# peter-seres/python-ray-tracer

Hardware: AMD Instinct MI355X
Metric: Mrays/sec + frame time (ms) at 1920x1080, 8 spheres, depth=3 (higher is better)
Workload: dtype f64

## Files before the change

### python-ray-tracer_amd/csrc/mi355rt.hip

```cpp
#include "../../include/mi355rt.h"
#include "rt_device.h"
#include "rt_bloom.h"
#include "rt_denoise.h"
#include "rt_denoise_var.h"
#include "rt_feedback.h"
#include "rt_film.h"
#include "rt_film_launch.h"
#include "rt_geometry.h"
#include "rt_guides.h"
#include "rt_launch.h"
#include "rt_plan.h"
#include "rt_scene.h"
#include "rt_streams.h"
#include "rt_temporal.h"

#include <cmath>
#include <cstdio>
#include <cstdlib>
#include <algorithm>
#include <array>
#include <cstring>
#include <memory>
#include <new>
#include <string>
#include <type_traits>
#include <utility>
#include <vector>

#pragma clang fp contract(off)

namespace {

std::string g_create_error;

struct Buf {
    void *p = nullptr;
    size_t cap = 0;
    Buf() = default;
    Buf(Buf &&o) noexcept { *this = std::move(o); }
    Buf &operator=(Buf &&o) noexcept { std::swap(p, o.p); std::swap(cap, o.cap); return *this; }
    ~Buf() { if (p) (void)hipFree(p); }
};

}

#define RT_COUNT_WORDS (4 + 2 * (RT_MAX_DEPTH + 1))
#define RT_RENDER_CHUNKS 8

struct rt_ctx {
    int device = 0;
    hipStream_t stream = nullptr;
    struct Pipeline {
        hipStream_t stream2 = nullptr, copy_stream = nullptr;
        hipEvent_t chunk_ev[RT_RENDER_CHUNKS] = {};
        hipStream_t chunk_stream[RT_RENDER_CHUNKS] = {};
        template <class F> void streams(F f)
        {
            for (hipStream_t s : {stream2, copy_stream}) if (s) f(s);
            for (hipStream_t s : chunk_stream) if (s) f(s);
        }
        ~Pipeline()
        {
            streams([](hipStream_t s) { (void)hipStreamDestroy(s); });
            for (hipEvent_t e : chunk_ev) if (e) (void)hipEventDestroy(e);
        }
    };
    std::unique_ptr<Pipeline> pipe;
    int chunk_mode = -1;
    int cluster_min = rt::CLUSTER_MIN;
    int lanes_primary = 1;
    rt::PlanKnobs knobs;
    int render_chunks = 4;
    int log_kernels = 0;
    int remeasure = 24;
    struct Slot {
        hipStream_t stream = nullptr;
        Buf u8, f32;
    } slots[RT_RENDER_SLOTS];
    hipEvent_t ev0 = nullptr, ev1 = nullptr;
    Buf scene[RT_SCENE_RING];
    int scene_cur = 0;
    Buf pixel_loc, u8, f32;
    rt::SceneLayout lay;
    Buf texels[RT_SCENE_RING];
    bool have_scene = false;
    rt::View view;
    size_t lds_limit_set[rt::FAMILIES] = {};
    size_t ground_lds_set = 0;
    size_t guides_lds_set = 0;
    unsigned *tile_stats = nullptr;
    struct Feedback : rt::FeedbackSlot {
        Buf cost, gtmp, btmp, order[2];
    } fbs[RT_FEEDBACK_SLOTS];
    rt::FeedbackBook book;
    rt_ctx() { for (int i = 0; i < RT_FEEDBACK_SLOTS; ++i) book.slot[i] = &fbs[i]; }
    template <class F> void own_streams(F f)
    {
        if (stream) f(stream);
        for (Slot &sl : slots) if (sl.stream) f(sl.stream);
        if (pipe) pipe->streams(f);
    }
    ~rt_ctx()
    {
        for (auto &f : fbs)
            for (void *e : rt::release_events(f)) (void)hipEventDestroy((hipEvent_t)e);
        pipe.reset();
        own_streams([](hipStream_t s) { (void)hipStreamDestroy(s); });
        for (hipEvent_t e : {ev0, ev1}) if (e) (void)hipEventDestroy(e);
    }
    rt_stats stats = {};
    Buf counts;
    int cu_count = 256;
    unsigned long long epoch = 1;
    unsigned long long scene_epoch = 1;
    rt::StreamBook<Buf> streams;
    std::string err;
};

namespace {

int fail(rt_ctx *ctx, int code, const std::string &msg)
{
    if (ctx) ctx->err = msg; else g_create_error = msg;
    return code;
}

#define RT_HIP(ctx, call)                                                                         \
    do {                                                                                          \
        hipError_t e_ = (call);                                                                   \
        if (e_ != hipSuccess)                                                                     \
            return fail((ctx), RT_ERR_HIP, std::string(#call) + ": " + hipGetErrorString(e_));    \
    } while (0)

int ensure(rt_ctx *ctx, Buf &b, size_t bytes)
{
    if (bytes <= b.cap) return RT_OK;
    if (b.p) { RT_HIP(ctx, hipFree(b.p)); b.p = nullptr; b.cap = 0; }
    RT_HIP(ctx, hipMalloc(&b.p, bytes));
    b.cap = bytes;
    return RT_OK;
}

int refuse(rt_ctx *ctx, const rt::Refusal &r)
{
    if (r.code == RT_OK) return RT_OK;
    return fail(ctx, r.code, r.entry ? std::string(r.entry) + ": " + r.msg : std::string(r.msg));
}

int check_params(rt_ctx *ctx, const rt_params *p, int x0, int x1) { return refuse(ctx, rt::check_params(ctx->have_scene, ctx->view, ctx->lay, p, x0, x1)); }

hipStream_t stream_of(rt_ctx *ctx, void *stream) { return stream ? (hipStream_t)stream : ctx->stream; }

using StreamRecord = rt::StreamBook<Buf>::Record;

int stream_record(rt_ctx *ctx, hipStream_t stream, StreamRecord **out)
{
    const int rc = ctx->streams.record(stream, out);
    if (rc != RT_OK) return fail(ctx, rc, ctx->streams.NO_MEMORY);
    ctx->streams.reads_scene(**out, ctx->scene_cur);
    return RT_OK;
}

int raise_lds(rt_ctx *ctx, const void *const *fns, size_t n, size_t lds, size_t &set)
{
    if (lds <= 48 * 1024 || lds <= set) return RT_OK;
    for (size_t i = 0; i < n; ++i)
        if (fns[i]) RT_HIP(ctx, hipFuncSetAttribute(fns[i], hipFuncAttributeMaxDynamicSharedMemorySize, (int)lds));
    set = lds;
    return RT_OK;
}

using rt::Shape; using rt::SHAPES; using rt::NSHAPES; using rt::has_kernel; using rt::has_ground_kernel;

template <rt::Family F, int I, bool GROUND = false>
const void *kernel_at()
{
    constexpr Shape s = SHAPES[I];
    if constexpr (GROUND ? has_ground_kernel(F, s) : has_kernel(F, s))
        return (const void *)rt::render_kernel<s.aa, s.park, s.wpw, s.count, s.lat, s.mode, F, GROUND>;
    else
        return nullptr;
}
template <rt::Family F, int... I>
std::array<const void *, NSHAPES> family_kernels(std::integer_sequence<int, I...>)
{
    return {kernel_at<F, I>()...};
}
template <int... I>
std::array<const void *, NSHAPES> ground_kernels(std::integer_sequence<int, I...>)
{
    return {kernel_at<rt::Family::PLAIN, I, true>()...};
}

constexpr std::make_integer_sequence<int, NSHAPES> ALL_SHAPES{};
const std::array<const void *, NSHAPES> KERNELS[rt::FAMILIES] = {
    family_kernels<rt::Family::PLAIN>(ALL_SHAPES), family_kernels<rt::Family::MAT>(ALL_SHAPES),
    family_kernels<rt::Family::REFR>(ALL_SHAPES),  family_kernels<rt::Family::SCAT>(ALL_SHAPES),
    family_kernels<rt::Family::SOFT>(ALL_SHAPES),  family_kernels<rt::Family::LENS>(ALL_SHAPES),
    family_kernels<rt::Family::LENS_SOFT>(ALL_SHAPES),
    family_kernels<rt::Family::TEX_SCAT>(ALL_SHAPES), family_kernels<rt::Family::TEX_SOFT>(ALL_SHAPES),
    family_kernels<rt::Family::TEX_LENS>(ALL_SHAPES), family_kernels<rt::Family::TEX_LENS_SOFT>(ALL_SHAPES),
    family_kernels<rt::Family::LIT_SCAT>(ALL_SHAPES), family_kernels<rt::Family::LIT_SOFT>(ALL_SHAPES),
    family_kernels<rt::Family::LIT_LENS>(ALL_SHAPES), family_kernels<rt::Family::LIT_LENS_SOFT>(ALL_SHAPES),
    family_kernels<rt::Family::SKY_SCAT>(ALL_SHAPES), family_kernels<rt::Family::SKY_SOFT>(ALL_SHAPES),
    family_kernels<rt::Family::SKY_LENS>(ALL_SHAPES), family_kernels<rt::Family::SKY_LENS_SOFT>(ALL_SHAPES),
};
const std::array<const void *, NSHAPES> GROUND_KERNELS = ground_kernels(ALL_SHAPES);
const std::array<const void *, NSHAPES> &kernels_of(int fi, bool ground) { return ground ? GROUND_KERNELS : KERNELS[fi]; }
static_assert(rt::FAMILIES == 19 && (int)rt::Family::TEX_LENS_SOFT == 10 && (int)rt::Family::LIT_LENS_SOFT == 14 &&
              (int)rt::Family::SKY_SCAT == 15 && (int)rt::Family::SKY_LENS_SOFT == 18,
              "KERNELS lists the families in enum order");

int stream_buffer(rt_ctx *ctx, Buf &b, hipStream_t stream, size_t bytes, bool sync)
{
    if (sync) RT_HIP(ctx, hipStreamSynchronize(stream));
    return ensure(ctx, b, bytes);
}

int acquire_tables(rt_ctx *ctx, StreamRecord &sr, const rt::KParams &k, const float **out)
{
    const hipStream_t stream = (hipStream_t)sr.stream;
    const rt::TableKey key = rt::table_key(ctx->scene_epoch, k.anchors, k.floor_anch, k.cam_o);
    const size_t bytes = rt::table_floats(k.S, k.NC, k.anchors, false, true, k.P) * sizeof(float);
    const rt::TableDecision d = ctx->streams.tables(sr, key, bytes);
    Buf &b = sr.buf[rt::BUF_TABLES0 + d.set];
    if (d.rebuild) {
        int rc = stream_buffer(ctx, b, stream, d.bytes, d.sync);
        if (rc != RT_OK) return rc;
        hipLaunchKernelGGL(rt::tables_kernel, dim3(1), dim3(rt::TABLE_THREADS), 0, stream, k, (float *)b.p);
        ctx->stats.table_builds++;
        RT_HIP(ctx, hipGetLastError());
        ctx->streams.tables_queued(sr, d.set, key);
    }
    *out = (const float *)b.p;
    return RT_OK;
}

int dispatch(rt_ctx *ctx, const rt_params *p, rt::KParams &k, const rt::LaunchPlan &plan, hipStream_t stream, int nframes, int64_t frame_stride);

int launch(rt_ctx *ctx, const rt_params *p, int x0, int x1, void *d_u8, void *d_f32, int64_t plane_stride,
           hipStream_t stream, int nframes = 1, int64_t frame_stride = 0)
{
    const rt::View &v = ctx->view;
    long long li0 = 0, li1 = 0;
    const bool lattice = p->aa_mode == RT_AA_REFERENCE && !v.explicit_grid && rt_geo_lattice(v.w, v.h, x0, x1, &li0, &li1) &&
                         !(p->flags & RT_FLAG_AA_PER_PIXEL);
    const rt::LaunchPlan plan = rt::plan_launch(ctx->lay, ctx->knobs, v.lens_a, !lattice && p->aa_mode != 0, p->flags, lattice, rt::anchors_of(ctx->lay));
    if (plan.index < 0 || !KERNELS[(int)plan.family][plan.index])
        return fail(ctx, RT_ERR_STATE, "no render kernel for this launch");
    StreamRecord *sr = nullptr;
    int rc = stream_record(ctx, stream, &sr);
    if (rc != RT_OK) return rc;
    rt::KParams k;
    rt::render_part(k, v, ctx->lay, plan.family, p, (const double *)ctx->scene[ctx->scene_cur].p, (const double *)ctx->pixel_loc.p,
                    (const float *)ctx->texels[ctx->scene_cur].p, ctx->lanes_primary, x0, x1, d_u8, d_f32, plane_stride, ctx->tile_stats);
    rc = acquire_tables(ctx, *sr, k, &k.ftab);
    if (rc != RT_OK) return rc;
    if (lattice) {
        Buf &lb = sr->buf[rt::BUF_LATTICE];
        const size_t bytes = (size_t)(li1 - li0) * (size_t)(2ll * v.h - 1) * 3 * sizeof(double);
        rc = stream_buffer(ctx, lb, stream, bytes, rt::growth(lb.cap, bytes).sync);
        if (rc != RT_OK) return rc;
        double *lat = (double *)lb.p;
        rt::KParams kl;
        rt::lattice_pair(k, kl, li0, li1, lat);
        const long long npx = (long long)(x1 - x0) * v.h;
        for (int f = 0; f < nframes; ++f) {
            rc = dispatch(ctx, p, kl, plan, stream, 1, 0);
            if (rc != RT_OK) return rc;
            const rt::KParams kf = rt::frame_params(k, f, frame_stride);
            hipLaunchKernelGGL(rt::aa_resolve_kernel, dim3((unsigned)((npx + 255) / 256)), dim3(256), 0, stream, kf);
            RT_HIP(ctx, hipGetLastError());
        }
        return RT_OK;
    }
    return dispatch(ctx, p, k, plan, stream, nframes, frame_stride);
}

using Feedback = rt_ctx::Feedback;
static_assert(std::is_convertible<hipStream_t, void *>::value && std::is_convertible<hipEvent_t, void *>::value,
              "rt_feedback.h keeps streams and events as opaque handles");
int feedback_slot(rt_ctx *ctx, const rt::FeedbackKey &key, Feedback **out);
int switch_order(rt_ctx *ctx, Feedback &f);
int launch_one(rt_ctx *ctx, rt::KParams &k, const rt::LaunchPlan &plan, const rt_geo_plan &g, const rt::OrderShape &os,
               Feedback *f, hipStream_t stream, int nframes, int64_t frame_stride);

int dispatch(rt_ctx *ctx, const rt_params *p, rt::KParams &k, const rt::LaunchPlan &plan, hipStream_t stream, int nframes, int64_t frame_stride)
{
    const int x0 = k.x0, x1 = k.x1;
    const rt_geo_plan g = rt_geo_plan_of(x0, x1, k.h, plan.shape.wpw, nframes);
    auto frame_of = [&](int fr) { return rt::frame_params(k, fr, frame_stride); };
    if (g.nslabs > 1) {
        for (int fr = 0; fr < nframes; ++fr)
            for (long long s = 0; s < g.nslabs; ++s) {
                rt::KParams kf = rt::slab_params(frame_of(fr), g, s);
                int rc = dispatch(ctx, p, kf, plan, stream, 1, 0);
                if (rc != RT_OK) return rc;
            }
        return RT_OK;
    }
    if (nframes > g.frames_per_dispatch) {
        const int fpd = (int)g.frames_per_dispatch;
        for (int fr = 0; fr < nframes; fr += fpd) {
            rt::KParams kf = frame_of(fr);
            int rc = dispatch(ctx, p, kf, plan, stream, std::min(fpd, nframes - fr), frame_stride);
            if (rc != RT_OK) return rc;
        }
        return RT_OK;
    }
    const rt::OrderShape os = rt::order_shape(plan, ctx->knobs, p->flags, g);
    Feedback *f = nullptr;
    if (os.feedback) {
        int rc = feedback_slot(ctx, rt::feedback_key(x0, x1, k.h, k.aa, plan.shape.lat, k.depth, k.spp, os.code), &f);
        if (rc == RT_OK) rc = switch_order(ctx, *f);
        if (rc != RT_OK) return rc;
    }
    if (nframes > 1 && f && !rt::settled(*f, ctx->epoch, ctx->remeasure)) {
        rt::KParams kf = frame_of(0);
        int rc = dispatch(ctx, p, kf, plan, stream, 1, 0);
        if (rc != RT_OK) return rc;
        if (f->building) RT_HIP(ctx, hipEventSynchronize((hipEvent_t)f->done));
        rt::KParams kr = frame_of(1);
        return dispatch(ctx, p, kr, plan, stream, nframes - 1, frame_stride);
    }
    return launch_one(ctx, k, plan, g, os, f, stream, nframes, frame_stride);
}

int feedback_slot(rt_ctx *ctx, const rt::FeedbackKey &key, Feedback **out)
{
    bool live = false;
    const int i = ctx->book.find(key, &live);
    if (live) RT_HIP(ctx, hipDeviceSynchronize());
    ctx->book.claim(i, key);
    Feedback *f = &ctx->fbs[i];
    if (!f->done) {
        hipEvent_t ev = nullptr;
        RT_HIP(ctx, hipEventCreateWithFlags(&ev, hipEventDisableTiming));
        f->done = ev;
    }
    *out = f;
    return RT_OK;
}

int switch_order(rt_ctx *ctx, Feedback &f)
{
    if (!f.building) return RT_OK;
    const hipError_t q = hipEventQuery((hipEvent_t)f.done);
    if (q != hipSuccess) {
        (void)hipGetLastError();
        return RT_OK;
    }
    for (void *us : rt::switch_order(f)) {
        hipEvent_t ev = (hipEvent_t)rt::take_spare(f);
        if (!ev) RT_HIP(ctx, hipEventCreateWithFlags(&ev, hipEventDisableTiming));
        RT_HIP(ctx, hipEventRecord(ev, (hipStream_t)us));
        rt::add_fence(f, us, ev);
    }
    return RT_OK;
}

int launch_one(rt_ctx *ctx, rt::KParams &k, const rt::LaunchPlan &plan, const rt_geo_plan &g, const rt::OrderShape &os,
               Feedback *f, hipStream_t stream, int nframes, int64_t frame_stride)
{
    const Shape &sh = plan.shape;
    const int fi = (int)plan.family;
    const bool ground = rt::ground_plane(ctx->lay, ctx->knobs, plan.family, sh.count ? RT_FLAG_COUNT_RAYS : 0) && has_ground_kernel(plan.family, sh);
    const std::array<const void *, NSHAPES> &kernels = kernels_of(fi, ground);
    const void *fn = kernels[plan.index];
    if (!fn) return fail(ctx, RT_ERR_STATE, "no render kernel for this launch");
    const unsigned grid = (unsigned)g.blocks;
    if (ctx->log_kernels)
        std::fprintf(stderr, "mi355rt: render_kernel<%d, %d, %d, %d, %d, %d, (rt::Family)%d>%s\n", (int)sh.aa, (int)sh.park, sh.wpw, (int)sh.count,
                     (int)sh.lat, sh.mode, fi, ground ? " ground" : "");
    int rc = raise_lds(ctx, kernels.data(), kernels.size(), plan.lds, ground ? ctx->ground_lds_set : ctx->lds_limit_set[fi]);
    if (rc != RT_OK) return rc;
    if (sh.count) {
        if (!ctx->counts.p) {
            rc = ensure(ctx, ctx->counts, RT_COUNT_WORDS * sizeof(unsigned long long));
            if (rc != RT_OK) return rc;
            RT_HIP(ctx, hipMemsetAsync(ctx->counts.p, 0, RT_COUNT_WORDS * sizeof(unsigned long long), stream));
        }
        k.ray_counts = (unsigned long long *)ctx->counts.p;
    }
    const rt::FeedbackLaunch d = f ? rt::decide_launch(*f, stream, ctx->epoch, ctx->remeasure) : rt::FeedbackLaunch{};
    if (d.read >= 0) k.order = (const unsigned *)f->order[d.read].p;
    if (d.measure) {
        const size_t words = (size_t)os.items * sizeof(unsigned);
        rc = ensure(ctx, f->cost, words);
        if (rc == RT_OK) rc = ensure(ctx, f->btmp, words);
        if (rc == RT_OK) rc = ensure(ctx, f->order[0], 2 * words);
        if (rc == RT_OK) rc = ensure(ctx, f->order[1], 2 * words);
        if (rc == RT_OK) rc = ensure(ctx, f->gtmp, words + sizeof(unsigned));
        if (rc != RT_OK) return rc;
        for (void *ev : d.wait) RT_HIP(ctx, hipStreamWaitEvent(stream, (hipEvent_t)ev, 0));
        k.cost = (unsigned *)f->cost.p;
    }
    rt::dispatch_part(k, nframes, grid, frame_stride, os);
    void *args[] = {(void *)&k};
    RT_HIP(ctx, hipLaunchKernel(fn, dim3(grid * (unsigned)nframes), dim3(64 * sh.wpw), args, plan.lds, stream));
    ctx->stats.launches++;
    ctx->stats.frames += (uint64_t)nframes;
    if (d.settled) ctx->stats.launches_settled++;
    if (d.measure) ctx->stats.launches_measuring++;
    if (d.measure) {
        hipLaunchKernelGGL(rt::order_kernel, dim3(1), dim3(rt::ORDER_THREADS), 0, stream, (const unsigned *)f->cost.p,
                           (unsigned *)f->gtmp.p, (unsigned *)f->btmp.p, (unsigned *)f->order[d.write].p, (int)os.items, os.otiles ? os.gshift + os.wshift : os.gshift,
                           os.otiles ? os.wshift : 0, os.otiles ? k.ntiles : (int)grid);
        RT_HIP(ctx, hipEventRecord((hipEvent_t)f->done, stream));
        rt::order_queued(*f, ctx->epoch);
    }
    RT_HIP(ctx, hipGetLastError());
    return RT_OK;
}

template <class Prepare>
int variance_filter(rt_ctx *ctx, const rt::DenoiseVarArgs &common, int levels, const rt::FilmPingPong &pp, hipStream_t st, Prepare prepare)
{
    const dim3 grid(rt::denoise_grid((long long)common.ws * common.h, ctx->cu_count));
    for (int k = 0; k <= levels; ++k) {
        const rt::FilmWrite w = rt::film_write(true, levels, k, nullptr, 0, pp);
        if (k == 0) prepare(w, grid);
        else hipLaunchKernelGGL(rt::denoise_var_kernel, grid, dim3(rt::DENOISE_THREADS), 0, st, rt::denoise_var_write(common, w, levels, k));
        RT_HIP(ctx, hipGetLastError());
    }
    return RT_OK;
}

template <class Args>
int temporal_launch(rt_ctx *ctx, void (*kernel)(Args), const Args &a, void *stream)
{
    RT_HIP(ctx, hipSetDevice(ctx->device));
    hipLaunchKernelGGL(kernel, dim3(rt::temporal_grid((long long)ctx->view.w * ctx->view.h, ctx->cu_count)), dim3(rt::TEMPORAL_THREADS), 0,
                       stream_of(ctx, stream), a);
    RT_HIP(ctx, hipGetLastError());
    return RT_OK;
}

}

extern "C" {

int rt_abi_version(void) { return RT_ABI_VERSION; }

int rt_device_count(int *count)
{
    if (!count) return RT_ERR_BAD_ARG;
    int n = 0;
    hipError_t e = hipGetDeviceCount(&n);
    if (e != hipSuccess) { *count = 0; g_create_error = std::string("hipGetDeviceCount: ") + hipGetErrorString(e); return RT_ERR_NO_DEVICE; }
    *count = n;
    return RT_OK;
}

int rt_create(rt_ctx **out, int device)
{
    if (!out) return fail(nullptr, RT_ERR_BAD_ARG, "ctx out-pointer is NULL");
    *out = nullptr;
    int n = 0;
    hipError_t e = hipGetDeviceCount(&n);
    if (e != hipSuccess || n <= 0)
        return fail(nullptr, RT_ERR_NO_DEVICE, std::string("no HIP device: ") + (e != hipSuccess ? hipGetErrorString(e) : "device count is 0"));
    if (device < 0 || device >= n) return fail(nullptr, RT_ERR_NO_DEVICE, "device index out of range");
    rt_ctx *ctx = new (std::nothrow) rt_ctx;
    if (!ctx) return fail(nullptr, RT_ERR_ALLOC, "out of host memory");
    ctx->device = device;
    if (const char *e = std::getenv("MI355RT_LANES_PRIMARY")) ctx->lanes_primary = std::atoi(e);
    if (const char *e = std::getenv("MI355RT_LANES_MINS")) ctx->knobs.lanes_min_spheres = std::atoi(e);
    if (const char *e = std::getenv("MI355RT_CLUSTER_MINS")) ctx->cluster_min = std::max(8, std::atoi(e));
    if (const char *e = std::getenv("MI355RT_CHUNK_MODE")) ctx->chunk_mode = std::atoi(e);
    if (const char *e = std::getenv("MI355RT_ORDER_GROUP")) { const int v = std::atoi(e); if (v >= 0 && v <= 6) ctx->knobs.order_group = v; }
    if (const char *e = std::getenv("MI355RT_REMEASURE")) ctx->remeasure = std::max(0, std::atoi(e));
    if (const char *e = std::getenv("MI355RT_F32_RECORDS")) ctx->knobs.f32_records = std::atoi(e) != 0;
    if (const char *e = std::getenv("MI355RT_WPW2_MAX_IMAGE")) ctx->knobs.wpw2_max_image = (size_t)std::max(0, std::atoi(e));
    if (const char *e = std::getenv("MI355RT_ORDER_TILES")) ctx->knobs.order_tiles = std::atoi(e) != 0;
    if (const char *e = std::getenv("MI355RT_LANES_PARK")) ctx->knobs.lanes_park = std::atoi(e) != 0;
    if (const char *e = std::getenv("MI355RT_GROUND_PLANE")) ctx->knobs.ground_plane = std::atoi(e) != 0;
    if (const char *e = std::getenv("MI355RT_LOG_KERNELS")) ctx->log_kernels = std::atoi(e) != 0;
    if (const char *e = std::getenv("MI355RT_SEQ_ORDER")) ctx->knobs.seq_order = std::atoi(e) != 0 ? 1 : 0;
    if (const char *e = std::getenv("MI355RT_CHUNKS")) { const int v = std::atoi(e); if (v >= 1 && v <= RT_RENDER_CHUNKS) ctx->render_chunks = v; }
    hipError_t s;
    if ((s = hipSetDevice(device)) != hipSuccess || (s = hipStreamCreateWithFlags(&ctx->stream, hipStreamNonBlocking)) != hipSuccess ||
        (s = hipEventCreate(&ctx->ev0)) != hipSuccess || (s = hipEventCreate(&ctx->ev1)) != hipSuccess) {
        std::string m = std::string("context setup: ") + hipGetErrorString(s);
        delete ctx;
        return fail(nullptr, RT_ERR_HIP, m);
    }
    {
        int cus = 0;
        if (hipDeviceGetAttribute(&cus, hipDeviceAttributeMultiprocessorCount, device) == hipSuccess && cus > 0) ctx->cu_count = cus;
        else (void)hipGetLastError();
    }
    *out = ctx;
    return RT_OK;
}

int rt_destroy(rt_ctx *ctx)
{
    if (!ctx) return RT_OK;
    (void)hipSetDevice(ctx->device);
    ctx->own_streams([](hipStream_t s) { (void)hipStreamSynchronize(s); });
    delete ctx;
    return RT_OK;
}

const char *rt_last_error(const rt_ctx *ctx) { return ctx ? ctx->err.c_str() : g_create_error.c_str(); }

static int set_scene(rt_ctx *ctx, const rt::SceneDesc &desc)
{
    if (!ctx) return RT_ERR_BAD_ARG;
    const rt::PackedScene ps = rt::pack_scene(desc, ctx->cluster_min, ctx->knobs.lanes_min_spheres);
    if (ps.status != RT_OK) return fail(ctx, ps.status, ps.error);
    RT_HIP(ctx, hipSetDevice(ctx->device));
    const size_t bytes = ps.rec.size() * sizeof(double);
    const int next = (ctx->scene_cur + 1) % RT_SCENE_RING;
    int rc = ctx->streams.drain_scene(next, [ctx](void *st) { RT_HIP(ctx, hipStreamSynchronize((hipStream_t)st)); return (int)RT_OK; });
    if (rc == RT_OK) rc = ensure(ctx, ctx->scene[next], bytes);
    if (rc != RT_OK) return rc;
    if (ps.layout.T > 0 || ps.layout.lit) {
        rc = ensure(ctx, ctx->texels[next], ps.texels.size() * sizeof(float));
        if (rc != RT_OK) return rc;
        RT_HIP(ctx, hipMemcpyAsync(ctx->texels[next].p, ps.texels.data(), ps.texels.size() * sizeof(float), hipMemcpyHostToDevice, ctx->stream));
    }
    RT_HIP(ctx, hipMemcpyAsync(ctx->scene[next].p, ps.rec.data(), bytes, hipMemcpyHostToDevice, ctx->stream));
    RT_HIP(ctx, hipStreamSynchronize(ctx->stream));
    ctx->scene_cur = next;
    ctx->lay = ps.layout;
    ctx->have_scene = true;
    ctx->epoch++;
    ctx->scene_epoch++;
    return RT_OK;
}

static rt::SceneDesc scene_desc(const float *spheres, int S, const float *lights, int L, const float *planes, int P, int flags,
                                const double *materials, int M, int ncols, const int32_t *sphere_material, const int32_t *plane_material)
{
    rt::SceneDesc d;
    d.spheres = spheres; d.S = S; d.lights = lights; d.L = L; d.planes = planes; d.P = P; d.flags = flags;
    d.materials = materials; d.M = M; d.ncols = ncols; d.sphere_material = sphere_material; d.plane_material = plane_material;
    return d;
}

static void add_textures(rt::SceneDesc &d, const rt_texture *textures, int T, const int32_t *sphere_texture, const int32_t *plane_texture,
                         const float *texels, int64_t n_texels)
{
    d.textures = textures; d.T = T; d.sphere_texture = sphere_texture; d.plane_texture = plane_texture;
    d.texels = texels; d.n_texels = n_texels;
}

static int set_scene_radii(rt_ctx *ctx, rt::SceneDesc &d, const float *light_radius, int shadow_samples)
{
    if (!ctx) return RT_ERR_BAD_ARG;
    if (d.L > 0 && !light_radius) return fail(ctx, RT_ERR_BAD_ARG, "light_radius is NULL with L > 0");
    static const float none = 0.0f;
    d.light_radius = light_radius ? light_radius : &none;
    d.shadow_samples = shadow_samples;
    return set_scene(ctx, d);
}

int rt_set_scene(rt_ctx *ctx, const float *spheres, int S, const float *lights, int L, const float *planes, int P, int flags)
{
    return set_scene(ctx, scene_desc(spheres, S, lights, L, planes, P, flags, nullptr, 0, 3, nullptr, nullptr));
}

int rt_set_scene_materials(rt_ctx *ctx, const float *spheres, int S, const float *lights, int L, const float *planes, int P, int flags,
                           const double *materials, int M, const int32_t *sphere_material, const int32_t *plane_material)
{
    return set_scene(ctx, scene_desc(spheres, S, lights, L, planes, P, flags, materials, M, 3, sphere_material, plane_material));
}

int rt_set_scene_materials_ex(rt_ctx *ctx, const float *spheres, int S, const float *lights, int L, const float *planes, int P, int flags,
                              const double *materials, int M, int ncols, const int32_t *sphere_material, const int32_t *plane_material)
{
    if (!ctx) return RT_ERR_BAD_ARG;
    if (ncols != 3 && ncols != 5) return fail(ctx, RT_ERR_BAD_ARG, "ncols must be 3 or 5");
    return set_scene(ctx, scene_desc(spheres, S, lights, L, planes, P, flags, materials, M, ncols, sphere_material, plane_material));
}

int rt_set_scene_materials_scatter(rt_ctx *ctx, const float *spheres, int S, const float *lights, int L, const float *planes, int P,
                                   int flags, const double *materials, int M, int ncols, const int32_t *sphere_material,
                                   const int32_t *plane_material)
{
    return set_scene(ctx, scene_desc(spheres, S, lights, L, planes, P, flags, materials, M, ncols, sphere_material, plane_material));
}

int rt_set_scene_area_lights(rt_ctx *ctx, const float *spheres, int S, const float *lights, int L, const float *planes, int P,
                             int flags, const double *materials, int M, int ncols, const int32_t *sphere_material,
                             const int32_t *plane_material, const float *light_radius, int shadow_samples)
{
    rt::SceneDesc d = scene_desc(spheres, S, lights, L, planes, P, flags, materials, M, ncols, sphere_material, plane_material);
    return set_scene_radii(ctx, d, light_radius, shadow_samples);
}

int rt_set_scene_textures(rt_ctx *ctx, const float *spheres, int S, const float *lights, int L, const float *planes, int P,
                          int flags, const double *materials, int M, int ncols, const int32_t *sphere_material,
                          const int32_t *plane_material, const float *light_radius, int shadow_samples,
                          const rt_texture *textures, int T, const int32_t *sphere_texture, const int32_t *plane_texture,
                          const float *texels, int64_t n_texels)
{
    rt::SceneDesc d = scene_desc(spheres, S, lights, L, planes, P, flags, materials, M, ncols, sphere_material, plane_material);
    add_textures(d, textures, T, sphere_texture, plane_texture, texels, n_texels);
    return set_scene_radii(ctx, d, light_radius, shadow_samples);
}

int rt_set_scene_lighting(rt_ctx *ctx, const float *spheres, int S, const float *lights, int L, const float *planes, int P,
                          int flags, const double *materials, int M, int ncols, const int32_t *sphere_material,
                          const int32_t *plane_material, const float *light_radius, int shadow_samples,
                          const rt_texture *textures, int T, const int32_t *sphere_texture, const int32_t *plane_texture,
                          const float *texels, int64_t n_texels, const float *light_rgb)
{
    rt::SceneDesc d = scene_desc(spheres, S, lights, L, planes, P, flags, materials, M, ncols, sphere_material, plane_material);
    add_textures(d, textures, T, sphere_texture, plane_texture, texels, n_texels);
    d.light_rgb = light_rgb; d.lighting = true;
    return set_scene_radii(ctx, d, light_radius, shadow_samples);
}

int rt_set_scene_sky(rt_ctx *ctx, const float *spheres, int S, const float *lights, int L, const float *planes, int P,
                     int flags, const double *materials, int M, int ncols, const int32_t *sphere_material,
                     const int32_t *plane_material, const float *light_radius, int shadow_samples,
                     const rt_texture *textures, int T, const int32_t *sphere_texture, const int32_t *plane_texture,
                     const float *texels, int64_t n_texels, const float *light_rgb, const double *sky)
{
    rt::SceneDesc d = scene_desc(spheres, S, lights, L, planes, P, flags, materials, M, ncols, sphere_material, plane_material);
    add_textures(d, textures, T, sphere_texture, plane_texture, texels, n_texels);
    d.light_rgb = light_rgb; d.lighting = true; d.sky = sky;
    return set_scene_radii(ctx, d, light_radius, shadow_samples);
}

int rt_set_camera(rt_ctx *ctx, const double origin[3], const double rotation[9])
{
    if (!ctx) return RT_ERR_BAD_ARG;
    if (!origin || !rotation) return fail(ctx, RT_ERR_BAD_ARG, "NULL camera array");
    rt::View &v = ctx->view;
    if (v.have_cam && std::memcmp(v.cam_o, origin, sizeof v.cam_o) == 0 &&
        std::memcmp(v.cam_R, rotation, sizeof v.cam_R) == 0) return RT_OK;
    std::memcpy(v.cam_o, origin, sizeof v.cam_o);
    std::memcpy(v.cam_R, rotation, sizeof v.cam_R);
    v.have_cam = true;
    ctx->epoch++;
    return RT_OK;
}

int rt_set_lens(rt_ctx *ctx, double aperture, double focus_distance)
{
    if (!ctx) return RT_ERR_BAD_ARG;
    if (!(std::isfinite(aperture) && aperture >= 0.0)) return fail(ctx, RT_ERR_BAD_ARG, "aperture must be finite and >= 0");
    if (!(std::isfinite(focus_distance) && focus_distance > 0.0))
        return fail(ctx, RT_ERR_BAD_ARG, "focus_distance must be finite and > 0");
    rt::View &v = ctx->view;
    if (aperture == v.lens_a && (focus_distance == v.lens_f || aperture == 0.0)) { v.lens_f = focus_distance; return RT_OK; }
    v.lens_a = aperture;
    v.lens_f = focus_distance;
    ctx->epoch++;
    return RT_OK;
}

int rt_set_raygen(rt_ctx *ctx, int w, int h, double px, double y0, double dy, double z0, double dz)
{
    if (!ctx) return RT_ERR_BAD_ARG;
    if (!rt_geo_frame_ok(w, h)) return fail(ctx, RT_ERR_BAD_ARG, "frame size out of range (1 <= w <= 2^31 - 8, 1 <= h <= 2^29 - 32, w*h <= 2^31)");
    rt::View &v = ctx->view;
    {
        const double now[5] = {px, y0, dy, z0, dz}, was[5] = {v.px, v.y0, v.dy, v.z0, v.dz};
        if (v.have_grid && !v.explicit_grid && v.w == w && v.h == h && std::memcmp(now, was, sizeof now) == 0)
            return RT_OK;
    }
    v.w = w; v.h = h; v.px = px; v.y0 = y0; v.dy = dy; v.z0 = z0; v.dz = dz;
    v.explicit_grid = false;
    v.have_grid = true;
    ctx->epoch++;
    return RT_OK;
}

int rt_set_pixel_loc(rt_ctx *ctx, const double *pixel_loc, int w, int h)
{
    if (!ctx) return RT_ERR_BAD_ARG;
    if (!pixel_loc) return fail(ctx, RT_ERR_BAD_ARG, "pixel_loc is NULL");
    if (!rt_geo_frame_ok(w, h)) return fail(ctx, RT_ERR_BAD_ARG, "frame size out of range (1 <= w <= 2^31 - 8, 1 <= h <= 2^29 - 32, w*h <= 2^31)");
    RT_HIP(ctx, hipSetDevice(ctx->device));
    const size_t bytes = (size_t)3 * w * h * sizeof(double);
    if (ctx->pixel_loc.p) RT_HIP(ctx, hipDeviceSynchronize());
    int rc = ensure(ctx, ctx->pixel_loc, bytes);
    if (rc != RT_OK) return rc;
    RT_HIP(ctx, hipMemcpyAsync(ctx->pixel_loc.p, pixel_loc, bytes, hipMemcpyHostToDevice, ctx->stream));
    RT_HIP(ctx, hipStreamSynchronize(ctx->stream));
    ctx->view.w = w; ctx->view.h = h;
    ctx->view.explicit_grid = true;
    ctx->view.have_grid = true;
    ctx->epoch++;
    return RT_OK;
}

int rt_render_device(rt_ctx *ctx, const rt_params *params, int x0, int x1, void *d_u8, void *d_f32, int64_t plane_stride, void *stream)
{
    if (!ctx) return RT_ERR_BAD_ARG;
    int rc = check_params(ctx, params, x0, x1);
    if (rc == RT_OK) rc = refuse(ctx, rt::check_device_outputs(ctx->view, params, x0, x1, 1, d_u8, d_f32, plane_stride, 0));
    if (rc != RT_OK) return rc;
    RT_HIP(ctx, hipSetDevice(ctx->device));
    return launch(ctx, params, x0, x1, d_u8, d_f32, plane_stride, stream_of(ctx, stream));
}

int rt_render_sequence(rt_ctx *ctx, const rt_params *params, int x0, int x1, int n, void *d_u8, void *d_f32, int64_t plane_stride,
                       int64_t frame_stride, const double *cameras, void *const *streams, int n_streams, int frames_per_launch)
{
    if (!ctx) return RT_ERR_BAD_ARG;
    if (n < 0) return fail(ctx, RT_ERR_BAD_ARG, "rt_render_sequence: negative frame count");
    if (n == 0) return RT_OK;
    if (cameras) {
        int rc0 = rt_set_camera(ctx, cameras, cameras + 3);
        if (rc0 != RT_OK) return rc0;
    }
    int rc = check_params(ctx, params, x0, x1);
    if (rc == RT_OK) rc = refuse(ctx, rt::check_device_outputs(ctx->view, params, x0, x1, n, d_u8, d_f32, plane_stride, frame_stride));
    if (rc != RT_OK) return rc;
    if (n_streams < 0 || (n_streams > 0 && !streams)) return fail(ctx, RT_ERR_BAD_ARG, "rt_render_sequence: n_streams without a stream array");
    RT_HIP(ctx, hipSetDevice(ctx->device));
    auto stream_of = [&](int i) { return (n_streams > 0 && streams[i % n_streams]) ? (hipStream_t)streams[i % n_streams] : ctx->stream; };
    uint8_t *u8 = (uint8_t *)d_u8;
    float *f32 = (float *)d_f32;
    if (cameras) {
        for (int i = 0; i < n; ++i) {
            rc = rt_set_camera(ctx, cameras + 12 * (size_t)i, cameras + 12 * (size_t)i + 3);
            if (rc == RT_OK) rc = launch(ctx, params, x0, x1, u8 ? u8 + (size_t)i * frame_stride : nullptr,
                                         f32 ? f32 + (size_t)i * frame_stride : nullptr, plane_stride, stream_of(i));
            if (rc != RT_OK) return rc;
        }
        return RT_OK;
    }
    const int fpl = frames_per_launch > 0 ? frames_per_launch : 8;
    for (int i = 0, g = 0; i < n; i += fpl, ++g) {
        const int nf = std::min(fpl, n - i);
        rc = launch(ctx, params, x0, x1, u8 ? u8 + (size_t)i * frame_stride : nullptr, f32 ? f32 + (size_t)i * frame_stride : nullptr,
                    plane_stride, stream_of(g), nf, frame_stride);
        if (rc != RT_OK) return rc;
    }
    return RT_OK;
}

static int film_queue_passes(rt_ctx *ctx, const rt_params *params, int x0, int x1, int passes, int reset, void *d_sum, int64_t sum_stride,
                             void *d_sq, int64_t sq_stride, void *stream)
{
    int rc = RT_OK;
    const long long npx = (long long)(x1 - x0) * ctx->view.h;
    RT_HIP(ctx, hipSetDevice(ctx->device));
    hipStream_t st = stream_of(ctx, stream);
    rt_params p = *params;
    p.flags &= ~(RT_FLAG_U8_RGB | RT_FLAG_U8_HWC);
    const rt::FilmBatch fb = rt::film_batch(npx, passes);
    StreamRecord *sr = nullptr;
    rc = stream_record(ctx, st, &sr);
    if (rc != RT_OK) return rc;
    Buf &scratch = sr->buf[rt::BUF_FILM];
    rc = stream_buffer(ctx, scratch, st, fb.batch * fb.pass_bytes, rt::growth(scratch.cap, fb.batch * fb.pass_bytes).sync);
    if (rc != RT_OK) return rc;
    float *const frames = (float *)scratch.p;
    const dim3 grid(rt::film_grid((npx + 3) >> 2, ctx->cu_count, 3), 3);
    for (int i = 0; i < passes; i += fb.batch) {
        const int nb = std::min(fb.batch, passes - i), first = (reset && i == 0) ? 1 : 0;
        for (int b = 0; b < nb; ++b) {
            p.seed = params->seed + (uint32_t)(i + b);
            rc = launch(ctx, &p, x0, x1, nullptr, frames + (size_t)b * 3 * fb.fplane, fb.fplane, st);
            if (rc != RT_OK) return rc;
        }
        if (d_sq) hipLaunchKernelGGL(rt::film_add2_kernel, grid, dim3(rt::FILM_THREADS), 0, st,
                                     rt::film_add2_args(d_sum, sum_stride, d_sq, sq_stride, frames, fb.fplane, npx, nb, first));
        else hipLaunchKernelGGL(rt::film_add_kernel, grid, dim3(rt::FILM_THREADS), 0, st, rt::film_add_args(d_sum, sum_stride, frames, fb.fplane, npx, nb, first));
        RT_HIP(ctx, hipGetLastError());
    }
    return RT_OK;
}

int rt_film_accumulate(rt_ctx *ctx, const rt_params *params, int x0, int x1, int passes, int reset, void *d_sum, int64_t sum_stride,
                       void *stream)
{
    if (!ctx) return RT_ERR_BAD_ARG;
    int rc = refuse(ctx, rt::check_film_accumulate("rt_film_accumulate", ctx->have_scene, ctx->view, ctx->lay, params, x0, x1, passes, d_sum, sum_stride,
                                                   false, nullptr, 0));
    if (rc != RT_OK) return rc;
    return film_queue_passes(ctx, params, x0, x1, passes, reset, d_sum, sum_stride, nullptr, 0, stream);
}

int rt_film_accumulate_moments(rt_ctx *ctx, const rt_params *params, int x0, int x1, int passes, int reset, void *d_sum, int64_t sum_stride,
                               void *d_sq, int64_t sq_stride, void *stream)
{
    if (!ctx) return RT_ERR_BAD_ARG;
    int rc = refuse(ctx, rt::check_film_accumulate("rt_film_accumulate_moments", ctx->have_scene, ctx->view, ctx->lay, params, x0, x1, passes, d_sum,
                                                   sum_stride, true, d_sq, sq_stride));
    if (rc != RT_OK) return rc;
    return film_queue_passes(ctx, params, x0, x1, passes, reset, d_sum, sum_stride, d_sq, sq_stride, stream);
}

int rt_film_resolve(rt_ctx *ctx, const void *d_sum, int64_t sum_stride, int ws, int h, int64_t n, const rt_film_tone *tone,
                    void *d_u8, void *d_f32, int64_t out_stride, void *stream)
{
    if (!ctx) return RT_ERR_BAD_ARG;
    int rc = refuse(ctx, rt::check_film_resolve(d_sum, sum_stride, ws, h, n, tone, d_u8, d_f32, out_stride));
    if (rc != RT_OK) return rc;
    RT_HIP(ctx, hipSetDevice(ctx->device));
    const rt::FilmResolveArgs a = rt::film_resolve_args(d_sum, sum_stride, ws, h, n, tone, d_u8, d_f32, out_stride);
    hipLaunchKernelGGL(rt::film_resolve_kernel, dim3(rt::film_grid((a.npx + 3) >> 2, ctx->cu_count, 1)), dim3(rt::FILM_THREADS), 0,
                       stream_of(ctx, stream), a);
    RT_HIP(ctx, hipGetLastError());
    return RT_OK;
}

int rt_render_guides(rt_ctx *ctx, int x0, int x1, void *d_guides, int64_t plane_stride, void *stream)
{
    if (!ctx) return RT_ERR_BAD_ARG;
    if (!d_guides) return fail(ctx, RT_ERR_BAD_ARG, "rt_render_guides: d_guides is NULL");
    const rt::View &v = ctx->view;
    int rc = refuse(ctx, rt::check_state(ctx->have_scene, v));
    if (rc == RT_OK) rc = refuse(ctx, rt::check_columns(v, x0, x1));
    if (rc != RT_OK) return rc;
    if (plane_stride < (int64_t)(x1 - x0) * v.h) return fail(ctx, RT_ERR_BAD_ARG, "rt_render_guides: plane_stride smaller than the slab");
    RT_HIP(ctx, hipSetDevice(ctx->device));
    hipStream_t st = stream_of(ctx, stream);
    StreamRecord *sr = nullptr;
    rc = stream_record(ctx, st, &sr);
    if (rc != RT_OK) return rc;
    rt::KParams k;
    rt::guides_part(k, v, ctx->lay, (const double *)ctx->scene[ctx->scene_cur].p, (const double *)ctx->pixel_loc.p,
                    (const float *)ctx->texels[ctx->scene_cur].p, ctx->lanes_primary, x0, x1, d_guides, plane_stride);
    const rt::GuidesPlan plan = rt::plan_guides(ctx->lay, ctx->knobs, k.anchors);
    if (ctx->log_kernels) std::fprintf(stderr, "mi355rt: guides_kernel<%d>\n", plan.mode);
    rc = acquire_tables(ctx, *sr, k, &k.ftab);
    if (rc != RT_OK) return rc;
    const void *fn = plan.mode == 2 ? (const void *)rt::guides_kernel<2> : (plan.mode == 1 ? (const void *)rt::guides_kernel<1> : (const void *)rt::guides_kernel<0>);
    const void *const all[] = {(const void *)rt::guides_kernel<0>, (const void *)rt::guides_kernel<1>, (const void *)rt::guides_kernel<2>};
    rc = raise_lds(ctx, all, 3, plan.lds, ctx->guides_lds_set);
    if (rc != RT_OK) return rc;
    rt::div_magic((unsigned)k.tiles_y, k.tiles_y_magic, k.tiles_y_shift);
    const rt_geo_plan g = rt_geo_plan_of(x0, x1, v.h, rt::GUIDE_WPW, 1);
    for (long long s = 0; s < g.nslabs; ++s) {
        rt::KParams ks = rt::slab_params(k, g, s);
        int tex = ctx->lay.T > 0 ? 1 : 0;
        void *args[] = {(void *)&ks, (void *)&tex};
        const unsigned blocks = (unsigned)((ks.ntiles + rt::GUIDE_WPW - 1) / rt::GUIDE_WPW);
        RT_HIP(ctx, hipLaunchKernel(fn, dim3(blocks), dim3(64 * rt::GUIDE_WPW), args, plan.lds, st));
    }
    RT_HIP(ctx, hipGetLastError());
    return RT_OK;
}

int rt_film_denoise(rt_ctx *ctx, const void *d_sum, int64_t sum_stride, int ws, int h, int64_t n, const void *d_guides, int64_t guide_stride,
                    const rt_denoise *dn, void *d_out, int64_t out_stride, void *d_work, int64_t work_stride, void *stream)
{
    if (!ctx) return RT_ERR_BAD_ARG;
    int nsq = -1;
    int rc = refuse(ctx, rt::check_film_denoise(d_sum, sum_stride, ws, h, n, d_guides, guide_stride, dn, d_out, out_stride, d_work, work_stride, nsq));
    if (rc != RT_OK) return rc;
    RT_HIP(ctx, hipSetDevice(ctx->device));
    hipStream_t st = stream_of(ctx, stream);
    const rt::FilmPingPong pp = {d_out, out_stride, d_work, work_stride};
    const dim3 grid(rt::denoise_grid((long long)ws * h, ctx->cu_count));
    for (int i = 0; i < (dn->levels ? dn->levels : 1); ++i) {
        const rt::FilmWrite w = rt::film_write(false, dn->levels, i, d_sum, sum_stride, pp);
        hipLaunchKernelGGL(rt::denoise_kernel, grid, dim3(rt::DENOISE_THREADS), 0, st, rt::denoise_args(w, d_guides, guide_stride, ws, h, n, dn, nsq, i));
        RT_HIP(ctx, hipGetLastError());
    }
    return RT_OK;
}

int rt_film_denoise_variance(rt_ctx *ctx, const void *d_sum, int64_t sum_stride, const void *d_sq, int64_t sq_stride, int ws, int h, int64_t n,
                             const void *d_guides, int64_t guide_stride, const rt_denoise_variance *dv, void *d_out, int64_t out_stride,
                             void *d_work, int64_t work_stride, void *stream)
{
    if (!ctx) return RT_ERR_BAD_ARG;
    int nsq = -1;
    int rc = refuse(ctx, rt::check_film_denoise_variance(d_sum, sum_stride, d_sq, sq_stride, ws, h, n, d_guides, guide_stride, dv, d_out, out_stride,
                                                         d_work, work_stride, nsq));
    if (rc != RT_OK) return rc;
    RT_HIP(ctx, hipSetDevice(ctx->device));
    hipStream_t st = stream_of(ctx, stream);
    rt::DenoiseVarArgs a = rt::denoise_var_common(d_guides, guide_stride, ws, h, dv, nsq);
    rt::denoise_var_inputs(a, d_sum, sum_stride, d_sq, sq_stride, n, dv->levels);
    return variance_filter(ctx, a, dv->levels, {d_out, out_stride, d_work, work_stride}, st, [&](const rt::FilmWrite &w, dim3 grid) {
        hipLaunchKernelGGL(rt::denoise_var_prepare_kernel, grid, dim3(rt::DENOISE_THREADS), 0, st, rt::denoise_var_write(a, w, dv->levels, 0));
    });
}

int rt_film_temporal(rt_ctx *ctx, const void *d_sum, int64_t sum_stride, int64_t n, const void *d_guides, int64_t guide_stride,
                     const void *d_hist, int64_t hist_stride, const void *d_hist_len, const void *d_hist_guides, int64_t hist_guide_stride,
                     const rt_temporal *tp, void *d_out, int64_t out_stride, void *d_out_len, void *stream)
{
    if (!ctx) return RT_ERR_BAD_ARG;
    const rt::View &v = ctx->view;
    int rc = refuse(ctx, rt::check_film_temporal("rt_film_temporal", v, d_sum, sum_stride, n, d_guides, guide_stride, d_hist, hist_stride, d_hist_len,
                                                 d_hist_guides, hist_guide_stride, tp, d_out, out_stride, d_out_len));
    if (rc != RT_OK) return rc;
    rt::TemporalArgs a;
    rt::temporal_args(a, v, d_sum, sum_stride, n, d_guides, guide_stride, d_hist, hist_stride, d_hist_len, d_hist_guides, hist_guide_stride, tp, d_out,
                      out_stride, d_out_len);
    return temporal_launch(ctx, rt::temporal_kernel, a, stream);
}

int rt_film_temporal_moments(rt_ctx *ctx, const void *d_sum, int64_t sum_stride, const void *d_sq, int64_t sq_stride, int64_t n,
                             const void *d_guides, int64_t guide_stride, const void *d_hist, int64_t hist_stride, const void *d_hist_sq,
                             int64_t hist_sq_stride, const void *d_hist_len, const void *d_hist_guides, int64_t hist_guide_stride,
                             const rt_temporal *tp, void *d_out, int64_t out_stride, void *d_out_sq, int64_t out_sq_stride, void *d_out_len,
                             void *stream)
{
    if (!ctx) return RT_ERR_BAD_ARG;
    const rt::View &v = ctx->view;
    int rc = refuse(ctx, rt::check_film_temporal_moments(v, d_sum, sum_stride, d_sq, sq_stride, n, d_guides, guide_stride, d_hist, hist_stride, d_hist_sq,
                                                         hist_sq_stride, d_hist_len, d_hist_guides, hist_guide_stride, tp, d_out, out_stride, d_out_sq,
                                                         out_sq_stride, d_out_len));
    if (rc != RT_OK) return rc;
    rt::TemporalMomentsArgs m;
    rt::temporal_args(m.t, v, d_sum, sum_stride, n, d_guides, guide_stride, d_hist, hist_stride, d_hist_len, d_hist_guides, hist_guide_stride, tp, d_out,
                      out_stride, d_out_len);
    rt::temporal_moments_args(m, d_sq, sq_stride, d_hist_sq, hist_sq_stride, d_out_sq, out_sq_stride);
    return temporal_launch(ctx, rt::temporal_moments_kernel, m, stream);
}

int rt_film_denoise_variance_temporal(rt_ctx *ctx, const void *d_mean, int64_t mean_stride, const void *d_msq, int64_t msq_stride,
                                      const void *d_len, int ws, int h, const void *d_guides, int64_t guide_stride,
                                      const rt_denoise_variance *dv, double spatial_below, void *d_out, int64_t out_stride, void *d_work,
                                      int64_t work_stride, void *stream)
{
    if (!ctx) return RT_ERR_BAD_ARG;
    int nsq = -1;
    int rc = refuse(ctx, rt::check_film_denoise_variance_temporal(d_mean, mean_stride, d_msq, msq_stride, d_len, ws, h, d_guides, guide_stride, dv,
                                                                  spatial_below, d_out, out_stride, d_work, work_stride, nsq));
    if (rc != RT_OK) return rc;
    RT_HIP(ctx, hipSetDevice(ctx->device));
    hipStream_t st = stream_of(ctx, stream);
    return variance_filter(ctx, rt::denoise_var_common(d_guides, guide_stride, ws, h, dv, nsq), dv->levels, {d_out, out_stride, d_work, work_stride}, st,
                           [&](const rt::FilmWrite &w, dim3 grid) {
        hipLaunchKernelGGL(rt::denoise_var_prepare_len_kernel, grid, dim3(rt::DENOISE_THREADS), 0, st,
                           rt::denoise_var_len_args(w, d_mean, mean_stride, d_msq, msq_stride, d_len, ws, h, d_guides, guide_stride, dv, spatial_below));
    });
}

int rt_film_bloom(rt_ctx *ctx, const void *d_sum, int64_t sum_stride, int ws, int h, int64_t n, const rt_bloom *bl, void *d_out,
                  int64_t out_stride, void *d_work, int64_t work_stride, void *stream)
{
    if (!ctx) return RT_ERR_BAD_ARG;
    int rc = refuse(ctx, rt::check_film_bloom(d_sum, sum_stride, ws, h, n, bl, d_out, out_stride, d_work, work_stride));
    if (rc != RT_OK) return rc;
    RT_HIP(ctx, hipSetDevice(ctx->device));
    hipStream_t st = stream_of(ctx, stream);
    const rt::BloomPlan plan = rt::bloom_plan(bl->levels, bl->flags);
    const dim3 grid(rt::bloom_grid((long long)ws * h, ctx->cu_count)), tiles(rt::bloom_tile_blocks(ws, h), 3), threads(rt::BLOOM_THREADS);
    for (int k = 0; k < plan.count; ++k) {
        const rt::BloomLaunch &l = plan.l[k];
        const rt::BloomArgs a = rt::bloom_args(l, d_sum, sum_stride, ws, h, n, bl, d_out, out_stride, d_work, work_stride);
        if (l.kind == rt::BLOOM_BRIGHT) hipLaunchKernelGGL(rt::bloom_bright_kernel, grid, threads, 0, st, a);
        else if (l.kind == rt::BLOOM_X) hipLaunchKernelGGL(rt::bloom_x_kernel, grid, threads, 0, st, a);
        else if (l.kind == rt::BLOOM_Y) hipLaunchKernelGGL(rt::bloom_y_kernel, grid, threads, 0, st, a);
        else if (l.step == 1) hipLaunchKernelGGL(rt::bloom_tile_kernel<1>, tiles, threads, 0, st, a);
        else if (l.step == 2) hipLaunchKernelGGL(rt::bloom_tile_kernel<2>, tiles, threads, 0, st, a);
        else hipLaunchKernelGGL(rt::bloom_tile_kernel<4>, tiles, threads, 0, st, a);
        RT_HIP(ctx, hipGetLastError());
    }
    return RT_OK;
}

static int render_staged(rt_ctx *ctx, const rt_params *params, int x0, int x1, uint8_t *out_u8, float *out_f32, Buf &u8, Buf &f32,
                         hipStream_t stream)
{
    const size_t npx = (size_t)(x1 - x0) * ctx->view.h;
    int rc = out_u8 ? ensure(ctx, u8, 3 * npx) : RT_OK;
    if (rc == RT_OK && out_f32) rc = ensure(ctx, f32, 3 * npx * sizeof(float));
    if (rc == RT_OK)
        rc = launch(ctx, params, x0, x1, out_u8 ? u8.p : nullptr, out_f32 ? f32.p : nullptr,
                    (params->flags & RT_FLAG_U8_HWC) ? (int64_t)(x1 - x0) : (int64_t)npx, stream);
    if (rc != RT_OK) return rc;
    if (out_u8) RT_HIP(ctx, hipMemcpyAsync(out_u8, u8.p, 3 * npx, hipMemcpyDeviceToHost, stream));
    if (out_f32) RT_HIP(ctx, hipMemcpyAsync(out_f32, f32.p, 3 * npx * sizeof(float), hipMemcpyDeviceToHost, stream));
    return RT_OK;
}

int rt_render(rt_ctx *ctx, const rt_params *params, int x0, int x1, uint8_t *out_u8, float *out_f32)
{
    if (!ctx) return RT_ERR_BAD_ARG;
    int rc = check_params(ctx, params, x0, x1);
    if (rc != RT_OK) return rc;
    if (!out_u8 && !out_f32) return fail(ctx, RT_ERR_BAD_ARG, "both output pointers are NULL");
    RT_HIP(ctx, hipSetDevice(ctx->device));
    const size_t npx = (size_t)(x1 - x0) * ctx->view.h;
    if (out_u8 && (rc = ensure(ctx, ctx->u8, 3 * npx)) != RT_OK) return rc;
    if (out_f32 && (rc = ensure(ctx, ctx->f32, 3 * npx * sizeof(float))) != RT_OK) return rc;
    if ((rc = refuse(ctx, rt::check_host_hwc(params, out_f32))) != RT_OK) return rc;
    const bool hwc = (params->flags & RT_FLAG_U8_HWC) != 0;
    const long long tiles = rt_geo_tiles(x1 - x0);
    const int NCH = ctx->render_chunks;
    if (hwc || NCH < 2 || npx < (1u << 19) || tiles < 4 * NCH) {
        rc = render_staged(ctx, params, x0, x1, out_u8, out_f32, ctx->u8, ctx->f32, ctx->stream);
        if (rc != RT_OK) return rc;
        RT_HIP(ctx, hipStreamSynchronize(ctx->stream));
        return RT_OK;
    }
    bool instream = false;
    {
        hipPointerAttribute_t at;
        void *probe = out_u8 ? (void *)out_u8 : (void *)out_f32;
        if (hipPointerGetAttributes(&at, probe) == hipSuccess) instream = (at.type == hipMemoryTypeHost);
        else (void)hipGetLastError();
        if (ctx->chunk_mode >= 0) instream = ctx->chunk_mode == 1;
    }
    if (!ctx->pipe) {
        std::unique_ptr<rt_ctx::Pipeline> pl(new (std::nothrow) rt_ctx::Pipeline);
        if (!pl) return fail(ctx, RT_ERR_ALLOC, "out of host memory");
        RT_HIP(ctx, hipStreamCreateWithFlags(&pl->stream2, hipStreamNonBlocking));
        RT_HIP(ctx, hipStreamCreateWithFlags(&pl->copy_stream, hipStreamNonBlocking));
        for (auto &e : pl->chunk_ev) RT_HIP(ctx, hipEventCreateWithFlags(&e, hipEventDisableTiming));
        int lo = 0, hi = 0;
        RT_HIP(ctx, hipDeviceGetStreamPriorityRange(&lo, &hi));
        for (int c = 0; c < RT_RENDER_CHUNKS; ++c)
            RT_HIP(ctx, hipStreamCreateWithPriority(&pl->chunk_stream[c], hipStreamNonBlocking, std::min(lo, hi + c)));
        ctx->pipe = std::move(pl);
    }
    rt_ctx::Pipeline &pl = *ctx->pipe;
    int cx[RT_RENDER_CHUNKS + 1];
    for (int c = 0; c <= NCH; ++c) cx[c] = (int)rt_geo_chunk_x(x0, x1, NCH, c);
    auto copy_chunk = [&](size_t off, size_t n, hipStream_t s) -> int {
        if (out_u8) {
            if (rt_geo_copy_2d((long long)npx, 1))
                RT_HIP(ctx, hipMemcpy2DAsync(out_u8 + off, npx, (uint8_t *)ctx->u8.p + off, npx, n, 3, hipMemcpyDeviceToHost, s));
            else
                for (size_t c = 0; c < 3; ++c)
                    RT_HIP(ctx, hipMemcpyAsync(out_u8 + c * npx + off, (uint8_t *)ctx->u8.p + c * npx + off, n, hipMemcpyDeviceToHost, s));
        }
        if (out_f32) {
            if (rt_geo_copy_2d((long long)npx, sizeof(float)))
                RT_HIP(ctx, hipMemcpy2DAsync(out_f32 + off, npx * sizeof(float), (float *)ctx->f32.p + off, npx * sizeof(float),
                                             n * sizeof(float), 3, hipMemcpyDeviceToHost, s));
            else
                for (size_t c = 0; c < 3; ++c)
                    RT_HIP(ctx, hipMemcpyAsync(out_f32 + c * npx + off, (float *)ctx->f32.p + c * npx + off, n * sizeof(float),
                                               hipMemcpyDeviceToHost, s));
        }
        return RT_OK;
    };
    unsigned *const tile_stats = ctx->tile_stats;
    const int tiles_y = (ctx->view.h + rt::TILE - 1) / rt::TILE;
    for (int c = 0; c < NCH; ++c) {
        hipStream_t s = instream ? pl.chunk_stream[c] : ((c & 1) ? pl.stream2 : ctx->stream);
        const size_t off = (size_t)(cx[c] - x0) * ctx->view.h, n = (size_t)(cx[c + 1] - cx[c]) * ctx->view.h;
        if (tile_stats) ctx->tile_stats = tile_stats + (size_t)((cx[c] - x0) / rt::TILE) * tiles_y;
        rc = launch(ctx, params, cx[c], cx[c + 1], out_u8 ? (uint8_t *)ctx->u8.p + off : nullptr,
                    out_f32 ? (float *)ctx->f32.p + off : nullptr, (int64_t)npx, s);
        ctx->tile_stats = tile_stats;
        if (rc != RT_OK) return rc;
        if (instream) {
            if ((rc = copy_chunk(off, n, s)) != RT_OK) return rc;
        } else RT_HIP(ctx, hipEventRecord(pl.chunk_ev[c], s));
    }
    if (instream) {
        for (int c = 0; c < NCH; ++c) RT_HIP(ctx, hipStreamSynchronize(pl.chunk_stream[c]));
        return RT_OK;
    }
    for (int c = 0; c < NCH; ++c) {
        const size_t off = (size_t)(cx[c] - x0) * ctx->view.h, n = (size_t)(cx[c + 1] - cx[c]) * ctx->view.h;
        RT_HIP(ctx, hipStreamWaitEvent(pl.copy_stream, pl.chunk_ev[c], 0));
        if ((rc = copy_chunk(off, n, pl.copy_stream)) != RT_OK) return rc;
    }
    RT_HIP(ctx, hipStreamSynchronize(pl.copy_stream));
    return RT_OK;
}

int rt_render_begin(rt_ctx *ctx, const rt_params *params, int x0, int x1, uint8_t *out_u8, float *out_f32, int slot)
{
    if (!ctx) return RT_ERR_BAD_ARG;
    int rc = check_params(ctx, params, x0, x1);
    if (rc != RT_OK) return rc;
    if (slot < 0 || slot >= RT_RENDER_SLOTS) return fail(ctx, RT_ERR_BAD_ARG, "rt_render_begin: slot outside 0..RT_RENDER_SLOTS-1");
    if (!out_u8 && !out_f32) return fail(ctx, RT_ERR_BAD_ARG, "both output pointers are NULL");
    if ((rc = refuse(ctx, rt::check_host_hwc(params, out_f32))) != RT_OK) return rc;
    RT_HIP(ctx, hipSetDevice(ctx->device));
    rt_ctx::Slot &sl = ctx->slots[slot];
    if (!sl.stream) RT_HIP(ctx, hipStreamCreateWithFlags(&sl.stream, hipStreamNonBlocking));
    return render_staged(ctx, params, x0, x1, out_u8, out_f32, sl.u8, sl.f32, sl.stream);
}

int rt_render_end(rt_ctx *ctx, int slot)
{
    if (!ctx) return RT_ERR_BAD_ARG;
    if (slot < 0 || slot >= RT_RENDER_SLOTS) return fail(ctx, RT_ERR_BAD_ARG, "rt_render_end: slot outside 0..RT_RENDER_SLOTS-1");
    RT_HIP(ctx, hipSetDevice(ctx->device));
    if (ctx->slots[slot].stream) RT_HIP(ctx, hipStreamSynchronize(ctx->slots[slot].stream));
    return RT_OK;
}

int rt_host_alloc(rt_ctx *ctx, size_t bytes, void **hptr)
{
    if (!ctx) return RT_ERR_BAD_ARG;
    if (!hptr || bytes == 0) return fail(ctx, RT_ERR_BAD_ARG, "rt_host_alloc: NULL out-pointer or zero size");
    RT_HIP(ctx, hipSetDevice(ctx->device));
    RT_HIP(ctx, hipHostMalloc(hptr, bytes, hipHostMallocDefault));
    return RT_OK;
}

int rt_host_free(rt_ctx *ctx, void *hptr)
{
    if (!hptr) return RT_OK;
    if (ctx) RT_HIP(ctx, hipSetDevice(ctx->device));
    RT_HIP(ctx, hipHostFree(hptr));
    return RT_OK;
}

int rt_malloc(rt_ctx *ctx, size_t bytes, void **dptr)
{
    if (!ctx) return RT_ERR_BAD_ARG;
    if (!dptr || bytes == 0) return fail(ctx, RT_ERR_BAD_ARG, "rt_malloc: NULL out-pointer or zero size");
    RT_HIP(ctx, hipSetDevice(ctx->device));
    RT_HIP(ctx, hipMalloc(dptr, bytes));
    return RT_OK;
}

int rt_free(rt_ctx *ctx, void *dptr)
{
    if (!ctx) return RT_ERR_BAD_ARG;
    if (!dptr) return RT_OK;
    RT_HIP(ctx, hipSetDevice(ctx->device));
    RT_HIP(ctx, hipStreamSynchronize(ctx->stream));
    RT_HIP(ctx, hipFree(dptr));
    return RT_OK;
}

int rt_memcpy_h2d(rt_ctx *ctx, void *dst_device, const void *src_host, size_t bytes)
{
    if (!ctx) return RT_ERR_BAD_ARG;
    if (!dst_device || !src_host) return fail(ctx, RT_ERR_BAD_ARG, "rt_memcpy_h2d: NULL pointer");
    RT_HIP(ctx, hipSetDevice(ctx->device));
    RT_HIP(ctx, hipMemcpyAsync(dst_device, src_host, bytes, hipMemcpyHostToDevice, ctx->stream));
    RT_HIP(ctx, hipStreamSynchronize(ctx->stream));
    return RT_OK;
}

int rt_memcpy_d2h(rt_ctx *ctx, void *dst_host, const void *src_device, size_t bytes)
{
    if (!ctx) return RT_ERR_BAD_ARG;
    if (!dst_host || !src_device) return fail(ctx, RT_ERR_BAD_ARG, "rt_memcpy_d2h: NULL pointer");
    RT_HIP(ctx, hipSetDevice(ctx->device));
    RT_HIP(ctx, hipMemcpyAsync(dst_host, src_device, bytes, hipMemcpyDeviceToHost, ctx->stream));
    RT_HIP(ctx, hipStreamSynchronize(ctx->stream));
    return RT_OK;
}

int rt_sync(rt_ctx *ctx)
{
    if (!ctx) return RT_ERR_BAD_ARG;
    RT_HIP(ctx, hipSetDevice(ctx->device));
    RT_HIP(ctx, hipStreamSynchronize(ctx->stream));
    return RT_OK;
}

int rt_stream_create(rt_ctx *ctx, void **stream)
{
    if (!ctx) return RT_ERR_BAD_ARG;
    if (!stream) return fail(ctx, RT_ERR_BAD_ARG, "stream out-pointer is NULL");
    *stream = nullptr;
    RT_HIP(ctx, hipSetDevice(ctx->device));
    hipStream_t s = nullptr;
    RT_HIP(ctx, hipStreamCreateWithFlags(&s, hipStreamNonBlocking));
    *stream = (void *)s;
    return RT_OK;
}

static int forget_stream(rt_ctx *ctx, hipStream_t stream)
{
    RT_HIP(ctx, hipStreamSynchronize(stream));
    ctx->book.forget(stream);
    ctx->streams.forget(stream);
    return RT_OK;
}

int rt_stream_destroy(rt_ctx *ctx, void *stream)
{
    if (!ctx) return RT_ERR_BAD_ARG;
    if (!stream) return RT_OK;
    RT_HIP(ctx, hipSetDevice(ctx->device));
    int rc = forget_stream(ctx, (hipStream_t)stream);
    if (rc != RT_OK) return rc;
    RT_HIP(ctx, hipStreamDestroy((hipStream_t)stream));
    return RT_OK;
}

int rt_stream_forget(rt_ctx *ctx, void *stream)
{
    if (!ctx) return RT_ERR_BAD_ARG;
    if (!stream) return RT_OK;
    if ((hipStream_t)stream == ctx->stream) return fail(ctx, RT_ERR_BAD_ARG, "rt_stream_forget: the context's own stream");
    RT_HIP(ctx, hipSetDevice(ctx->device));
    return forget_stream(ctx, (hipStream_t)stream);
}

int rt_stream_sync(rt_ctx *ctx, void *stream)
{
    if (!ctx) return RT_ERR_BAD_ARG;
    RT_HIP(ctx, hipSetDevice(ctx->device));
    RT_HIP(ctx, hipStreamSynchronize(stream_of(ctx, stream)));
    return RT_OK;
}

int rt_timer_begin(rt_ctx *ctx, void *stream)
{
    if (!ctx) return RT_ERR_BAD_ARG;
    RT_HIP(ctx, hipSetDevice(ctx->device));
    RT_HIP(ctx, hipEventRecord(ctx->ev0, stream_of(ctx, stream)));
    return RT_OK;
}

int rt_timer_end(rt_ctx *ctx, void *stream, float *ms)
{
    if (!ctx) return RT_ERR_BAD_ARG;
    if (!ms) return fail(ctx, RT_ERR_BAD_ARG, "ms is NULL");
    RT_HIP(ctx, hipSetDevice(ctx->device));
    RT_HIP(ctx, hipEventRecord(ctx->ev1, stream_of(ctx, stream)));
    RT_HIP(ctx, hipEventSynchronize(ctx->ev1));
    RT_HIP(ctx, hipEventElapsedTime(ms, ctx->ev0, ctx->ev1));
    return RT_OK;
}

int rt_set_tile_stats(rt_ctx *ctx, void *d_cycles)
{
    if (!ctx) return RT_ERR_BAD_ARG;
    ctx->tile_stats = (unsigned *)d_cycles;
    return RT_OK;
}

int rt_get_stats(rt_ctx *ctx, rt_stats *out)
{
    if (!ctx) return RT_ERR_BAD_ARG;
    if (!out) return fail(ctx, RT_ERR_BAD_ARG, "stats is NULL");
    RT_HIP(ctx, hipSetDevice(ctx->device));
    unsigned long long c[RT_COUNT_WORDS] = {0};
    if (ctx->counts.p) {
        RT_HIP(ctx, hipDeviceSynchronize());
        RT_HIP(ctx, hipMemcpy(c, ctx->counts.p, sizeof c, hipMemcpyDeviceToHost));
    }
    *out = ctx->stats;
    out->closest_queries = c[0]; out->shadow_traced = c[1]; out->shadow_skipped = c[2]; out->hits = c[3];
    for (int b = 0; b <= RT_MAX_DEPTH; ++b) { out->bounce_waves[b] = c[4 + 2 * b]; out->bounce_lanes[b] = c[5 + 2 * b]; }
    return RT_OK;
}

int rt_reset_stats(rt_ctx *ctx)
{
    if (!ctx) return RT_ERR_BAD_ARG;
    RT_HIP(ctx, hipSetDevice(ctx->device));
    if (ctx->counts.p) {
        RT_HIP(ctx, hipDeviceSynchronize());
        RT_HIP(ctx, hipMemset(ctx->counts.p, 0, RT_COUNT_WORDS * sizeof(unsigned long long)));
    }
    ctx->stats = rt_stats{};
    return RT_OK;
}

int rt_get_kernel_info(rt_ctx *ctx, rt_kernel_info *info)
{
    if (!ctx) return RT_ERR_BAD_ARG;
    if (!info) return fail(ctx, RT_ERR_BAD_ARG, "info is NULL");
    RT_HIP(ctx, hipSetDevice(ctx->device));
    hipFuncAttributes a;
    const bool ground = ctx->have_scene && rt::ground_plane(ctx->lay, ctx->knobs, rt::Family::PLAIN, 0);
    const void *fn = ground ? (const void *)rt::render_kernel<false, true, 2, false, false, 0, rt::Family::PLAIN, true>
                            : (const void *)rt::render_kernel<false, true, 2>;
    RT_HIP(ctx, hipFuncGetAttributes(&a, fn));
    hipDeviceProp_t prop;
    RT_HIP(ctx, hipGetDeviceProperties(&prop, ctx->device));
    std::memset(info, 0, sizeof *info);
    info->vgprs = a.numRegs;
    info->lds_static = (int32_t)a.sharedSizeBytes;
    info->max_threads = a.maxThreadsPerBlock;
    info->wave_size = prop.warpSize;
    info->cu_count = prop.multiProcessorCount;
    info->clock_khz = prop.clockRate;
    return RT_OK;
}

}
```

### python-ray-tracer_amd/csrc/rt_device.h

```cpp
#pragma once
#include <hip/hip_runtime.h>
#include <stdint.h>
#include "rt_kparams.h"
#include "rt_math.h"
#include "rt_cull.h"
#include "rt_facing.h"
#include "rt_layout.h"

#pragma clang fp contract(off)

#ifndef RT_FAST_DIVSQRT
#define RT_FAST_DIVSQRT 1
#endif
#ifndef RT_FAST_NORMALIZE
#define RT_FAST_NORMALIZE 1
#endif
#ifndef RT_FACING_SKIP
#define RT_FACING_SKIP 1
#endif
#ifndef RT_DEFER_DIRECTION
#define RT_DEFER_DIRECTION 1
#endif
#ifndef RT_DEFER_SHADOW
#define RT_DEFER_SHADOW 1
#endif

namespace rt {

constexpr int TABLE_THREADS = 256;

__device__ __forceinline__ int div_by(int n, int d, unsigned M, unsigned sh)
{
    return d == 1 ? n : (int)(__umulhi((unsigned)n, M) >> sh);
}

__device__ __forceinline__ V3 normalize3(const V3 &v)
{
#if RT_FAST_NORMALIZE == 0
    return normalize3_generic(v);
#else
    const double nn = v.x * v.x + v.y * v.y + v.z * v.z;
    const double cmin = __builtin_fmin(__builtin_fmin(__builtin_fabs(v.x), __builtin_fabs(v.y)), __builtin_fabs(v.z));
    const bool ok = (cmin >= NORMALIZE_MIN_COMPONENT) && (nn <= NORMALIZE_MAX_NN);
    if (__builtin_amdgcn_ballot_w64(!ok) != 0ull) return normalize3_generic(v);
    return normalize3_seeded(v, nn, __builtin_amdgcn_rsq(nn));
#endif
}
__device__ __forceinline__ double div_inrange(double a, double b)
{
#if RT_FAST_DIVSQRT == 0
    return a / b;
#else
    return div_seeded(a, b, __builtin_amdgcn_rcp(b));
#endif
}
__device__ __forceinline__ double sqrt_inrange(double x)
{
#if RT_FAST_DIVSQRT == 0
    return __builtin_sqrt(x);
#else
    return sqrt_seeded(x, __builtin_amdgcn_rsq(x));
#endif
}
__device__ __forceinline__ V3 renormalize_unit(const V3 &d)
{
    const double nn = d.x * d.x + d.y * d.y + d.z * d.z;
    const double e = nn - 1.0;
    if (__builtin_amdgcn_ballot_w64(!(__builtin_fabs(e) < UNIT_WINDOW)) != 0ull) return normalize3_generic(d);
    return renormalize_unit_fast(d, e);
}

enum { HIT_NONE = 0, HIT_SPHERE = 1, HIT_PLANE = 2 };

typedef __attribute__((address_space(3))) double lds_f64;
__device__ __forceinline__ unsigned fresh_lane()
{
    unsigned l;
    asm volatile("v_mbcnt_lo_u32_b32 %0, -1, 0\n\tv_mbcnt_hi_u32_b32 %0, -1, %0" : "=v"(l));
    return l;
}
template <bool PARK, int WGT, bool REMAT = false> struct Park3 {
    volatile lds_f64 *p;
    volatile lds_f64 *sbase;
    V3 v;
    __device__ __forceinline__ Park3(double *base, int slot, int wave = 0)
        : p(REMAT ? nullptr : (volatile lds_f64 *)base + slot * 3 * WGT + threadIdx.x),
          sbase(REMAT ? (volatile lds_f64 *)base + slot * 3 * WGT + wave * 64 : nullptr), v{0.0, 0.0, 0.0} {}
    __device__ __forceinline__ volatile lds_f64 *at() const { if constexpr (REMAT) return sbase + fresh_lane(); else return p; }
    __device__ __forceinline__ void set(const V3 &a)
    {
        if constexpr (PARK) { volatile lds_f64 *q = at(); q[0] = a.x; q[WGT] = a.y; q[2 * WGT] = a.z; } else v = a;
    }
    __device__ __forceinline__ V3 get() const
    {
        if constexpr (PARK) { volatile lds_f64 *q = at(); return V3{q[0], q[WGT], q[2 * WGT]}; } else return v;
    }
};


template <Family F, int WSLOT, bool FRESH> struct MatState {
    static constexpr bool mat = has_mat(F), refr = has_refr(F), scat = has_scat(F), soft = has_soft(F), lens = has_lens(F), tex = has_tex(F), lit = has_lit(F), sky = has_sky(F);
    static constexpr int COLS = table_cols(F);
    unsigned tab;
    unsigned ids;
    int nsh;
    enum { W = 0, LAMB = 1, REFL = 2, QX = 3, QY = 4, QZ = 5, ETA = 6, ROUGH = 7, KEY = 8, LKEY = 9 };
    template <int WGT, int k> __device__ __forceinline__ volatile lds_f64 *at(const double *acc, int wave) const
    {
        if constexpr (FRESH) return (volatile lds_f64 *)acc + (WSLOT + k) * WGT + wave * 64 + fresh_lane();
        else return (volatile lds_f64 *)acc + (WSLOT + k) * WGT + threadIdx.x;
    }
    __device__ __forceinline__ volatile const lds_f64 *entry(int slot) const
    {
        unsigned t = tab, i = ids;
        asm volatile("" : "+s"(t), "+s"(i));
        typedef __attribute__((address_space(3))) const int lds_ci32;
        const int m = ((lds_ci32 *)(size_t)i)[slot];
        return (volatile const lds_f64 *)(size_t)t + COLS * m;
    }
};
#define SLOT(X) (*ms.template at<WGT, MS::X>(lds.acc, lds.wave))
template <int WSLOT, bool FRESH> struct MatState<Family::PLAIN, WSLOT, FRESH> {
    static_assert(!has_mat(Family::PLAIN), "MS::mat is has_mat(family) on both sides: the host folds p.lamb into facing_tau by the same predicate");
    static constexpr bool mat = false, refr = false, scat = false, soft = false, lens = false, tex = false, lit = false, sky = false;
};


extern __shared__ double lds_raw[];

struct Lds {
    __device__ __forceinline__ const double *recs() const { return lds_raw; }
    const float *sph32;
    const float *tab;
    const float *csph32;
    const float *ctab;
    const float *cbox;
    const float *gbox;
    const float *gtab;
    const float *col32;
    int NC;
    int wave;
    bool pairs;
    bool groups;
    bool trim;
    bool defer;
#ifdef RT_REGION_STATS
    unsigned *reg;
#endif
    double *acc;
};

#ifdef RT_REGION_STATS
__device__ __forceinline__ void region_mark(unsigned *reg, int id)
{
    volatile unsigned *r = reg + (threadIdx.x >> 6) * 32;
    const unsigned now = (unsigned)__builtin_amdgcn_s_memtime();
    const unsigned last = r[31], c = r[30];
    r[id + c] = r[id + c] + (now - last);
    r[31] = now;
}
#define RT_MARK(id) region_mark(lds.reg, id)
#else
#define RT_MARK(id)
#endif

typedef __attribute__((address_space(3))) const f4 lds_cf4;
__device__ __forceinline__ lds_cf4 *pin_lds(const float *generic)
{
    unsigned a = (unsigned)(size_t)(__attribute__((address_space(3))) const float *)generic;
    asm volatile("" : "+v"(a));
    return (lds_cf4 *)(size_t)a;
}

typedef unsigned long long lanemask;
__device__ __forceinline__ lanemask m_nlt_abs(float a, float b)
{
    lanemask m; asm volatile("v_cmp_nlt_f32_e64 %0, |%1|, %2" : "=s"(m) : "v"(a), "v"(b)); return m;
}
__device__ __forceinline__ lanemask m_nlt_neg(float a, float b)
{
    lanemask m; asm volatile("v_cmp_nlt_f32_e64 %0, %1, -%2" : "=s"(m) : "v"(a), "v"(b)); return m;
}
__device__ __forceinline__ lanemask m_ngt(float a, float b)
{
    lanemask m; asm volatile("v_cmp_ngt_f32_e64 %0, %1, %2" : "=s"(m) : "v"(a), "v"(b)); return m;
}
__device__ __forceinline__ lanemask m_ne(int a, int b)
{
    lanemask m; asm volatile("v_cmp_ne_u32_e64 %0, %1, %2" : "=s"(m) : "v"(a), "s"(b)); return m;
}
__device__ __forceinline__ unsigned push_any(unsigned acc, lanemask m)
{
    asm volatile("s_cmp_lg_u64 %1, 0\n\ts_addc_u32 %0, %0, %0" : "+s"(acc) : "s"(m) : "scc");
    return acc;
}

__device__ __forceinline__ int order_bucket(unsigned c)
{
    if (c < 32u) return (int)c;
    const int msb = 31 - __builtin_clz(c);
    return ((msb - 4) << 5) | (int)((c >> (msb - 5)) & 31u);
}
constexpr int ORDER_THREADS = 1024, ORDER_BUCKETS = 1024, ORDER_XCDS = 8;


struct RayBox { F3 inv, clo, chi; bool sane; };
__device__ __forceinline__ float vmin3(float a, float b, float c) { float r; asm("v_min3_f32 %0, %1, %2, %3" : "=v"(r) : "v"(a), "v"(b), "v"(c)); return r; }
__device__ __forceinline__ float vmax3(float a, float b, float c) { float r; asm("v_max3_f32 %0, %1, %2, %3" : "=v"(r) : "v"(a), "v"(b), "v"(c)); return r; }
__device__ __forceinline__ float vmin(float a, float b) { float r; asm("v_min_f32 %0, %1, %2" : "=v"(r) : "v"(a), "v"(b)); return r; }
__device__ __forceinline__ float vmax(float a, float b) { float r; asm("v_max_f32 %0, %1, %2" : "=v"(r) : "v"(a), "v"(b)); return r; }
__device__ __forceinline__ void raybox_axis(float o, float R, float m, float &inv, float &clo, float &chi)
{
    const float Rs = __builtin_fabsf(R) < 0x1p-40f ? __builtin_copysignf(0x1p-40f, R) : R;
    inv = __builtin_amdgcn_rcpf(Rs);
    const float a = -((o + m) * inv), b = -((o - m) * inv);
    const float da = __builtin_fabsf(a) * 0x1p-21f, db = __builtin_fabsf(b) * 0x1p-21f;
    clo = inv > 0.0f ? a - da : a + da;
    chi = inv > 0.0f ? b + db : b - db;
}
__device__ __forceinline__ RayBox make_raybox(const RayF &q, float extent2)
{
    RayBox rb;
    const float m = 0x1p-18f * (__builtin_sqrtf(extent2) + (__builtin_fabsf(q.o.x) + __builtin_fabsf(q.o.y) + __builtin_fabsf(q.o.z)));
    raybox_axis(q.o.x, q.R.x, m, rb.inv.x, rb.clo.x, rb.chi.x);
    raybox_axis(q.o.y, q.R.y, m, rb.inv.y, rb.clo.y, rb.chi.y);
    raybox_axis(q.o.z, q.R.z, m, rb.inv.z, rb.clo.z, rb.chi.z);
    const float chk = (q.o.x + q.o.y + q.o.z) + (q.R.x + q.R.y + q.R.z);
    rb.sane = (chk == chk) && __builtin_fabsf(chk) < 0x1p100f;
    return rb;
}
__device__ __forceinline__ bool box_open(const f4 lo, const f4 hi, const RayBox &rb)
{
    const float ax = __builtin_fmaf(lo[0], rb.inv.x, rb.clo.x), bx = __builtin_fmaf(hi[0], rb.inv.x, rb.chi.x);
    const float ay = __builtin_fmaf(lo[1], rb.inv.y, rb.clo.y), by = __builtin_fmaf(hi[1], rb.inv.y, rb.chi.y);
    const float az = __builtin_fmaf(lo[2], rb.inv.z, rb.clo.z), bz = __builtin_fmaf(hi[2], rb.inv.z, rb.chi.z);
    const float tn = vmax3(vmin(ax, bx), vmin(ay, by), vmin(az, bz));
    const float tf = vmin3(vmax(ax, bx), vmax(ay, by), vmax(az, bz));
    return !(tf < vmax(tn * (1.0f - 0x1p-18f), 0.0f));
}

template <bool ANCH, bool SELF, bool PAIRS>
__device__ __forceinline__ unsigned cull4(lds_cf4 *base, const RayF &q, int jsel, unsigned acc)
{
    static_assert(CULL_STRIDE == 4, "one 16-byte entry per (anchor, sphere)");
    f4 pending = {0.0f, 0.0f, 0.0f, 0.0f};
#pragma unroll
    for (int u = 3; u >= 0; --u) {
        f4 e;
        if constexpr (PAIRS) {
            if (u & 1) {
                asm volatile("" ::: "memory");
                e = base[u];
                f4 enext = base[u - 1];
                asm volatile("" : "+v"(e), "+v"(enext));
                pending = enext;
            } else e = pending;
        } else {
            asm volatile("" ::: "memory");
            e = base[u];
        }
        lanemask open;
        if constexpr (ANCH) {
            const float sd = __builtin_fmaf(e[2], q.R.z, __builtin_fmaf(e[1], q.R.y, e[0] * q.R.x));
            open = m_nlt_abs(sd, e[3]);
        } else {
            const float lx = q.o.x - e[0], ly = q.o.y - e[1], lz = q.o.z - e[2];
            const float sd = __builtin_fmaf(lz, q.R.z, __builtin_fmaf(ly, q.R.y, lx * q.R.x));
            const float ll = __builtin_fmaf(lz, lz, __builtin_fmaf(ly, ly, lx * lx));
            const float cc = ll - e[3];
            const float D = __builtin_fmaf(sd, sd, -cc);
            const float mg = __builtin_fmaf(CULL_K_ORIGIN, ll + e[3], q.mgq);
            const float es = __builtin_fmaf(CULL_K_S, ll, q.esq);
            open = m_nlt_neg(D, mg) & (m_ngt(sd, es) | m_ngt(cc, mg));
        }
        if constexpr (SELF) open &= m_ne(jsel, u);
        acc = push_any(acc, open);
    }
    return acc;
}

template <bool ANCH, bool SELF>
__device__ __forceinline__ unsigned long long cull_mask_t(const Lds &lds, int S, int anchor, int k0, int n,
                                                          const RayF &q, int selfj)
{
    unsigned long long mask = 0ull;
    const int Sp = padS(S, lds.NC);
    lds_cf4 *sbase = pin_lds(ANCH ? lds.tab + ((size_t)anchor * Sp + k0) * CULL_STRIDE : lds.sph32 + 4 * k0);
    if (lds.NC > 0) {
        const int NCp = pad4(lds.NC), c0 = k0 / CLUSTER, nc = (n + CLUSTER - 1) / CLUSTER;
        if (ANCH && lds.groups) {
            static_assert(CLUSTER * SUPER == 64, "a 64-sphere chunk is one group of clusters");
            const f4 ge = *pin_lds(lds.gtab + ((size_t)anchor * pad4(supers(lds.NC)) + (k0 >> 6)) * CULL_STRIDE);
            const float gs = __builtin_fmaf(ge[2], q.R.z, __builtin_fmaf(ge[1], q.R.y, ge[0] * q.R.x));
            if (m_nlt_abs(gs, ge[3]) == 0ull) return 0ull;
        }
        lds_cf4 *cbase = pin_lds(ANCH ? lds.ctab + ((size_t)anchor * NCp + c0) * CULL_STRIDE : lds.csph32 + 4 * c0);
        unsigned cm = 0;
        for (int j = 0; j < nc; j += 4) cm |= (lds.pairs ? cull4<ANCH, false, true>(cbase + j, q, -1, 0u) : cull4<ANCH, false, false>(cbase + j, q, -1, 0u)) << j;
        while (cm) {
            const int c = __builtin_ctz(cm);
            cm &= cm - 1u;
            const int jb = c * CLUSTER;
            const unsigned hi = lds.pairs ? cull4<ANCH, SELF, true>(sbase + jb + 4, q, selfj - jb - 4, 0u) : cull4<ANCH, SELF, false>(sbase + jb + 4, q, selfj - jb - 4, 0u);
            const unsigned lohi = lds.pairs ? cull4<ANCH, SELF, true>(sbase + jb, q, selfj - jb, hi) : cull4<ANCH, SELF, false>(sbase + jb, q, selfj - jb, hi);
            mask |= (unsigned long long)lohi << jb;
        }
    } else {
        const int npad = pad4(n);
        for (int j = 0; j < npad; j += 4) mask |= (unsigned long long)(lds.pairs ? cull4<ANCH, SELF, true>(sbase + j, q, selfj - j, 0u) : cull4<ANCH, SELF, false>(sbase + j, q, selfj - j, 0u)) << j;
    }
    return mask;
}

__device__ __forceinline__ unsigned long long cull_mask(const Lds &lds, int S, int anchor, int k0, int n,
                                                        const V3 &o, const F3 &dir, float extent2, int self)
{
    RayF q = make_rayf_dir(dir);
    if (anchor >= 0) {
        const bool cand = self >= k0 && self < k0 + n;
        if (__builtin_amdgcn_ballot_w64(cand) != 0ull) {
            add_origin(q, o, extent2);
            const float *cs = lds.sph32 + 4 * self;
            const bool self_culled = cand ? cull_origin(f4{cs[0], cs[1], cs[2], cs[3]}, q) : false;
            if (__builtin_amdgcn_ballot_w64(self_culled) != 0ull)
                return cull_mask_t<true, true>(lds, S, anchor, k0, n, q, self_culled ? self - k0 : -1);
        }
        return cull_mask_t<true, false>(lds, S, anchor, k0, n, q, -1);
    }
    add_origin(q, o, extent2);
    return cull_mask_t<false, false>(lds, S, anchor, k0, n, q, -1);
}

__device__ __forceinline__ unsigned long long cull_mask(const Lds &lds, int S, int anchor, int k0, int n,
                                                        const V3 &o, const V3 &R, float extent2, int self)
{
    return cull_mask(lds, S, anchor, k0, n, o, cull_dir32(R), extent2, self);
}


__device__ __forceinline__ int opaque(int x)
{
    asm volatile("" : "+s"(x));
    return x;
}

template <bool GROUND = false> __device__ __forceinline__ int plane_code(const KParams &p, int k)
{
    if constexpr (GROUND) return 3;
    unsigned c = p.plane_codes;
    asm volatile("" : "+s"(c));
    return k < 4 ? (int)(signed char)(c >> (8 * k)) : 0;
}

template <bool GROUND = false> __device__ __forceinline__ int plane_count(const KParams &p)
{
    if constexpr (GROUND) return 1;
    else return opaque(p.P);
}

__device__ __forceinline__ void plane_den_num(const double *__restrict__ g, int code, const V3 &o, const V3 &d, double &den, double &num,
                                              bool no_negate = false)
{
    if (code == 0) {
        const V3 n{g[3], g[4], g[5]};
        den = dot3(d, n);
        const V3 LP{g[0] - o.x, g[1] - o.y, g[2] - o.z};
        num = dot3(LP, n);
    } else {
        const int a = code < 0 ? -code : code;
        double dc, lp;
        if (a == 1)      { dc = d.x; lp = g[0] - o.x; }
        else if (a == 2) { dc = d.y; lp = g[1] - o.y; }
        else             { dc = d.z; lp = g[2] - o.z; }
        if (code > 0 || no_negate) { den = dc; num = lp; } else { den = -dc; num = -lp; }
    }
}

struct SphHot { double x, y, z, r2; };
template <bool F32> __device__ __forceinline__ SphHot sphere_hot(const Lds &lds, int k)
{
    if constexpr (F32) {
        const f4 c = *(lds_cf4 *)(size_t)(unsigned)(size_t)(__attribute__((address_space(3))) const float *)(lds.sph32 + 4 * k);
        return SphHot{(double)c[0], (double)c[1], (double)c[2], (double)c[3]};
    } else {
        const double *g = lds.recs() + k * SPH_STRIDE;
        return SphHot{g[0], g[1], g[2], g[3]};
    }
}
template <bool F32> __device__ __forceinline__ double sphere_orig(const Lds &lds, const KParams &p, int k)
{
    if constexpr (F32) return p.scene[(size_t)k * SPH_STRIDE + 7]; else return lds.recs()[k * SPH_STRIDE + 7];
}

template <bool F32>
__device__ __forceinline__ void sphere_closest(const Lds &lds, const KParams &p, int k, const V3 &o, const V3 &R, double a,
                                               double &bestn, int &bidx)
{
    const SphHot g = sphere_hot<F32>(lds, k);
    const V3 Lv{o.x - g.x, o.y - g.y, o.z - g.z};
    const double s = dot3(Lv, R);
    const double cc = dot3(Lv, Lv) - g.r2;
    const double D = s * s - a * cc;
    if (D >= 0.0 && !(s >= 0.0 && cc >= 0.0)) {
        const double q = sqrt_inrange(D);
        double n = -s - q;
        if (!(n > 0.0)) n = -s + q;
        if (n > 0.0) {
            bool take = n < bestn;
            const bool close = __builtin_fabs(n - bestn) < bestn * 0x1p-50;
            if (__builtin_amdgcn_ballot_w64(close) != 0ull) {
                if (close) {
                    const double tq = n / a, tb = bestn / a;
                    take = tq < tb || (tq == tb && sphere_orig<F32>(lds, p, k) < sphere_orig<F32>(lds, p, bidx));
                }
            }
            if (take) { bestn = n; bidx = k; }
        }
    }
}

template <bool F32>
__device__ __forceinline__ bool sphere_any(const Lds &lds, int k, const V3 &o, const V3 &R, double a, bool a_sane)
{
    const SphHot g = sphere_hot<F32>(lds, k);
    const V3 Lv{o.x - g.x, o.y - g.y, o.z - g.z};
    const double s = dot3(Lv, R);
    const double cc = dot3(Lv, Lv) - g.r2;
    const double D = s * s - a * cc;
    if (D >= 0.0 && !(s >= 0.0 && cc >= 0.0)) {
        if (s < 0.0 && -s < 499.0 && D < 249001.0 && a_sane) return true;
        const double q = __builtin_sqrt(D);
        double n = -s - q;
        if (!(n > 0.0)) n = -s + q;
        if (n > 0.0) {
            const double t = n / a;
            if (999.0 > t && t > 0.0) return true;
        }
    }
    return false;
}

__device__ __forceinline__ bool lane_of(lanemask m)
{
    unsigned x; asm("v_cndmask_b32_e64 %0, 0, 1, %1" : "=v"(x) : "s"(m)); return x != 0u;
}
__device__ __forceinline__ lanemask lanes_where(bool c) { return __builtin_amdgcn_ballot_w64(c); }

template <bool F32>
__device__ __forceinline__ lanemask sphere_any_mask(const Lds &lds, int k, const V3 &o, const V3 &R, double a, lanemask a_sane)
{
    const SphHot g = sphere_hot<F32>(lds, k);
    const V3 Lv{o.x - g.x, o.y - g.y, o.z - g.z};
    const double s = dot3(Lv, R);
    const double cc = dot3(Lv, Lv) - g.r2;
    const double D = s * s - a * cc;
    const lanemask dpos = lanes_where(D >= 0.0), sneg = lanes_where(s < 0.0);
    const lanemask cand = dpos & (sneg | lanes_where(!(cc >= 0.0)));
    const lanemask fast = dpos & sneg & lanes_where(-s < 499.0) & lanes_where(D < 249001.0) & a_sane;
    lanemask hit = fast;
    const lanemask slow = cand & ~fast;
    if (slow != 0ull) {
        bool h = false;
        if (lane_of(slow)) {
            const double q = __builtin_sqrt(D);
            double n = -s - q;
            if (!(n > 0.0)) n = -s + q;
            if (n > 0.0) {
                const double t = n / a;
                h = 999.0 > t && t > 0.0;
            }
        }
        hit |= lanes_where(h);
    }
    return hit;
}


template <bool ANCH>
__device__ __forceinline__ bool lane_open(const f4 e, const RayF &q)
{
    if constexpr (ANCH) {
        const float sd = __builtin_fmaf(e[2], q.R.z, __builtin_fmaf(e[1], q.R.y, e[0] * q.R.x));
        return !(__builtin_fabsf(sd) < e[3]);
    } else return !cull_origin(e, q);
}
__device__ __forceinline__ lds_cf4 *lds_f4(const float *generic)
{
    return (lds_cf4 *)(size_t)(unsigned)(size_t)(__attribute__((address_space(3))) const float *)generic;
}

template <bool ANCH>
__device__ __forceinline__ unsigned lane_cluster_bits(const Lds &lds, int anchor, int cb, int nc, const RayF &q, float extent2)
{
    unsigned cm = 0u;
    if constexpr (ANCH) {
        const int NCp = pad4(lds.NC), NGp = pad4(supers(lds.NC));
        lds_cf4 *base = pin_lds(lds.ctab + ((size_t)anchor * NCp + cb) * CULL_STRIDE);
        lds_cf4 *gbase = pin_lds(lds.gtab + ((size_t)anchor * NGp + cb / SUPER) * CULL_STRIDE);
        for (int c0 = 0; c0 < nc; c0 += SUPER) {
            if (__builtin_amdgcn_ballot_w64(lane_open<true>(gbase[c0 / SUPER], q)) == 0ull) continue;
            const int c1 = c0 + SUPER < nc ? c0 + SUPER : nc;
            for (int c = c0; c < c1; c += 4) {
#pragma unroll
                for (int u = 0; u < 4; ++u) {
                    asm volatile("" ::: "memory");
                    const f4 e = base[c + u];
                    cm |= lane_open<true>(e, q) ? (1u << (c + u)) : 0u;
                }
            }
        }
    } else {
        const RayBox rb = make_raybox(q, extent2);
        lds_cf4 *base = pin_lds(lds.cbox + (size_t)cb * BOX_STRIDE);
        lds_cf4 *gbase = pin_lds(lds.gbox + (size_t)(cb / SUPER) * BOX_STRIDE);
        static_assert(SUPER == 8, "a group's clusters are one byte of the mask");
        for (int c0 = 0; c0 < nc; c0 += SUPER) {
            const bool gopen = box_open(gbase[2 * (c0 / SUPER)], gbase[2 * (c0 / SUPER) + 1], rb) || !rb.sane;
            if (__builtin_amdgcn_ballot_w64(gopen) == 0ull) continue;
            const int c1 = c0 + SUPER < nc ? c0 + SUPER : nc;
            for (int c = c0; c < c1; c += 2) {
#pragma unroll
                for (int u = 0; u < 2; ++u) {
                    asm volatile("" ::: "memory");
                    const f4 lo = base[2 * (c + u)], hi = base[2 * (c + u) + 1];
                    cm |= box_open(lo, hi, rb) ? (1u << (c + u)) : 0u;
                }
            }
        }
        if (!rb.sane) cm = ~0u;
    }
    return cm & (nc >= 32 ? ~0u : ((1u << nc) - 1u));
}

template <bool ANCH>
__device__ __forceinline__ unsigned lane_sphere_bits(const Lds &lds, int S, int anchor, int kb, const RayF &q)
{
    const int Sp = padS(S, lds.NC);
    lds_cf4 *sb = lds_f4(ANCH ? lds.tab + ((size_t)anchor * Sp + kb) * CULL_STRIDE : lds.sph32 + 4 * kb);
    unsigned sm = 0u;
#pragma unroll
    for (int j = 0; j < CLUSTER; ++j) sm |= lane_open<ANCH>(sb[j], q) ? (1u << j) : 0u;
    const int nv = S - kb;
    return nv >= CLUSTER ? sm : (sm & ((1u << nv) - 1u));
}

#ifdef RT_LANE_STATS
__device__ __forceinline__ void lane_stats(const KParams &p, int base, unsigned v)
{
    if (!p.tile_cycles) return;
    unsigned mx = v, sum = v;
    for (int d = 32; d >= 1; d >>= 1) { const unsigned m2 = __shfl_xor(mx, d), s2 = __shfl_xor(sum, d); mx = m2 > mx ? m2 : mx; sum += s2; }
    if ((threadIdx.x & 63) == __builtin_ctzll(__builtin_amdgcn_ballot_w64(true))) {
        unsigned *c = p.tile_cycles + p.ntiles + base;
        atomicAdd(c + 0, 1u); atomicAdd(c + 1, mx); atomicAdd(c + 2, (sum + 63u) >> 6); atomicAdd(c + 3, sum);
    }
}
struct LaneCount {
    unsigned n;
    __device__ __forceinline__ LaneCount(unsigned v = 0u) : n(v) {}
    __device__ __forceinline__ void set(unsigned v) { n = v; }
    __device__ __forceinline__ void report(const KParams &p, int base) const { lane_stats(p, base, n); }
};
#else
struct LaneCount {
    __device__ __forceinline__ LaneCount(unsigned = 0u) {}
    __device__ __forceinline__ void set(unsigned) {}
    __device__ __forceinline__ void report(const KParams &, int) const {}
};
#endif
template <bool ANCH>
__device__ __forceinline__ void lanes_closest(const Lds &lds, const KParams &p, int anchor, const V3 &o, const V3 &R, double a,
                                              double &bestn, int &bidx)
{
    RayF q = make_rayf_dir(R);
    if constexpr (!ANCH) add_origin(q, o, p.extent2);
    for (int cb = 0; cb < lds.NC; cb += 32) {
        const int nc = lds.NC - cb < 32 ? lds.NC - cb : 32;
        unsigned cm = lane_cluster_bits<ANCH>(lds, anchor, cb, nc, q, p.extent2);
        RT_MARK(1);
        LaneCount(__builtin_popcount(cm)).report(p, 0);
        while (__builtin_amdgcn_ballot_w64(cm != 0u) != 0ull) {
            LaneCount smc;
            if (cm != 0u) {
                const int kb = (cb + __builtin_ctz(cm)) * CLUSTER;
                cm &= cm - 1u;
                unsigned sm = lane_sphere_bits<ANCH>(lds, p.S, anchor, kb, q);
                smc.set(__builtin_popcount(sm));
                while (__builtin_amdgcn_ballot_w64(sm != 0u) != 0ull) {
                    if (sm != 0u) {
                        const int k = kb + __builtin_ctz(sm);
                        sm &= sm - 1u;
                        sphere_closest<true>(lds, p, k, o, R, a, bestn, bidx);
                    }
                }
            }
            smc.report(p, 4);
        }
        RT_MARK(2);
    }
}

template <bool ANCH>
__device__ __forceinline__ bool lanes_any(const Lds &lds, const KParams &p, int anchor, const V3 &o, const V3 &R, double a, int self)
{
    const bool a_sane = (a > 0.999999 && a < 1.000001);
    RayF q = make_rayf_dir(R);
    bool self_culled = false;
    if constexpr (ANCH) {
        if (__builtin_amdgcn_ballot_w64(self >= 0) != 0ull) {
            add_origin(q, o, p.extent2);
            if (self >= 0) { const float *cs = lds.sph32 + 4 * self; self_culled = cull_origin(f4{cs[0], cs[1], cs[2], cs[3]}, q); }
        }
    } else add_origin(q, o, p.extent2);
    bool occ = false;
    for (int cb = 0; cb < lds.NC; cb += 32) {
        if (cb > 0 && __builtin_amdgcn_ballot_w64(!occ) == 0ull) break;
        const int nc = lds.NC - cb < 32 ? lds.NC - cb : 32;
        unsigned cm = lane_cluster_bits<ANCH>(lds, anchor, cb, nc, q, p.extent2);
        RT_MARK(7);
        if (occ) cm = 0u;
        LaneCount(__builtin_popcount(cm)).report(p, 8);
        while (__builtin_amdgcn_ballot_w64(cm != 0u) != 0ull) {
            LaneCount smc;
            if (cm != 0u) {
                const int kb = (cb + __builtin_ctz(cm)) * CLUSTER;
                cm &= cm - 1u;
                unsigned sm = lane_sphere_bits<ANCH>(lds, p.S, anchor, kb, q);
                if (self_culled && self >= kb && self < kb + CLUSTER) sm &= ~(1u << (self - kb));
                smc.set(__builtin_popcount(sm));
                while (__builtin_amdgcn_ballot_w64(sm != 0u) != 0ull) {
                    if (sm != 0u) {
                        const int k = kb + __builtin_ctz(sm);
                        sm &= sm - 1u;
                        if (sphere_any<true>(lds, k, o, R, a, a_sane)) { occ = true; sm = 0u; cm = 0u; }
                    }
                }
            }
            smc.report(p, 12);
        }
        RT_MARK(8);
    }
    return occ;
}

__device__ __forceinline__ double pinned_here(double x)
{
    asm volatile("" : "+v"(x));
    return x;
}
template <bool F32, bool IN_WINDOW>
__device__ __forceinline__ double closest_spheres(const Lds &lds, const KParams &p, int S, int canchor, const V3 &o, const V3 &d, double e,
                                                  double &bestn, int &bidx)
{
    double a = 1.0;
    V3 Rg{0.0, 0.0, 0.0};
    if constexpr (!IN_WINDOW) { Rg = normalize3_generic(d); a = dot3(Rg, Rg); }
    for (int k0 = 0; k0 < S; k0 += 64) {
      const int n = (S - k0 < 64) ? S - k0 : 64;
      unsigned long long mask = cull_mask(lds, S, canchor, k0, n, o, cull_dir32(IN_WINDOW ? d : Rg), p.extent2, -1);
      mask &= (n == 64) ? ~0ull : ((1ull << n) - 1ull);
      RT_MARK(1);
      if (mask) {
        V3 R = Rg;
        if constexpr (IN_WINDOW) { R = renormalize_unit_fast(d, pinned_here(e)); a = dot3(R, R); }
        do {
          const int k = k0 + __builtin_ctzll(mask);
          mask &= mask - 1ull;
          sphere_closest<F32>(lds, p, k, o, R, a, bestn, bidx);
        } while (mask);
      }
      RT_MARK(2);
    }
    return a;
}
template <bool IN_WINDOW>
__device__ __forceinline__ lanemask any_spheres_masks(const Lds &lds, const KParams &p, int S, int canchor, const V3 &o, const V3 &d, double e,
                                                      int self, lanemask live)
{
    lanemask occ = 0ull;
    V3 Rg{0.0, 0.0, 0.0};
    if constexpr (!IN_WINDOW) Rg = normalize3_generic(d);
    for (int k0 = 0; k0 < S; k0 += 64) {
      if (k0 > 0 && (live & ~occ) == 0ull) break;
      const int n = (S - k0 < 64) ? S - k0 : 64;
      unsigned long long mask = cull_mask(lds, S, canchor, k0, n, o, cull_dir32(IN_WINDOW ? d : Rg), p.extent2, self);
      mask &= (n == 64) ? ~0ull : ((1ull << n) - 1ull);
      RT_MARK(7);
      if (mask) {
        V3 R = Rg;
        if constexpr (IN_WINDOW) R = renormalize_unit_fast(d, pinned_here(e));
        const double a = dot3(R, R);
        const lanemask a_sane = lanes_where(a > 0.999999) & lanes_where(a < 1.000001);
        do {
          const int k = k0 + __builtin_ctzll(mask);
          mask &= mask - 1ull;
          occ |= sphere_any_mask<false>(lds, k, o, R, a, a_sane);
          if (mask && (live & ~occ) == 0ull) break;
        } while (mask);
      }
      RT_MARK(8);
    }
    return occ;
}

template <int MODE, bool GROUND = false>
__device__ __forceinline__ void closest_hit(const Lds &lds, const KParams &p, const V3 &o, const V3 &d, int anchor,
                                            double &t_out, int &idx_out, int &type_out)
{
    const int P = plane_count<GROUND>(p);
    const int S = p.S;
    constexpr bool F32 = MODE >= 1;
    double bestn = __builtin_inf();
    int bidx = -1;
    double aq;
    if (MODE < 2 && lds.defer) {
        const double e = unit_excess(d);
        const bool in_window = cull_reads_d(__builtin_amdgcn_ballot_w64(outside_unit_window(e)));
        RT_MARK(0);
        const int canchor = (opaque(p.anchors) > 0) ? anchor : -1;
        if (in_window) aq = closest_spheres<F32, true>(lds, p, S, canchor, o, d, e, bestn, bidx);
        else aq = closest_spheres<F32, false>(lds, p, S, canchor, o, d, e, bestn, bidx);
    } else {
    const V3 R = renormalize_unit(d);
    const double a = dot3(R, R);
    RT_MARK(0);
    const int canchor = (opaque(p.anchors) > 0) ? anchor : -1;
    if (MODE >= 2 && lds.NC > 0 && (canchor < 0 || p.lanes_primary)) {
        if (canchor >= 0) lanes_closest<true>(lds, p, canchor, o, R, a, bestn, bidx);
        else lanes_closest<false>(lds, p, -1, o, R, a, bestn, bidx);
    } else
    for (int k0 = 0; k0 < S; k0 += 64) {
      const int n = (S - k0 < 64) ? S - k0 : 64;
      unsigned long long mask = cull_mask(lds, S, canchor, k0, n, o, R, p.extent2, -1);
      mask &= (n == 64) ? ~0ull : ((1ull << n) - 1ull);
      RT_MARK(1);
      while (mask) {
        const int k = k0 + __builtin_ctzll(mask);
        mask &= mask - 1ull;
        sphere_closest<F32>(lds, p, k, o, R, a, bestn, bidx);
      }
      RT_MARK(2);
    }
    aq = a;
    }
    double best = 999.0;
    int idx = -1, type = HIT_NONE;
    if (bidx >= 0) {
        const double t = div_inrange(bestn, aq);
        if (best > t && t > 0.0) { best = t; idx = bidx; type = HIT_SPHERE; }
    }
    const double *pl = lds.recs() + (F32 ? 0 : opaque(p.S) * SPH_STRIDE);
    for (int k = 0; k < P; ++k) {
        const double *g = pl + k * PL_STRIDE;
        double den, num;
        plane_den_num(g, plane_code<GROUND>(p, k), o, d, den, num, lds.trim);
        if (!(__builtin_fabs(den) < 0.001)) {
            const double t = div_inrange(num, den);
            if (best > t && t > 0.0) { best = t; idx = k; type = HIT_PLANE; }
        }
    }
    t_out = best; idx_out = idx; type_out = type;
    RT_MARK(3);
}

template <bool GROUND = false>
__device__ __forceinline__ bool any_hit_masks(const Lds &lds, const KParams &p, const V3 &o, const V3 &d, int anchor, int self)
{
    const int P = plane_count<GROUND>(p);
    const int S = p.S;
    const lanemask live = lanes_where(true);
    lanemask occ;
    if (RT_DEFER_SHADOW != 0 && lds.defer) {
        const double e = unit_excess(d);
        const bool in_window = cull_reads_d(__builtin_amdgcn_ballot_w64(outside_unit_window(e)));
        RT_MARK(6);
        const int canchor = (opaque(p.anchors) > 0) ? anchor : -1;
        if (in_window) occ = any_spheres_masks<true>(lds, p, S, canchor, o, d, e, self, live);
        else occ = any_spheres_masks<false>(lds, p, S, canchor, o, d, e, self, live);
    } else {
    const V3 R = renormalize_unit(d);
    const double a = dot3(R, R);
    RT_MARK(6);
    const int canchor = (opaque(p.anchors) > 0) ? anchor : -1;
    const lanemask a_sane = lanes_where(a > 0.999999) & lanes_where(a < 1.000001);
    occ = 0ull;
    for (int k0 = 0; k0 < S; k0 += 64) {
      if (k0 > 0 && (live & ~occ) == 0ull) break;
      const int n = (S - k0 < 64) ? S - k0 : 64;
      unsigned long long mask = cull_mask(lds, S, canchor, k0, n, o, R, p.extent2, self);
      mask &= (n == 64) ? ~0ull : ((1ull << n) - 1ull);
      RT_MARK(7);
      while (mask) {
        const int k = k0 + __builtin_ctzll(mask);
        mask &= mask - 1ull;
        occ |= sphere_any_mask<false>(lds, k, o, R, a, a_sane);
        if (mask && (live & ~occ) == 0ull) break;
      }
      RT_MARK(8);
    }
    }
    const double *pl = lds.recs() + opaque(p.S) * SPH_STRIDE;
    for (int k = 0; k < P; ++k) {
        if ((live & ~occ) == 0ull) break;
        const double *g = pl + k * PL_STRIDE;
        double den, num;
        plane_den_num(g, plane_code<GROUND>(p, k), o, d, den, num, true);
        const double an = __builtin_fabs(num), ad = __builtin_fabs(den);
        int sx = (int)(__builtin_bit_cast(unsigned long long, num) >> 32) ^ (int)(__builtin_bit_cast(unsigned long long, den) >> 32);
        asm("" : "+v"(sx));
        const lanemask ahead = lanes_where(!(ad < 0.001)) & lanes_where(sx >= 0) & lanes_where(an > 0.0);
        const lanemask sure = lanes_where(an < 998.0 * ad);
        occ |= ahead & sure;
        const lanemask edge = ahead & ~sure & ~occ;
        if (edge != 0ull) {
            bool h = false;
            if (lane_of(edge) && !(an > 1000.0 * ad)) { const double t = num / den; h = 999.0 > t && t > 0.0; }
            occ |= lanes_where(h);
        }
    }
    RT_MARK(9);
    return lane_of(occ);
}

template <int MODE, bool GROUND = false>
__device__ __forceinline__ bool any_hit(const Lds &lds, const KParams &p, const V3 &o, const V3 &d, int anchor, int self, bool lanes = true)
{
    if (MODE == 0 && lds.trim) return any_hit_masks<GROUND>(lds, p, o, d, anchor, self);
    const int P = plane_count<GROUND>(p);
    const int S = p.S;
    const V3 R = renormalize_unit(d);
    const double a = dot3(R, R);
    RT_MARK(6);
    const bool a_sane = (a > 0.999999 && a < 1.000001);
    bool occ = false;
    const int canchor = (opaque(p.anchors) > 0) ? anchor : -1;
    if (MODE >= 2 && lds.NC > 0 && lanes) {
        occ = (canchor >= 0) ? lanes_any<true>(lds, p, canchor, o, R, a, self) : lanes_any<false>(lds, p, -1, o, R, a, self);
    } else
    for (int k0 = 0; k0 < S; k0 += 64) {
      if (k0 > 0 && __builtin_amdgcn_ballot_w64(!occ) == 0ull) break;
      const int n = (S - k0 < 64) ? S - k0 : 64;
      unsigned long long mask = cull_mask(lds, S, canchor, k0, n, o, R, p.extent2, self);
      mask &= (n == 64) ? ~0ull : ((1ull << n) - 1ull);
      RT_MARK(7);
      while (mask) {
        const int k = k0 + __builtin_ctzll(mask);
        mask &= mask - 1ull;
        if (!occ) occ = sphere_any<(MODE >= 1)>(lds, k, o, R, a, a_sane);
        if (mask && __builtin_amdgcn_ballot_w64(!occ) == 0ull) break;
      }
      RT_MARK(8);
    }
    const double *pl = lds.recs() + (MODE >= 1 ? 0 : opaque(p.S) * SPH_STRIDE);
    for (int k = 0; k < P; ++k) {
        if (!occ) {
            const double *g = pl + k * PL_STRIDE;
            double den, num;
            plane_den_num(g, plane_code<GROUND>(p, k), o, d, den, num);
            if (!(__builtin_fabs(den) < 0.001)) {
                const double an = __builtin_fabs(num), ad = __builtin_fabs(den);
                const bool same_sign = (num > 0.0 && den > 0.0) || (num < 0.0 && den < 0.0);
                if (same_sign) {
                    if (an < 998.0 * ad) occ = true;
                    else if (!(an > 1000.0 * ad)) { const double t = num / den; if (999.0 > t && t > 0.0) occ = true; }
                }
            }
        }
    }
    RT_MARK(9);
    return occ;
}

template <bool COUNT> struct RayCount {
    __device__ __forceinline__ void closest(bool) {}
    __device__ __forceinline__ void hit(bool) {}
    __device__ __forceinline__ void shadow(bool, bool) {}
};
template <> struct RayCount<true> {
    unsigned n_closest = 0, n_issued = 0, n_skipped = 0, n_hit = 0;
    __device__ __forceinline__ void closest(bool alive) { n_closest += alive ? 1u : 0u; }
    __device__ __forceinline__ void hit(bool alive) { n_hit += alive ? 1u : 0u; }
    __device__ __forceinline__ void shadow(bool alive, bool traced) { n_issued += (alive && traced) ? 1u : 0u; n_skipped += (alive && !traced) ? 1u : 0u; }
};

__device__ __forceinline__ V3 hash_unit3(unsigned key, unsigned t)
{
    return V3{hash_unit(key, t), hash_unit(key, t | 1u), hash_unit(key, t | 2u)};
}

__device__ __forceinline__ V3 soft_light_point(unsigned key, const double *g)
{
#pragma unroll 1
    for (int j = 0; j < 8; ++j) {
        const unsigned t = (unsigned)j << 2;
        const V3 c = hash_unit3(key, t);
        if (dot3(c, c) < 1.0) { const double rho = g[3]; return V3{g[0] + rho * c.x, g[1] + rho * c.y, g[2] + rho * c.z}; }
    }
    return V3{g[0], g[1], g[2]};
}

__device__ __forceinline__ V3 mirror_dir(const V3 &d, const V3 &N)
{
    const double c2 = -2.0 * dot3(d, N);
    return renormalize_unit(V3{d.x + c2 * N.x, d.y + c2 * N.y, d.z + c2 * N.z});
}

__device__ __forceinline__ V3 soft_light_dir(unsigned lkey, int b, int m, int i, const double *g, const V3 &Pt)
{
    const unsigned key = lkey ^ (((unsigned)b << 15) | ((unsigned)m << 9) | ((unsigned)i << 5));
    const V3 Q = soft_light_point(key, g);
    return normalize3(V3{Q.x - Pt.x, Q.y - Pt.y, Q.z - Pt.z});
}

template <int WGT, class MS>
__device__ __forceinline__ bool scatter_continue(const Lds &lds, const MS &ms, const V3 &N, int b, double rough, V3 &nd)
{
    const unsigned key = (unsigned)SLOT(KEY);
    const V3 R = nd;
    bool found = false;
    V3 q{0.0, 0.0, 0.0};
#pragma unroll 1
    for (int j = 0; j < 8 && !found; ++j) {
        const unsigned t = ((unsigned)b << 5) | ((unsigned)j << 2);
        const V3 c = hash_unit3(key, t);
        if (dot3(c, c) < 1.0) { q = c; found = true; }
    }
    if (found) nd = normalize3(V3{R.x + rough * q.x, R.y + rough * q.y, R.z + rough * q.z});
    const double sR = dot3(R, N), sD = dot3(nd, N);
    return (sR > 0.0 && sD > 0.0) || (sR < 0.0 && sD < 0.0);
}

template <int WGT, class MS>
__device__ __forceinline__ bool refract_continue(const Lds &lds, const MS &ms, const V3 &N, const V3 &Pt, V3 &o, V3 &d, int sb = -1)
{
    const double eta_slot = SLOT(ETA);
    V3 nd;
    bool from_q = false, reflect = true;
    if (eta_slot != 0.0) {
        const double c = dot3(d, N);
        const bool enter = c < 0.0;
        from_q = enter;
        if (eta_slot < 0.0) { nd = d; reflect = false; }
        else {
            const double eta = enter ? 1.0 / eta_slot : eta_slot;
            const double ci = enter ? -c : c;
            const double k = 1.0 - (eta * eta) * (1.0 - ci * ci);
            if (k >= 0.0) {
                const double cn = eta * ci - __builtin_sqrt(k);
                const V3 n = enter ? N : V3{-N.x, -N.y, -N.z};
                nd = renormalize_unit(V3{eta * d.x + cn * n.x, eta * d.y + cn * n.y, eta * d.z + cn * n.z});
                reflect = false;
            } else from_q = !enter;
        }
    }
    bool keep = true;
    if (reflect) {
        nd = mirror_dir(d, N);
        if constexpr (MS::scat) {
            const double rough = SLOT(ROUGH);
            if (rough > 0.0 && sb >= 0) keep = scatter_continue<WGT>(lds, ms, N, sb, rough, nd);
        }
    }
    V3 b = Pt;
    if (from_q) b = V3{SLOT(QX), SLOT(QY), SLOT(QZ)};
    o = V3{b.x + 0.0002 * nd.x, b.y + 0.0002 * nd.y, b.z + 0.0002 * nd.z};
    d = nd;
    return keep;
}

__host__ __device__ inline double texel_wrap(double g, double n, double rn)
{
    double f = __builtin_floor(g);
    f = f >= -0x1p30 ? f : -0x1p30;
    f = f > 0x1p30 - 1.0 ? 0x1p30 - 1.0 : f;
    double j = f - n * __builtin_floor(f * rn);
    if (j < 0.0) j += n;
    if (j >= n) j -= n;
    return j;
}
__device__ __forceinline__ unsigned texel_of(const KParams &p, int slot, const V3 &Pt)
{
    const int k = (int)p.lens.texels[4 * (size_t)slot + 3];
    unsigned ti = (unsigned)slot;
    if (k >= 0) {
        const double *r = p.scene + (size_t)p.lens.tex + 1 + TEX_STRIDE * k;
        const V3 dd{Pt.x - r[0], Pt.y - r[1], Pt.z - r[2]};
        const double j0 = texel_wrap(((dd.x * r[3]) + (dd.y * r[4])) + (dd.z * r[5]), r[12], r[15]);
        const double j1 = texel_wrap(((dd.x * r[6]) + (dd.y * r[7])) + (dd.z * r[8]), r[13], r[16]);
        const double j2 = texel_wrap(((dd.x * r[9]) + (dd.y * r[10])) + (dd.z * r[11]), r[14], r[17]);
        ti = (unsigned)(r[18] + ((j2 * r[13] + j1) * r[12] + j0));
    }
    return ti;
}

typedef __attribute__((address_space(4))) const double sky_f64;
typedef __attribute__((address_space(4))) const long long sky_i64;
__device__ __forceinline__ V3 sky_color(const double *block, const V3 &d)
{
    sky_f64 *k = (sky_f64 *)(size_t)block;
    const double h = dot3(d, V3{k[0], k[1], k[2]});
    const bool below = h < 0.0;
    const double a = below ? -h : h;
    double one = 1.0;
    asm volatile("" : "+s"(one));
    double t = a > 1.0 ? one : a;
    const int nsharp = (int)((sky_i64 *)k)[12];
    if (nsharp > 0) {
        double q = 1.0 - t;
#pragma unroll 1
        for (int i = 0; i < nsharp; ++i) q = q * q;
        t = 1.0 - q;
    }
    const double zx = k[6], zy = k[7], zz = k[8], nx = k[9], ny = k[10], nz = k[11];
    V3 g{k[3] + t * (below ? nx : zx), k[4] + t * (below ? ny : zy), k[5] + t * (below ? nz : zz)};
    const double s = dot3(d, V3{k[13], k[14], k[15]});
    if (s > 0.0) {
        double q = s;
        const int nhalo = (int)((sky_i64 *)k)[23];
#pragma unroll 1
        for (int i = 0; i < nhalo; ++i) q = q * q;
        g = V3{g.x + k[20] * q, g.y + k[21] * q, g.z + k[22] * q};
    }
    if (s >= k[16]) g = V3{g.x + k[17], g.y + k[18], g.z + k[19]};
    return g;
}

__device__ __forceinline__ int hit_slot(int type, int idx, int S) { return (type == HIT_SPHERE) ? idx : S + idx; }
template <bool NOREC> __device__ __forceinline__ int plane_base(int S) { return NOREC ? 0 : S * SPH_STRIDE; }
template <bool NOREC>
__device__ __forceinline__ void hit_normal(const Lds &lds, int type, int idx, int plb, const V3 &Pt, V3 &N, V3 &bN)
{
    if (type == HIT_SPHERE) {
        const SphHot g = sphere_hot<NOREC>(lds, idx);
        N = normalize3(V3{Pt.x - g.x, Pt.y - g.y, Pt.z - g.z});
        bN = V3{0.0002 * N.x, 0.0002 * N.y, 0.0002 * N.z};
    } else {
        const double *g = lds.recs() + plb + idx * PL_STRIDE;
        N = V3{g[6], g[7], g[8]};
        bN = V3{g[9], g[10], g[11]};
    }
}

template <bool PARK, int WGT, bool COUNT, int MODE, class MS, bool GROUND = false>
__device__ __forceinline__ void trace_bounce(const Lds &lds, const KParams &p, bool &alive, int anchor,
                                             V3 &o, V3 &d, V3 &rgb, RayCount<COUNT> &cnt, MS &ms, int b = 0)
{
    constexpr bool NOREC = MODE >= 1;
    constexpr bool FACING_SKIP = RT_FACING_SKIP != 0 && MODE != 2;
    const int S = p.S, P = p.P, L = opaque(p.L);
    rgb = V3{0.0, 0.0, 0.0};
    double t = 999.0; int idx = -1, type = HIT_NONE;
    cnt.closest(alive);
    RT_MARK(11);
    if (alive) closest_hit<MODE, GROUND>(lds, p, o, d, MS::lens ? -1 : anchor, t, idx, type);
    if constexpr (MS::sky) {
        if (alive && type == HIT_NONE) rgb = sky_color(p.scene + (size_t)p.lens.sky, d);
    }
    alive = alive && (type != HIT_NONE);
    cnt.hit(alive);
    if (alive) {
        V3 Pt{o.x + t * d.x, o.y + t * d.y, o.z + t * d.z};
        const int plb = plane_base<NOREC>(NOREC ? 0 : opaque(S));
        const int coff = (type == HIT_SPHERE) ? idx * SPH_STRIDE + 4 : plb + idx * PL_STRIDE + 12;
        volatile const lds_f64 *colp = (volatile const lds_f64 *)lds.recs() + coff;
        volatile const double *colf = (NOREC && type == HIT_SPHERE) ? p.scene + coff : lds.recs() + coff;
        typedef __attribute__((address_space(3))) float lds_f32;
        volatile const lds_f32 *col1 = nullptr;
        if constexpr (MODE == 1) col1 = (volatile const lds_f32 *)lds.col32 + 4 * ((type == HIT_SPHERE) ? idx : (int)padS(S, lds.NC) + idx);
        unsigned texi = 0u;
        if constexpr (MS::tex) texi = texel_of(p, hit_slot(type, idx, S), Pt);
        auto texel = [&](int c) -> double { return (double)((volatile const float *)p.lens.texels)[4 * (size_t)texi + c]; };
        V3 colr{0.0, 0.0, 0.0};
        if constexpr (!PARK && MS::tex) {
            const f4 tc = reinterpret_cast<const f4 *>(p.lens.texels)[texi];
            colr = V3{(double)tc[0], (double)tc[1], (double)tc[2]};
        }
        else if constexpr (!PARK) colr = (MODE == 1) ? V3{(double)col1[0], (double)col1[1], (double)col1[2]} : V3{colf[0], colf[1], colf[2]};
        auto col = [&](int c) -> double {
            if constexpr (PARK && MS::tex) return texel(c);
            else if constexpr (PARK && MODE == 1) return (double)col1[c];
            else if constexpr (PARK && NOREC) return colf[c];
            else if constexpr (PARK) return colp[c];
            else return c == 0 ? colr.x : (c == 1 ? colr.y : colr.z);
        };
        auto lambert_add = [&](double k, const V3 &e) {
            rgb = V3{rgb.x + (k * e.x) * col(0), rgb.y + (k * e.y) * col(1), rgb.z + (k * e.z) * col(2)};
        };
        volatile const lds_f64 *mp = nullptr;
        V3 N, bN;
        hit_normal<NOREC>(lds, type, idx, plb, Pt, N, bN);
        if constexpr (MS::mat) {
            mp = ms.entry((type == HIT_SPHERE) ? idx : S + idx);
            SLOT(LAMB) = mp[1];
            if constexpr (MS::refr) {
                const double tr = mp[3];
                const bool glass = tr > 0.0;
                SLOT(REFL) = glass ? tr : mp[2];
                SLOT(ETA) = glass ? ((type == HIT_SPHERE) ? mp[4] : -1.0) : 0.0;
                if (glass) {
                    SLOT(QX) = Pt.x - bN.x;
                    SLOT(QY) = Pt.y - bN.y;
                    SLOT(QZ) = Pt.z - bN.z;
                }
                if constexpr (MS::scat) SLOT(ROUGH) = mp[5];
            } else
            SLOT(REFL) = mp[2];
            const double amb = mp[0];
            rgb = V3{0.0 + amb * col(0), 0.0 + amb * col(1), 0.0 + amb * col(2)};
        } else
        rgb = V3{p.amb * col(0), p.amb * col(1), p.amb * col(2)};
        Pt = V3{Pt.x + bN.x, Pt.y + bN.y, Pt.z + bN.z};
        const int self = (type == HIT_SPHERE) ? idx : -1;
        Park3<PARK, WGT, MODE == 3> dpark(lds.acc, 1, lds.wave);
        dpark.set(d);
        RT_MARK(4);

        const double *lt = lds.recs() + plb + opaque(P) * PL_STRIDE;
        if constexpr (MS::lit) {
        const unsigned lslot = (unsigned)(hit_slot(type, idx, S));
        auto lit_row = [&]() { return (volatile const double *)(p.scene + (size_t)p.lens.lit + (size_t)LT_STRIDE * L) + 2 * (size_t)lslot; };
        auto again = [](int m) { asm volatile("" : "+v"(m)); return m; };
        auto point_Ld = [&](int m) {
            const double *g = lt + m * LT_STRIDE;
            return normalize3(V3{g[0] - Pt.x, g[1] - Pt.y, g[2] - Pt.z});
        };
        auto soft_Ld = [&](int m, int i) { return soft_light_dir((unsigned)SLOT(LKEY), b, m, i, lt + m * LT_STRIDE, Pt); };
        auto lit_add = [&](int m, double k, auto &&form_Ld) {
            const double *e = p.scene + (size_t)p.lens.lit + LT_STRIDE * m;
            const double er = e[0], eg = e[1], eb = e[2];
            if (k > 0.0) lambert_add(k, V3{er, eg, eb});
            volatile const double *lr = lit_row();
            const double spec = lr[0];
            if (spec > 0.0) {
              const V3 Ld = form_Ld();
              if (dot3(Ld, N) > 0.0) {
                const V3 dd = dpark.get();
                const V3 H = normalize3(V3{Ld.x - dd.x, Ld.y - dd.y, Ld.z - dd.z});
                const double s = dot3(N, H);
                if (s > 0.0) {
                    double q = s;
                    const int nsq = (int)lr[1];
#pragma unroll 1
                    for (int i = 0; i < nsq; ++i) q = q * q;
                    const double a = spec * q;
                    rgb = V3{rgb.x + a * er, rgb.y + a * eg, rgb.z + a * eb};
                }
              }
            }
        };
        for (int m = 0; m < L; ++m) {
            if constexpr (MS::soft) {
#pragma unroll 1
                for (int i = 0; i < ms.nsh; ++i) {
                    const V3 Ld = soft_Ld(m, i);
                    const double cN = dot3(Ld, N);
                    const double k = SLOT(LAMB) * cN;
                    RT_MARK(5);
                    if (k > 0.0 || (lit_row()[0] > 0.0 && cN > 0.0)) {
                        const bool occluded = any_hit<MODE, GROUND>(lds, p, Pt, Ld, -1, self, true);
                        if (!occluded) lit_add(m, k, [&]() { return soft_Ld(again(m), i); });
                    }
                }
            } else {
                if constexpr (FACING_SKIP) {
                    const double *g = lt + m * LT_STRIDE;
                    const bool cert = rt_facing_certified_lamb(g[0] - Pt.x, g[1] - Pt.y, g[2] - Pt.z, N.x, N.y, N.z, p.facing_tau,
                                                               SLOT(LAMB));
                    if (__builtin_amdgcn_ballot_w64(!cert) == 0ull) { RT_MARK(5); continue; }
                }
                const V3 Ld = point_Ld(m);
                const double cN = dot3(Ld, N);
                const double k = SLOT(LAMB) * cN;
                RT_MARK(5);
                if (k > 0.0 || (lit_row()[0] > 0.0 && cN > 0.0)) {
                    const bool occluded = any_hit<MODE, GROUND>(lds, p, Pt, Ld, 1 + m, self, anchor != 0 || p.lanes_primary);
                    if (!occluded) lit_add(m, k, [&]() { return point_Ld(again(m)); });
                }
            }
        }
        } else
        if constexpr (MS::soft) {
        for (int m = 0; m < L; ++m) {
            const double *g = lt + m * LT_STRIDE;
#pragma unroll 1
            for (int i = 0; i < ms.nsh; ++i) {
                const V3 Ld = soft_light_dir((unsigned)SLOT(LKEY), b, m, i, g, Pt);
                const double k = SLOT(LAMB) * dot3(Ld, N);
                RT_MARK(5);
                if (k > 0.0) {
                    const bool occluded = any_hit<MODE, GROUND>(lds, p, Pt, Ld, -1, self, true);
                    if (!occluded) lambert_add(k, V3{1.0, 1.0, 1.0});
                }
            }
        }
        } else
        for (int m = 0; m < L; ++m) {
            const double *g = lt + m * LT_STRIDE;
            const V3 v{g[0] - Pt.x, g[1] - Pt.y, g[2] - Pt.z};
            double lamb;
            if constexpr (MS::mat) lamb = SLOT(LAMB); else lamb = p.lamb;
            if constexpr (FACING_SKIP) {
                bool cert;
                if constexpr (MS::mat) cert = rt_facing_certified_lamb(v.x, v.y, v.z, N.x, N.y, N.z, p.facing_tau, lamb);
                else cert = rt_facing_certified(v.x, v.y, v.z, N.x, N.y, N.z, p.facing_tau);
                if (__builtin_amdgcn_ballot_w64(!cert) == 0ull) {
                    cnt.shadow(true, false);
                    RT_MARK(5);
                    continue;
                }
            }
            const V3 Ld = normalize3(v);
            const double k = lamb * dot3(Ld, N);
            cnt.shadow(true, k > 0.0);
            RT_MARK(5);
            if (k > 0.0) {
                const bool occluded = any_hit<MODE, GROUND>(lds, p, Pt, Ld, 1 + m, self, anchor != 0 || p.lanes_primary);
                if (!occluded) lambert_add(k, V3{1.0, 1.0, 1.0});
            }
        }
        d = dpark.get();
        if constexpr (MS::scat) {
            alive = refract_continue<WGT>(lds, ms, N, Pt, o, d, b < p.depth ? b : -1);
        } else if constexpr (MS::refr) {
            refract_continue<WGT>(lds, ms, N, Pt, o, d);
        } else {
        const V3 Rd = mirror_dir(d, N);
        o = V3{Pt.x + 0.0002 * Rd.x, Pt.y + 0.0002 * Rd.y, Pt.z + 0.0002 * Rd.z};
        d = Rd;
        }
        RT_MARK(10);
    }
}


template <bool PARK, int WGT, bool COUNT, int MODE, class MS, bool GROUND = false>
__device__ __forceinline__ V3 sample(const Lds &lds, const KParams &p, bool alive, V3 o, V3 d, RayCount<COUNT> &cnt, MS &ms,
                                     unsigned key = 0u, unsigned lkey = 0u)
{
    Park3<PARK, WGT, MODE == 3> acc(lds.acc, 0, lds.wave);
    acc.set(V3{0.0, 0.0, 0.0});
    if constexpr (MS::mat) SLOT(W) = 1.0;
    if constexpr (MS::scat) SLOT(KEY) = (double)key;
    if constexpr (MS::soft) SLOT(LKEY) = (double)lkey;
    for (int b = 0; b <= p.depth; ++b) {
        if (__builtin_amdgcn_ballot_w64(alive) == 0ull) break;
        if constexpr (COUNT) {
            const unsigned long long am = __builtin_amdgcn_ballot_w64(alive);
            if ((threadIdx.x & 63u) == 0u && p.ray_counts) {
                atomicAdd(&p.ray_counts[4 + 2 * b], 1ull);
                atomicAdd(&p.ray_counts[5 + 2 * b], (unsigned long long)__builtin_popcountll(am));
            }
        }
        V3 rgb;
#ifdef RT_REGION_STATS
        ((volatile unsigned *)lds.reg)[(threadIdx.x >> 6) * 32 + 30] = b >= 2 ? 12u : 0u;
#endif
        trace_bounce<PARK, WGT, COUNT, MODE, MS, GROUND>(lds, p, alive, b == 0 ? 0 : -1, o, d, rgb, cnt, ms, b);
        if (b == 0) acc.set(rgb);
        else {
            double wgt;
            if constexpr (MS::mat) wgt = SLOT(W); else wgt = p.refl_pow[b - 1];
            const V3 a = acc.get();
            acc.set(V3{a.x + wgt * rgb.x, a.y + wgt * rgb.y, a.z + wgt * rgb.z});
        }
        if constexpr (MS::mat) {
            if (alive) {
                volatile lds_f64 *w = &SLOT(W);
                *w = *w * SLOT(REFL);
            }
        }
    }
    return acc.get();
}

__device__ __forceinline__ V3 pixel_P(const KParams &p, int x, int y)
{
    if (p.pixel_loc) {
        const size_t wh = (size_t)p.w * p.h, o = (size_t)x * p.h + y;
        return V3{p.pixel_loc[o], p.pixel_loc[wh + o], p.pixel_loc[2 * wh + o]};
    }
    return V3{p.px, (double)x * p.dy + p.y0, (double)y * p.dz + p.z0};
}

__device__ __forceinline__ V3 lattice_P(const KParams &p, int i, int j)
{
    const double ya = (double)(i >> 1) * p.dy + p.y0, yb = (double)((i + 1) >> 1) * p.dy + p.y0;
    const double za = (double)(j >> 1) * p.dz + p.z0, zb = (double)((j + 1) >> 1) * p.dz + p.z0;
    return V3{p.px, (i & 1) ? 0.5 * ya + 0.5 * yb : ya, (j & 1) ? 0.5 * za + 0.5 * zb : za};
}

__device__ __forceinline__ V3 primary_dir(const KParams &p, const V3 &P)
{
    const V3 v{p.cam_R[0] * P.x + p.cam_R[1] * P.y + p.cam_R[2] * P.z,
               p.cam_R[3] * P.x + p.cam_R[4] * P.y + p.cam_R[5] * P.z,
               p.cam_R[6] * P.x + p.cam_R[7] * P.y + p.cam_R[8] * P.z};
    return normalize3(v);
}

__device__ __forceinline__ void lens_ray(const KParams &p, unsigned x, unsigned y, unsigned s, const V3 &P, V3 &o, V3 &d)
{
    const V3 v{p.cam_R[0] * P.x + p.cam_R[1] * P.y + p.cam_R[2] * P.z,
               p.cam_R[3] * P.x + p.cam_R[4] * P.y + p.cam_R[5] * P.z,
               p.cam_R[6] * P.x + p.cam_R[7] * P.y + p.cam_R[8] * P.z};
    const double t = p.lens.focus / P.x;
    const V3 F{p.cam_o[0] + t * v.x, p.cam_o[1] + t * v.y, p.cam_o[2] + t * v.z};
    const unsigned key = lens_key(x, y, s, p.seed);
    double u0 = 0.0, u1 = 0.0;
#pragma unroll 1
    for (int j = 0; j < 8; ++j) {
        const unsigned tj = (unsigned)j << 1;
        const double c0 = hash_unit(key, tj);
        const double c1 = hash_unit(key, tj | 1u);
        if (c0 * c0 + c1 * c1 < 1.0) { u0 = c0; u1 = c1; break; }
    }
    const double a0 = p.lens.aperture * u0, a1 = p.lens.aperture * u1;
    o = V3{(p.cam_o[0] + a0 * p.cam_R[1]) + a1 * p.cam_R[2], (p.cam_o[1] + a0 * p.cam_R[4]) + a1 * p.cam_R[5],
           (p.cam_o[2] + a0 * p.cam_R[7]) + a1 * p.cam_R[8]};
    d = normalize3(V3{F.x - o.x, F.y - o.y, F.z - o.z});
}

__device__ __forceinline__ void store_pixel(const KParams &p, long long off, long long fo, double R, double G, double B)
{
    if (p.out_u8) {
        const uint8_t r8 = clip_color(R), g8 = clip_color(G), b8 = clip_color(B);
        const uint8_t c1 = p.u8_rgb ? g8 : b8, c2 = p.u8_rgb ? b8 : g8;
        uint8_t *o8 = p.out_u8 + fo;
        if (p.u8_hwc) {
            const long long xr = off / p.h, yy = off - xr * p.h;
            uint8_t *px = o8 + (yy * p.plane_stride + xr) * 3;
            px[0] = r8; px[1] = c1; px[2] = c2;
        } else {
            o8[off] = r8;
            o8[p.plane_stride + off] = c1;
            o8[2 * p.plane_stride + off] = c2;
        }
    }
    if (p.out_f32) {
        float *o32 = p.out_f32 + fo;
        o32[off] = (float)R;
        o32[p.plane_stride + off] = (float)G;
        o32[2 * p.plane_stride + off] = (float)B;
    }
}

__global__ __launch_bounds__(TABLE_THREADS) void tables_kernel(const KParams p, float *__restrict__ out)
{
    const int nrec = (int)lds_doubles(p.S, p.P, p.L);
    const int Sp = padS(p.S, p.NC), NCp = pad4(p.NC);
    const TableLayout tl = table_layout(p.S, p.NC, p.anchors, p.P);
    float *sph32 = out;
    float *tab = out + tl.tab;
    float *csph32 = out + tl.csph32;
    float *ctab = out + tl.ctab;
    const double *rec = p.scene;
    const float NINF = -__builtin_inff();
    for (int k = threadIdx.x; k < Sp; k += TABLE_THREADS) {
        const double *g = rec + k * SPH_STRIDE;
        const bool real = k < p.S;
        sph32[4 * k + 0] = real ? (float)g[0] : 0.0f; sph32[4 * k + 1] = real ? (float)g[1] : 0.0f;
        sph32[4 * k + 2] = real ? (float)g[2] : 0.0f; sph32[4 * k + 3] = real ? (float)g[3] : NINF;
    }
    float *col32 = out + tl.col32;
    for (int k = threadIdx.x; k < Sp + pad4(p.P); k += TABLE_THREADS) {
        const double *g = k < p.S ? rec + k * SPH_STRIDE + 4 : rec + p.S * SPH_STRIDE + (k - Sp) * PL_STRIDE + 12;
        const bool real = k < p.S || (k >= Sp && k - Sp < p.P);
        for (int c = 0; c < 3; ++c) col32[4 * k + c] = real ? (float)g[c] : 0.0f;
        col32[4 * k + 3] = 0.0f;
    }
    const double *lt = rec + p.S * SPH_STRIDE + p.P * PL_STRIDE;
    for (int e = threadIdx.x; e < p.anchors * Sp; e += TABLE_THREADS) {
        const int a = e / Sp, k = e - a * Sp;
        float *t = tab + (size_t)e * CULL_STRIDE;
        if (k >= p.S) { t[0] = t[1] = t[2] = 0.0f; t[3] = -NINF; continue; }
        const double *g = rec + k * SPH_STRIDE;
        const double ax = a ? lt[(a - 1) * LT_STRIDE + 0] : p.cam_o[0];
        const double ay = a ? lt[(a - 1) * LT_STRIDE + 1] : p.cam_o[1];
        const double az = a ? lt[(a - 1) * LT_STRIDE + 2] : p.cam_o[2];
        const double lx = ax - g[0], ly = ay - g[1], lz = az - g[2];
        const double ll = lx * lx + ly * ly + lz * lz;
        t[0] = (float)lx; t[1] = (float)ly; t[2] = (float)lz;
        t[3] = anchored_tau(ll, g[3], p.floor_anch);
    }
    const double *cl = rec + nrec;
    for (int c = threadIdx.x; c < NCp; c += TABLE_THREADS) {
        const bool real = c < p.NC;
        const double *g = cl + (real ? c : 0) * CL_STRIDE;
        csph32[4 * c + 0] = real ? (float)g[0] : 0.0f; csph32[4 * c + 1] = real ? (float)g[1] : 0.0f;
        csph32[4 * c + 2] = real ? (float)g[2] : 0.0f;
        csph32[4 * c + 3] = real ? (float)(g[3] * (1.0 + 0x1p-20)) : NINF;
    }
    for (int e = threadIdx.x; e < p.anchors * NCp; e += TABLE_THREADS) {
        const int a = e / NCp, c = e - a * NCp;
        float *t = ctab + (size_t)e * CULL_STRIDE;
        if (c >= p.NC) { t[0] = t[1] = t[2] = 0.0f; t[3] = -NINF; continue; }
        const double *g = cl + c * CL_STRIDE;
        const double ax = a ? lt[(a - 1) * LT_STRIDE + 0] : p.cam_o[0];
        const double ay = a ? lt[(a - 1) * LT_STRIDE + 1] : p.cam_o[1];
        const double az = a ? lt[(a - 1) * LT_STRIDE + 2] : p.cam_o[2];
        const double lx = ax - g[0], ly = ay - g[1], lz = az - g[2];
        const double ll = lx * lx + ly * ly + lz * lz;
        t[0] = (float)lx; t[1] = (float)ly; t[2] = (float)lz;
        t[3] = anchored_tau(ll, g[3], p.floor_anch);
    }
    float *cbox = out + tl.cbox;
    for (int c = threadIdx.x; c < NCp; c += TABLE_THREADS) {
        double lo[3] = {1e30, 1e30, 1e30}, hi[3] = {-1e30, -1e30, -1e30};
        for (int k = c * CLUSTER; k < (c + 1) * CLUSTER && k < p.S; ++k) {
            const double *g = rec + k * SPH_STRIDE;
            const double rad = __builtin_sqrt(g[3]) * (1.0 + 0x1p-20) + 1e-30;
            for (int i = 0; i < 3; ++i) { lo[i] = __builtin_fmin(lo[i], g[i] - rad); hi[i] = __builtin_fmax(hi[i], g[i] + rad); }
        }
        float *b = cbox + (size_t)c * BOX_STRIDE;
        for (int i = 0; i < 3; ++i) {
            b[i] = (float)(lo[i] - (__builtin_fabs(lo[i]) * 0x1p-22 + 1e-30));
            b[4 + i] = (float)(hi[i] + (__builtin_fabs(hi[i]) * 0x1p-22 + 1e-30));
        }
        b[3] = 0.0f; b[7] = 0.0f;
    }
    __syncthreads();
    for (int g = threadIdx.x; g < supers(p.NC); g += TABLE_THREADS) {
        float *b = out + tl.gbox + (size_t)g * BOX_STRIDE;
        for (int i = 0; i < 3; ++i) { b[i] = __builtin_inff(); b[4 + i] = -__builtin_inff(); }
        for (int c = g * SUPER; c < (g + 1) * SUPER && c < p.NC; ++c)
            for (int i = 0; i < 3; ++i) {
                b[i] = __builtin_fminf(b[i], cbox[(size_t)c * BOX_STRIDE + i]);
                b[4 + i] = __builtin_fmaxf(b[4 + i], cbox[(size_t)c * BOX_STRIDE + 4 + i]);
            }
        b[3] = 0.0f; b[7] = 0.0f;
    }
    const int NG = supers(p.NC), NGp = pad4(NG);
    const double *gr = cl + (size_t)p.NC * CL_STRIDE;
    for (int e = threadIdx.x; e < p.anchors * NGp; e += TABLE_THREADS) {
        const int a = e / NGp, g = e - a * NGp;
        float *t = out + tl.gtab + (size_t)e * CULL_STRIDE;
        if (g >= NG) { t[0] = t[1] = t[2] = 0.0f; t[3] = -NINF; continue; }
        const double *c = gr + g * CL_STRIDE;
        const double ax = a ? lt[(a - 1) * LT_STRIDE + 0] : p.cam_o[0];
        const double ay = a ? lt[(a - 1) * LT_STRIDE + 1] : p.cam_o[1];
        const double az = a ? lt[(a - 1) * LT_STRIDE + 2] : p.cam_o[2];
        const double lx = ax - c[0], ly = ay - c[1], lz = az - c[2];
        const double ll = lx * lx + ly * ly + lz * lz;
        t[0] = (float)lx; t[1] = (float)ly; t[2] = (float)lz;
        t[3] = anchored_tau(ll, c[3], p.floor_anch);
    }
}

template <Family F, int WSLOT, bool FRESH>
__device__ __forceinline__ MatState<F, WSLOT, FRESH> mat_state(double *matl, int M, int nsh = 1)
{
    typedef __attribute__((address_space(3))) double lds_d;
    typedef MatState<F, WSLOT, FRESH> MS;
    if constexpr (MS::mat) return MS{(unsigned)(size_t)(lds_d *)(matl + 1), (unsigned)(size_t)(lds_d *)(matl + 1 + MS::COLS * M), nsh};
    else return {};
}

__device__ __forceinline__ void tile_xy(const KParams &p, int tile, int &tx, int &ty)
{
    tx = div_by(tile, p.tiles_y, p.tiles_y_magic, p.tiles_y_shift);
    ty = tile - tx * p.tiles_y;
}

template <bool AA, bool PARK, int WPW, bool COUNT = false, bool LAT = false, int MODE = 0, Family F = Family::PLAIN, bool GROUND = false>
__global__ __launch_bounds__(64 * WPW, MODE >= 2 ? RT_W_LANES : (AA ? (PARK ? RT_W_AAPARK : 4) : (PARK ? RT_W_PARK : 5))) void render_kernel(const KParams p)
{
    constexpr int WG_THREADS = 64 * WPW, WAVES_PER_WG = WPW;
    constexpr bool M2 = MODE >= 2;
    constexpr bool NOREC = MODE >= 1;
    constexpr bool MAT = has_mat(F), SCAT = has_scat(F), SOFT = has_soft(F), LENS = has_lens(F), TEX = has_tex(F);
    const int nrec = (int)lds_doubles(NOREC ? 0 : p.S, p.P, p.L);
    const double *rec_src = p.scene + (NOREC ? (size_t)p.S * SPH_STRIDE : 0);
    double *accum = lds_raw + nrec;
    int *offw = reinterpret_cast<int *>(accum + lds_slots(AA, PARK, M2, F) * WG_THREADS);
    float *sph32 = reinterpret_cast<float *>(offw + lds_offset_words(PARK, WG_THREADS));
    const TableLayout tl = table_layout(p.S, p.NC, p.anchors, p.P);
    const bool LANES = MODE >= 2 && p.anchors > 0;
    float *tab = sph32 + tl.tab;
    float *csph32 = LANES ? nullptr : sph32 + tl.csph32;
    float *ctab = sph32 + tl.ctab;
    float *cbox = sph32 + tl.cbox;
    const size_t ntab = MODE == 1 ? tl.total_col : (LANES ? tl.total_lanes : tl.total);
    unsigned *wgstat = reinterpret_cast<unsigned *>(sph32 + ntab);
    if (threadIdx.x == 0) { wgstat[0] = 0u; wgstat[1] = 0u; }
    {
        for (int i = threadIdx.x; i < nrec; i += WG_THREADS) lds_raw[i] = rec_src[i];
        const int nf4 = (int)(ntab / 4);
        const f4 *src = reinterpret_cast<const f4 *>(p.ftab);
        f4 *dst = reinterpret_cast<f4 *>(sph32);
        for (int i = threadIdx.x; i < nf4; i += WG_THREADS) dst[i] = src[i];
    }
#ifdef RT_REGION_STATS
    double *matl = reinterpret_cast<double *>(wgstat + 4 + WPW * 32);
#else
    double *matl = reinterpret_cast<double *>(wgstat + 4);
#endif
    int nmat = 0, nsh = 1;
    if constexpr (MAT) {
        const double *msrc = p.scene + ((LENS || TEX) ? (size_t)p.lens.mat : mat_offset(p.S, p.P, p.L, p.NC));
        nmat = (int)msrc[0];
        const int nm = (int)mat_doubles(nmat, p.S, p.P, F);
        for (int i = threadIdx.x; i < nm; i += WG_THREADS) matl[i] = msrc[i];
        if constexpr (SOFT) nsh = (int)msrc[nm - 1];
    }
    __syncthreads();
#ifdef RT_REGION_STATS
    const Lds lds{sph32, tab, csph32, ctab, cbox, sph32 + tl.gbox, sph32 + tl.gtab, MODE == 1 ? sph32 + tl.col32 : nullptr, WPW == 2 ? 0 : p.NC, __builtin_amdgcn_readfirstlane((int)(threadIdx.x >> 6)), MODE < 2, MODE >= 2, WPW == 2 && !MAT, RT_DEFER_DIRECTION != 0 && MODE < 2 && !(AA && PARK), wgstat + 4, accum};
    for (int i = threadIdx.x & 63; i < 32; i += 64) lds.reg[(threadIdx.x >> 6) * 32 + i] = 0u;
    if ((threadIdx.x & 63) == 0) lds.reg[(threadIdx.x >> 6) * 32 + 31] = (unsigned)__builtin_amdgcn_s_memtime();
#else
    const Lds lds{sph32, tab, csph32, ctab, cbox, sph32 + tl.gbox, sph32 + tl.gtab, MODE == 1 ? sph32 + tl.col32 : nullptr, WPW == 2 ? 0 : p.NC, __builtin_amdgcn_readfirstlane((int)(threadIdx.x >> 6)), MODE < 2, MODE >= 2, WPW == 2 && !MAT, RT_DEFER_DIRECTION != 0 && MODE < 2 && !(AA && PARK), accum};
#endif

    const int wave = threadIdx.x >> 6, lane = threadIdx.x & 63;
    int bid = (int)blockIdx.x;
    const unsigned *ord = p.order;
    if (p.nframes > 1) {
        const int frame = div_by(bid, p.bpf, p.bpf_magic, p.bpf_shift);
        bid -= frame * p.bpf;
        if (ord && frame < p.nframes - 1) ord += p.seq_offset;
    }
    const bool by_tile = WPW >= TILE_ORDER_MIN_WPW && p.order_tiles;
    const int block = by_tile ? bid : (ord ? (int)ord[bid] : bid);
    const int wave_u = __builtin_amdgcn_readfirstlane(wave);
    const int tile_v = by_tile ? (ord ? (int)ord[bid * WAVES_PER_WG + wave_u] : bid * WAVES_PER_WG + wave_u) : block * WAVES_PER_WG + wave;
    const int tile = WPW >= TILE_ORDER_MIN_WPW ? __builtin_amdgcn_readfirstlane(tile_v) : tile_v;
    if (tile >= p.ntiles) return;
    const unsigned long long t_begin = (p.tile_cycles || p.cost) ? __builtin_amdgcn_s_memtime() : 0ull;
    int tx, ty;
    tile_xy(p, tile, tx, ty);
    const int x = p.x0 + tx * TILE + (lane >> 3);
    const int y = ty * TILE + (lane & 7);
    bool inb = (x < p.x1) && (y < p.h);
    if constexpr (LAT) inb = inb && ((((x | y) & 1) == 0) || (x >= 1 && x <= p.w - 2 && y >= 1 && y <= p.h - 2));
    const int xc = inb ? x : p.x0, yc = inb ? y : 0;
    typedef __attribute__((address_space(3))) int lds_i32;
    constexpr bool OFF_REMAT = PARK && MODE == 3;
    volatile lds_i32 *offp = OFF_REMAT ? nullptr : (volatile lds_i32 *)offw + threadIdx.x;
    if constexpr (PARK && !OFF_REMAT) *offp = inb ? (x - p.x0) * p.h + y : -1;

    const V3 o{p.cam_o[0], p.cam_o[1], p.cam_o[2]};
    RayCount<COUNT> cnt;
    constexpr int WSLOT = lds_slots(AA, PARK, M2, Family::PLAIN);
    auto ms = mat_state<F, WSLOT, !PARK || MODE == 3>(matl, nmat, nsh);
    const unsigned sseed = SCAT ? p.seed : 0u;
    double R, G, B;
    if constexpr (!AA) {
        unsigned key = 0u, lkey = 0u;
        if constexpr (SCAT) key = LAT ? scatter_key((unsigned)xc, (unsigned)yc, 0u, sseed) : scatter_key(2u * xc, 2u * yc, 0u, sseed);
        if constexpr (SOFT) lkey = LAT ? soft_key((unsigned)xc, (unsigned)yc, 0u, sseed) : soft_key(2u * xc, 2u * yc, 0u, sseed);
        const V3 P0 = LAT ? lattice_P(p, xc, yc) : pixel_P(p, xc, yc);
        V3 ro = o, rd;
        if constexpr (LENS) lens_ray(p, LAT ? (unsigned)xc : 2u * xc, LAT ? (unsigned)yc : 2u * yc, 0u, P0, ro, rd);
        else rd = primary_dir(p, P0);
        const V3 c = sample<PARK, WG_THREADS, COUNT, MODE, decltype(ms), GROUND>(lds, p, inb, ro, rd, cnt, ms, key, lkey);
        R = c.x; G = c.y; B = c.z;
    } else {
        const bool stoch = (p.aa == 2);
        const bool interior = !stoch && inb && x >= 1 && x <= p.w - 2 && y >= 1 && y <= p.h - 2;
        const int ntaps = stoch ? p.spp : ((__builtin_amdgcn_ballot_w64(interior) != 0ull) ? 9 : 1);
        constexpr unsigned NBX = 0x8858u, NBY = 0x0A25u;
        Park3<PARK && !M2, WG_THREADS> taps(lds.acc, 2);
#pragma unroll 1
        for (int tap = 0; tap < ntaps; ++tap) {
            const V3 Pp = pixel_P(p, xc, yc);
            V3 Pt = Pp;
            unsigned key = 0u, lkey = 0u;
            unsigned lx = 2u * xc, ly = 2u * yc;
            if constexpr (SCAT) key = scatter_key(2u * xc, 2u * yc, stoch ? (unsigned)tap : 0u, sseed);
            if constexpr (SOFT) lkey = soft_key(2u * xc, 2u * yc, stoch ? (unsigned)tap : 0u, sseed);
            if (stoch) {
                const unsigned hh = jitter_hash((unsigned)xc, (unsigned)yc, (unsigned)tap, p.seed);
                const double u = (double)(hh & 0xFFFFu) * 0x1p-16 + (0x1p-17 - 0.5);
                const double v = (double)(hh >> 16) * 0x1p-16 + (0x1p-17 - 0.5);
                Pt = V3{Pp.x, Pp.y + u * p.dy, Pp.z + v * p.dz};
            } else if (tap) {
                const int k = tap - 1;
                const int ddx = (int)((NBX >> (2 * k)) & 3u) - 1, ddy = (int)((NBY >> (2 * k)) & 3u) - 1;
                const V3 Pn = pixel_P(p, interior ? x + ddx : xc, interior ? y + ddy : yc);
                Pt = V3{0.5 * Pp.x + 0.5 * Pn.x, 0.5 * Pp.y + 0.5 * Pn.y, 0.5 * Pp.z + 0.5 * Pn.z};
                if constexpr (SCAT) key = scatter_key((unsigned)(2 * xc + ddx), (unsigned)(2 * yc + ddy), 0u, sseed);
                if constexpr (SOFT) lkey = soft_key((unsigned)(2 * xc + ddx), (unsigned)(2 * yc + ddy), 0u, sseed);
                if constexpr (LENS) { lx = (unsigned)(2 * xc + ddx); ly = (unsigned)(2 * yc + ddy); }
            }
            V3 ro = o, rd;
            if constexpr (LENS) lens_ray(p, lx, ly, stoch ? (unsigned)tap : 0u, Pt, ro, rd);
            else rd = primary_dir(p, Pt);
            const V3 s = sample<PARK, WG_THREADS, COUNT, MODE, decltype(ms), GROUND>(lds, p, (tap && !stoch) ? interior : inb, ro, rd, cnt, ms, key, lkey);
            if (tap == 0) taps.set(s);
            else if (stoch) { const V3 a = taps.get(); taps.set(V3{a.x + s.x, a.y + s.y, a.z + s.z}); }
            else if (interior) { const V3 a = taps.get(); taps.set(V3{a.x + s.x, a.y + s.z, a.z + s.y}); }
        }
        { const V3 a = taps.get(); R = a.x; G = a.y; B = a.z; }
        if (stoch) { const double n = (double)p.spp; R = R / n; G = G / n; B = B / n; }
        else if (interior) { R = R / 9; G = G / 9; B = B / 9; }
    }

    long long off;
    if constexpr (OFF_REMAT) {
        const int l2 = (int)fresh_lane();
        const int x2 = p.x0 + tx * TILE + (l2 >> 3), y2 = ty * TILE + (l2 & 7);
        bool inb2 = (x2 < p.x1) && (y2 < p.h);
        if constexpr (LAT) inb2 = inb2 && ((((x2 | y2) & 1) == 0) || (x2 >= 1 && x2 <= p.w - 2 && y2 >= 1 && y2 <= p.h - 2));
        off = inb2 ? (long long)((x2 - p.x0) * p.h + y2) : -1ll;
    } else if constexpr (PARK) off = *offp; else off = inb ? (long long)(x - p.x0) * p.h + y : -1ll;
    if (off >= 0) {
        if constexpr (LAT) {
            double *q = p.out_f64 + off * 3;
            q[0] = R; q[1] = G; q[2] = B;
        } else {
            const long long fo = opaque(p.nframes) > 1 ? (long long)div_by((int)blockIdx.x, p.bpf, p.bpf_magic, p.bpf_shift) * p.frame_stride : 0ll;
            store_pixel(p, off, fo, R, G, B);
        }
    }
#ifdef RT_REGION_STATS
    RT_MARK(11);
    if (p.tile_cycles && (threadIdx.x & 63) < 24)
        atomicAdd(p.tile_cycles + p.ntiles + 16 + (threadIdx.x & 63), lds.reg[(threadIdx.x >> 6) * 32 + (threadIdx.x & 63)] >> 6);
#endif
    if constexpr (COUNT) {
        unsigned v[4] = {cnt.n_closest, cnt.n_issued, cnt.n_skipped, cnt.n_hit};
#pragma unroll
        for (int c = 0; c < 4; ++c) {
#pragma unroll
            for (int d = 32; d >= 1; d >>= 1) v[c] += __shfl_down(v[c], d);
            if ((threadIdx.x & 63) == 0 && p.ray_counts) atomicAdd(&p.ray_counts[c], (unsigned long long)v[c]);
        }
    }
    if ((p.tile_cycles || p.cost) && (threadIdx.x & 63) == 0) {
        const unsigned cyc = (unsigned)(__builtin_amdgcn_s_memtime() - t_begin);
        if (p.tile_cycles) p.tile_cycles[tile] = cyc;
        if (p.cost) {
            if (by_tile) p.cost[tile] = cyc >> 2;
            else {
                const int expected = (p.ntiles - block * WAVES_PER_WG < WAVES_PER_WG) ? p.ntiles - block * WAVES_PER_WG : WAVES_PER_WG;
                atomicAdd(&wgstat[0], cyc >> 2);
                if ((int)atomicAdd(&wgstat[1], 1u) == expected - 1) p.cost[block] = atomicAdd(&wgstat[0], 0u);
            }
        }
    }
}

__global__ __launch_bounds__(256) void aa_resolve_kernel(const KParams p)
{
    const long long idx = (long long)blockIdx.x * 256 + threadIdx.x;
    if (idx >= (long long)(p.x1 - p.x0) * p.h) return;
    const int xr = (int)(idx / p.h), y = (int)(idx - (long long)xr * p.h), x = p.x0 + xr;
    const double *c = p.out_f64 + ((size_t)(2 * x - p.lat_x0) * p.lat_h + 2 * y) * 3;
    double R = c[0], G = c[1], B = c[2];
    if (x >= 1 && x <= p.w - 2 && y >= 1 && y <= p.h - 2) {
        constexpr unsigned NBX = 0x8858u, NBY = 0x0A25u;
#pragma unroll
        for (int k = 0; k < 8; ++k) {
            const int ddx = (int)((NBX >> (2 * k)) & 3u) - 1, ddy = (int)((NBY >> (2 * k)) & 3u) - 1;
            const double *s = c + ((long long)ddx * p.lat_h + ddy) * 3;
            R += s[0]; G += s[2]; B += s[1];
        }
        R = R / 9; G = G / 9; B = B / 9;
    }
    store_pixel(p, idx, 0ll, R, G, B);
}

__global__ __launch_bounds__(ORDER_THREADS) void order_kernel(const unsigned *__restrict__ cost, unsigned *__restrict__ gtmp,
                                                               unsigned *__restrict__ btmp, unsigned *__restrict__ order, int nblocks, int gshift,
                                                               int wshift, int nvalid)
{
    const unsigned wm = (1u << wshift) - 1u;
    auto place = [&](unsigned x, unsigned t, unsigned tail_) -> unsigned {
        return x < (unsigned)ORDER_XCDS ? ((((unsigned)ORDER_XCDS * (t >> wshift) + x) << wshift) | (t & wm)) : tail_ + t;
    };
    auto cost_of = [&](int it) -> unsigned { return it < nvalid ? cost[it] : 0u; };
    __shared__ unsigned hist[(ORDER_XCDS + 1) * ORDER_BUCKETS];
    __shared__ unsigned scan[ORDER_THREADS / 64];
    static_assert(ORDER_THREADS == ORDER_BUCKETS, "thread i owns bucket 1023 - i");
    const int i = threadIdx.x, lane = i & 63, wv = i >> 6;
    const int gb = 1 << gshift;
    const int full = nblocks >> gshift;
    const int rows = full / ORDER_XCDS;
    auto scan_classes = [&](int nc) {
        for (int c = 0; c < nc; ++c) {
            __syncthreads();
            const unsigned v = hist[c * ORDER_BUCKETS + ORDER_BUCKETS - 1 - i];
            unsigned incl = v;
#pragma unroll
            for (int d = 1; d < 64; d <<= 1) {
                const unsigned up = __shfl_up(incl, d);
                if (lane >= d) incl += up;
            }
            if (lane == 63) scan[wv] = incl;
            __syncthreads();
            unsigned base = 0;
            for (int w = 0; w < wv; ++w) base += scan[w];
            hist[c * ORDER_BUCKETS + ORDER_BUCKETS - 1 - i] = base + incl - v;
        }
        __syncthreads();
    };
    for (int k = i; k < (ORDER_XCDS + 1) * ORDER_BUCKETS; k += ORDER_THREADS) hist[k] = 0u;
    __syncthreads();
    for (int g = i; g < full; g += ORDER_THREADS) {
        unsigned long long sum = 0;
        for (int k = 0; k < gb; ++k) sum += cost_of((g << gshift) + k);
        const unsigned mean = (unsigned)(sum >> gshift);
        const int bkt = order_bucket(mean);
        gtmp[g] = ((unsigned)bkt << 20) | atomicAdd(&hist[bkt], 1u);
    }
    scan_classes(1);
    for (int g = i; g < full; g += ORDER_THREADS) {
        const unsigned s = gtmp[g];
        const int r = (int)(hist[s >> 20] + (s & 0xFFFFFu));
        const int q = r / ORDER_XCDS, c = r - q * ORDER_XCDS;
        gtmp[g] = q < rows ? (unsigned)((q & 1) ? ORDER_XCDS - 1 - c : c) : (unsigned)ORDER_XCDS;
    }
    __syncthreads();
    const unsigned tail = (unsigned)(ORDER_XCDS * rows * gb);
    {
        unsigned *seq = order + nblocks;
        const int per = (full + ORDER_THREADS - 1) / ORDER_THREADS;
        const int g0 = i * per < full ? i * per : full, g1 = g0 + per < full ? g0 + per : full;
        unsigned base[ORDER_XCDS + 1];
        for (int c = 0; c <= ORDER_XCDS; ++c) {
            unsigned v = 0;
            for (int g = g0; g < g1; ++g) v += gtmp[g] == (unsigned)c ? 1u : 0u;
            unsigned incl = v;
#pragma unroll
            for (int d = 1; d < 64; d <<= 1) {
                const unsigned up = __shfl_up(incl, d);
                if (lane >= d) incl += up;
            }
            __syncthreads();
            if (lane == 63) scan[wv] = incl;
            __syncthreads();
            unsigned b0 = 0;
            for (int w = 0; w < wv; ++w) b0 += scan[w];
            base[c] = b0 + incl - v;
        }
        for (int g = g0; g < g1; ++g) {
            const unsigned c = gtmp[g];
            unsigned jg = 0;
#pragma unroll
            for (int cc = 0; cc <= ORDER_XCDS; ++cc) if (c == (unsigned)cc) jg = base[cc]++;
            for (int k = 0; k < gb; ++k) {
                const unsigned j = jg * (unsigned)gb + (unsigned)k;
                seq[place(c, j, tail)] = (unsigned)((g << gshift) + k);
            }
        }
        for (int b = (full << gshift) + i; b < nblocks; b += ORDER_THREADS) seq[b] = (unsigned)b;
    }
    __syncthreads();
    for (int k = i; k < (ORDER_XCDS + 1) * ORDER_BUCKETS; k += ORDER_THREADS) hist[k] = 0u;
    __syncthreads();
    for (int b = i; b < nblocks; b += ORDER_THREADS) {
        const int g = b >> gshift;
        const unsigned x = g < full ? gtmp[g] : (unsigned)ORDER_XCDS;
        const int bkt = order_bucket(cost_of(b));
        btmp[b] = ((unsigned)bkt << 22) | atomicAdd(&hist[x * ORDER_BUCKETS + bkt], 1u);
    }
    scan_classes(ORDER_XCDS + 1);
    for (int b = i; b < nblocks; b += ORDER_THREADS) {
        const int g = b >> gshift;
        const unsigned s = btmp[b], x = g < full ? gtmp[g] : (unsigned)ORDER_XCDS;
        const unsigned j = hist[x * ORDER_BUCKETS + (s >> 22)] + (s & 0x3FFFFFu);
        order[place(x, j, tail)] = (unsigned)b;
    }
}

}
```

### python-ray-tracer_amd/csrc/rt_plan.h

```cpp
#pragma once
#include "rt_layout.h"
#include "rt_scene.h"
#include "rt_geometry.h"

#include <algorithm>
#include <cstddef>

namespace rt {

struct PlanKnobs {
    int lanes_min_spheres = 161;
    int f32_records = 1;
    size_t wpw2_max_image = 4608;
    int lanes_park = 1;
    int order_group = -1;
    int order_tiles = 1;
    int seq_order = -1;
    int ground_plane = 1;
};

inline Family family_of(const SceneLayout &s, double lens_a)
{
    using F = Family;
    const bool lens = lens_a > 0.0, soft = s.soft_n > 0;
    if (s.M <= 0) return F::PLAIN;
    if (s.sky)
        return lens ? (soft ? F::SKY_LENS_SOFT : F::SKY_LENS) : (soft ? F::SKY_SOFT : F::SKY_SCAT);
    if (s.lit)
        return lens ? (soft ? F::LIT_LENS_SOFT : F::LIT_LENS) : (soft ? F::LIT_SOFT : F::LIT_SCAT);
    if (s.T > 0)
        return lens ? (soft ? F::TEX_LENS_SOFT : F::TEX_LENS) : (soft ? F::TEX_SOFT : F::TEX_SCAT);
    if (lens) return soft ? F::LENS_SOFT : F::LENS;
    return block_family(s.M, s.mat_cols, soft);
}

struct Shape {
    bool aa, park;
    int wpw;
    bool count, lat;
    int mode;
    constexpr bool operator==(const Shape &o) const
    {
        return aa == o.aa && park == o.park && wpw == o.wpw && count == o.count && lat == o.lat && mode == o.mode;
    }
};

constexpr Shape SHAPES[] = {
    {false, false, 2, false, false, 0}, {false, true, 2, false, false, 0}, {true, false, 2, false, false, 0}, {true, true, 2, false, false, 0},
    {false, false, 4, false, false, 0}, {false, true, 4, false, false, 0}, {true, false, 4, false, false, 0}, {true, true, 4, false, false, 0},
    {false, false, 4, false, false, 1}, {false, true, 4, false, false, 1},
    {false, false, 2, false, true, 0}, {false, true, 2, false, true, 0}, {false, false, 4, false, true, 0}, {false, true, 4, false, true, 0},
    {false, false, 4, false, true, 1}, {false, true, 4, false, true, 1},
    {false, false, 4, false, false, 2}, {false, true, 4, false, false, 2}, {true, false, 4, false, false, 2}, {true, true, 4, false, false, 3},
    {false, false, 4, false, true, 2}, {false, true, 4, false, true, 2},
    {false, false, 4, true, false, 0}, {true, false, 4, true, false, 0}, {false, false, 4, true, true, 0},
};
constexpr int NSHAPES = sizeof SHAPES / sizeof SHAPES[0];

constexpr bool has_kernel(Family f, const Shape &s)
{
    return (!s.count || f == Family::PLAIN) && !(has_refr(f) && s.park && s.mode < 2);
}

constexpr Shape NO_GROUND_TWIN[] = {
    {false, false, 2, false, false, 0}, {true, false, 2, false, false, 0},
    {false, false, 4, false, false, 1}, {false, false, 4, false, true, 1},
    {false, false, 4, false, false, 2}, {false, false, 4, false, true, 2},
};
constexpr bool has_ground_kernel(Family f, const Shape &s)
{
    if (f != Family::PLAIN || s.count) return false;
    for (const Shape &n : NO_GROUND_TWIN)
        if (n == s) return false;
    return true;
}

inline bool ground_plane(const SceneLayout &lay, const PlanKnobs &kn, Family fam, int flags)
{
    const int code0 = (int)(signed char)(lay.plane_codes & 0xffu);
    return kn.ground_plane != 0 && fam == Family::PLAIN && !(flags & RT_FLAG_COUNT_RAYS) && lay.P == 1 && code0 == 3;
}

constexpr int PARK_WAVES = 24;
constexpr size_t CU_LDS = 160 * 1024;

constexpr bool missing_kernels_never_park()
{
    for (int fi = 0; fi < FAMILIES; ++fi)
        for (const Shape &s : SHAPES) {
            const Family f = (Family)fi;
            if (s.count || has_kernel(f, s)) continue;
            const size_t wgt = 64 * s.wpw;
            const size_t least = lds_slots(s.aa, true, s.mode >= 2, f) * wgt * sizeof(double) +
                                 wgt * sizeof(int) + 16;
            if (!s.park || s.mode >= 2 || least * (PARK_WAVES / s.wpw) <= CU_LDS) return false;
        }
    return true;
}
static_assert(missing_kernels_never_park(), "the parking rule can pick a render kernel that is not compiled");

inline int anchors_of(const SceneLayout &lay)
{
    const size_t table = (size_t)(lay.L + 1) * (padS(lay.S, lay.NC) + pad4(lay.NC)) * CULL_STRIDE * sizeof(float);
    return (table <= (size_t)MAX_CULL_TABLE_BYTES) ? lay.L + 1 : 0;
}

inline size_t lds_bytes(const SceneLayout &lay, int anchors, Family f, const Shape &s)
{
    const bool lanes = s.mode >= 2;
    return lds_bytes(lay.S, lay.P, lay.L, lay.NC, anchors, s.aa, s.park, 64 * s.wpw, lanes && anchors > 0, lanes, s.mode == 1, f, lay.M);
}

struct LaunchPlan {
    Family family;
    Shape shape;
    int index;
    size_t lds;
};

inline LaunchPlan plan_launch(const SceneLayout &lay, const PlanKnobs &kn, double lens_a, bool aa, int flags, bool lattice, int anchors)
{
    const Family fam = family_of(lay, lens_a);
    const bool count = (flags & RT_FLAG_COUNT_RAYS) != 0;
    const size_t image = lds_doubles(lay.S, lay.P, lay.L) * sizeof(double) + table_floats(lay.S, lay.NC, anchors) * sizeof(float);
    const bool lanes = lay.NC > 0 && lay.S >= kn.lanes_min_spheres && !count && !(flags & RT_FLAG_NO_BUNDLES);
    const int wpw = (image <= kn.wpw2_max_image && !count && lay.NC == 0) ? 2 : 4;
    auto bytes = [&](bool park, int mode) { return lds_bytes(lay, anchors, fam, Shape{aa, park, wpw, count, lattice, mode}); };
    auto per_cu = [&](int mode) {
        const size_t lp = bytes(true, mode);
        if (lp * 6 <= CU_LDS) return (int)std::min<size_t>(7, CU_LDS / lp);
        return (int)std::min<size_t>(5, CU_LDS / bytes(false, mode));
    };
    const bool norec = !lanes && !count && !aa && wpw == 4 && kn.f32_records && per_cu(1) > per_cu(0);
    const int mode = lanes ? 2 : (norec ? 1 : 0);
    const size_t lds_park = bytes(true, mode);
    const bool park = !count && (lanes ? (lds_park * RT_W_LANES <= CU_LDS && kn.lanes_park) : lds_park * (PARK_WAVES / wpw) <= CU_LDS);
    LaunchPlan pl;
    pl.family = fam;
    pl.shape = Shape{aa, park, wpw, count, lattice, lanes && aa && park ? 3 : mode};
    pl.lds = park ? lds_park : bytes(false, mode);
    pl.index = -1;
    for (int i = 0; i < NSHAPES; ++i)
        if (SHAPES[i] == pl.shape) pl.index = i;
    return pl;
}

struct GuidesPlan {
    int mode;
    size_t lds;
};

inline GuidesPlan plan_guides(const SceneLayout &lay, const PlanKnobs &kn, int anchors)
{
    SceneLayout l = lay;
    l.M = 0; l.soft_n = 0; l.T = 0; l.lit = false; l.sky = false;
    const LaunchPlan pl = plan_launch(l, kn, 0.0, false, 0, false, anchors);
    GuidesPlan g;
    g.mode = pl.shape.mode >= 2 ? 2 : pl.shape.mode;
    g.lds = lds_bytes(l, anchors, Family::PLAIN, Shape{false, false, 4, false, false, g.mode});
    return g;
}

struct OrderShape {
    bool feedback;
    int gshift;
    int wshift;
    bool otiles;
    unsigned items;
    int code;
    int seq_offset;
};

inline OrderShape order_shape(const LaunchPlan &pl, const PlanKnobs &kn, int flags, const rt_geo_plan &g)
{
    const int wpw = pl.shape.wpw;
    const unsigned grid = (unsigned)g.blocks;
    OrderShape o;
    o.feedback = !(flags & RT_FLAG_NO_FEEDBACK) && grid > 1 && grid < (1u << 20);
    o.gshift = kn.order_group >= 0 ? kn.order_group : (wpw == 2 ? 3 : 2);
    o.otiles = wpw >= TILE_ORDER_MIN_WPW && kn.order_tiles && o.feedback;
    o.wshift = wpw == 4 ? 2 : 1;
    o.items = o.otiles ? grid * (unsigned)wpw : grid;
    o.code = wpw + (pl.shape.mode >= 2 ? 32 : 0) + (o.otiles ? 64 : 0);
    o.seq_offset = (kn.seq_order < 0 ? wpw == 2 : kn.seq_order != 0) ? (int)o.items : 0;
    return o;
}

}
```

Before: 227,300.

## Add small-scene kernel twins specialized for up to eight spheres in cull groups

Adds render kernel variants templated on a compile-time number of four-sphere cull groups, selected when the scene has a ground plane, no clusters and at most eight spheres. Culling then runs over a fixed unrolled set of groups into a 32-bit mask, with no 64-sphere chunk loop, and the closest-hit and shadow loops iterate over that mask directly. This targets loop, mask and branching overhead for the small benchmark scene. In exchange it adds more kernel instantiations, which increases binary size and compile time, and a separate LDS-limit bookkeeping path.

```diff
diff --git a/python-ray-tracer_amd/csrc/mi355rt.hip b/python-ray-tracer_amd/csrc/mi355rt.hip
--- a/python-ray-tracer_amd/csrc/mi355rt.hip
+++ b/python-ray-tracer_amd/csrc/mi355rt.hip
@@ -87,6 +87,7 @@
     rt::View view;
     size_t lds_limit_set[rt::FAMILIES] = {};
     size_t ground_lds_set = 0;
+    size_t small_lds_set[rt::SMALL_MAX_GROUPS] = {};
     size_t guides_lds_set = 0;
     unsigned *tile_stats = nullptr;
     struct Feedback : rt::FeedbackSlot {
@@ -170,14 +171,14 @@
     return RT_OK;
 }
 
-using rt::Shape; using rt::SHAPES; using rt::NSHAPES; using rt::has_kernel; using rt::has_ground_kernel;
-
-template <rt::Family F, int I, bool GROUND = false>
+using rt::Shape; using rt::SHAPES; using rt::NSHAPES; using rt::has_kernel; using rt::has_ground_kernel; using rt::has_small_kernel;
+
+template <rt::Family F, int I, bool GROUND = false, int NG = 0>
 const void *kernel_at()
 {
     constexpr Shape s = SHAPES[I];
-    if constexpr (GROUND ? has_ground_kernel(F, s) : has_kernel(F, s))
-        return (const void *)rt::render_kernel<s.aa, s.park, s.wpw, s.count, s.lat, s.mode, F, GROUND>;
+    if constexpr (NG > 0 ? has_small_kernel(F, s) : (GROUND ? has_ground_kernel(F, s) : has_kernel(F, s)))
+        return (const void *)rt::render_kernel<s.aa, s.park, s.wpw, s.count, s.lat, s.mode, F, GROUND, NG>;
     else
         return nullptr;
 }
@@ -190,6 +191,11 @@
 std::array<const void *, NSHAPES> ground_kernels(std::integer_sequence<int, I...>)
 {
     return {kernel_at<rt::Family::PLAIN, I, true>()...};
+}
+template <int NG, int... I>
+std::array<const void *, NSHAPES> small_kernels(std::integer_sequence<int, I...>)
+{
+    return {kernel_at<rt::Family::PLAIN, I, true, NG>()...};
 }
 
 constexpr std::make_integer_sequence<int, NSHAPES> ALL_SHAPES{};
@@ -206,7 +212,18 @@
     family_kernels<rt::Family::SKY_LENS>(ALL_SHAPES), family_kernels<rt::Family::SKY_LENS_SOFT>(ALL_SHAPES),
 };
 const std::array<const void *, NSHAPES> GROUND_KERNELS = ground_kernels(ALL_SHAPES);
-const std::array<const void *, NSHAPES> &kernels_of(int fi, bool ground) { return ground ? GROUND_KERNELS : KERNELS[fi]; }
+const std::array<const void *, NSHAPES> SMALL_KERNELS[rt::SMALL_MAX_GROUPS] = {small_kernels<1>(ALL_SHAPES), small_kernels<2>(ALL_SHAPES)};
+static_assert(rt::SMALL_MAX_GROUPS == 2, "SMALL_KERNELS lists the twins of every number of cull groups");
+const std::array<const void *, NSHAPES> &kernels_of(int fi, bool ground, int ng = 0)
+{
+    return ng > 0 ? SMALL_KERNELS[ng - 1] : (ground ? GROUND_KERNELS : KERNELS[fi]);
+}
+const void *kernel_of_shape(const std::array<const void *, NSHAPES> &kernels, const Shape &s)
+{
+    for (int i = 0; i < NSHAPES; ++i)
+        if (SHAPES[i] == s) return kernels[i];
+    return nullptr;
+}
 static_assert(rt::FAMILIES == 19 && (int)rt::Family::TEX_LENS_SOFT == 10 && (int)rt::Family::LIT_LENS_SOFT == 14 &&
               (int)rt::Family::SKY_SCAT == 15 && (int)rt::Family::SKY_LENS_SOFT == 18,
               "KERNELS lists the families in enum order");
@@ -365,14 +382,17 @@
     const Shape &sh = plan.shape;
     const int fi = (int)plan.family;
     const bool ground = rt::ground_plane(ctx->lay, ctx->knobs, plan.family, sh.count ? RT_FLAG_COUNT_RAYS : 0) && has_ground_kernel(plan.family, sh);
-    const std::array<const void *, NSHAPES> &kernels = kernels_of(fi, ground);
+    const int ng = has_small_kernel(plan.family, sh) ? rt::cull_groups(ctx->lay, ctx->knobs, plan.family, sh.count ? RT_FLAG_COUNT_RAYS : 0, k.anchors) : 0;
+    const std::array<const void *, NSHAPES> &kernels = kernels_of(fi, ground, ng);
     const void *fn = kernels[plan.index];
     if (!fn) return fail(ctx, RT_ERR_STATE, "no render kernel for this launch");
     const unsigned grid = (unsigned)g.blocks;
     if (ctx->log_kernels)
         std::fprintf(stderr, "mi355rt: render_kernel<%d, %d, %d, %d, %d, %d, (rt::Family)%d>%s\n", (int)sh.aa, (int)sh.park, sh.wpw, (int)sh.count,
                      (int)sh.lat, sh.mode, fi, ground ? " ground" : "");
-    int rc = raise_lds(ctx, kernels.data(), kernels.size(), plan.lds, ground ? ctx->ground_lds_set : ctx->lds_limit_set[fi]);
+    if (ctx->log_kernels && ng > 0) std::fprintf(stderr, "mi355rt: cull groups %d\n", ng);
+    int rc = raise_lds(ctx, kernels.data(), kernels.size(), plan.lds,
+                       ng > 0 ? ctx->small_lds_set[ng - 1] : (ground ? ctx->ground_lds_set : ctx->lds_limit_set[fi]));
     if (rc != RT_OK) return rc;
     if (sh.count) {
         if (!ctx->counts.p) {
@@ -475,6 +495,7 @@
     if (const char *e = std::getenv("MI355RT_ORDER_TILES")) ctx->knobs.order_tiles = std::atoi(e) != 0;
     if (const char *e = std::getenv("MI355RT_LANES_PARK")) ctx->knobs.lanes_park = std::atoi(e) != 0;
     if (const char *e = std::getenv("MI355RT_GROUND_PLANE")) ctx->knobs.ground_plane = std::atoi(e) != 0;
+    if (const char *e = std::getenv("MI355RT_SMALL_SCENE")) ctx->knobs.small_scene = std::atoi(e) != 0;
     if (const char *e = std::getenv("MI355RT_LOG_KERNELS")) ctx->log_kernels = std::atoi(e) != 0;
     if (const char *e = std::getenv("MI355RT_SEQ_ORDER")) ctx->knobs.seq_order = std::atoi(e) != 0 ? 1 : 0;
     if (const char *e = std::getenv("MI355RT_CHUNKS")) { const int v = std::atoi(e); if (v >= 1 && v <= RT_RENDER_CHUNKS) ctx->render_chunks = v; }
@@ -1256,7 +1277,11 @@
     RT_HIP(ctx, hipSetDevice(ctx->device));
     hipFuncAttributes a;
     const bool ground = ctx->have_scene && rt::ground_plane(ctx->lay, ctx->knobs, rt::Family::PLAIN, 0);
-    const void *fn = ground ? (const void *)rt::render_kernel<false, true, 2, false, false, 0, rt::Family::PLAIN, true>
+    constexpr Shape headline{false, true, 2, false, false, 0};
+    const int ng = ground && has_small_kernel(rt::Family::PLAIN, headline)
+                       ? rt::cull_groups(ctx->lay, ctx->knobs, rt::Family::PLAIN, 0, rt::anchors_of(ctx->lay)) : 0;
+    const void *fn = ng > 0 ? kernel_of_shape(SMALL_KERNELS[ng - 1], headline)
+                   : ground ? (const void *)rt::render_kernel<false, true, 2, false, false, 0, rt::Family::PLAIN, true>
                             : (const void *)rt::render_kernel<false, true, 2>;
     RT_HIP(ctx, hipFuncGetAttributes(&a, fn));
     hipDeviceProp_t prop;
diff --git a/python-ray-tracer_amd/csrc/rt_device.h b/python-ray-tracer_amd/csrc/rt_device.h
--- a/python-ray-tracer_amd/csrc/rt_device.h
+++ b/python-ray-tracer_amd/csrc/rt_device.h
@@ -279,10 +279,18 @@
     return acc;
 }
 
-template <bool ANCH, bool SELF>
+template <bool ANCH, bool SELF, int NG = 0>
 __device__ __forceinline__ unsigned long long cull_mask_t(const Lds &lds, int S, int anchor, int k0, int n,
                                                           const RayF &q, int selfj)
 {
+    if constexpr (NG > 0) {
+        lds_cf4 *sbase = pin_lds(ANCH ? lds.tab + (size_t)anchor * (4 * NG) * CULL_STRIDE : lds.sph32);
+        unsigned m = 0u;
+#pragma unroll
+        for (int g = NG - 1; g >= 0; --g)
+            m = lds.pairs ? cull4<ANCH, SELF, true>(sbase + 4 * g, q, selfj - 4 * g, m) : cull4<ANCH, SELF, false>(sbase + 4 * g, q, selfj - 4 * g, m);
+        return m;
+    }
     unsigned long long mask = 0ull;
     const int Sp = padS(S, lds.NC);
     lds_cf4 *sbase = pin_lds(ANCH ? lds.tab + ((size_t)anchor * Sp + k0) * CULL_STRIDE : lds.sph32 + 4 * k0);
@@ -312,29 +320,31 @@
     return mask;
 }
 
+template <int NG = 0>
 __device__ __forceinline__ unsigned long long cull_mask(const Lds &lds, int S, int anchor, int k0, int n,
                                                         const V3 &o, const F3 &dir, float extent2, int self)
 {
     RayF q = make_rayf_dir(dir);
     if (anchor >= 0) {
-        const bool cand = self >= k0 && self < k0 + n;
+        const bool cand = NG > 0 ? self >= 0 : (self >= k0 && self < k0 + n);
         if (__builtin_amdgcn_ballot_w64(cand) != 0ull) {
             add_origin(q, o, extent2);
             const float *cs = lds.sph32 + 4 * self;
             const bool self_culled = cand ? cull_origin(f4{cs[0], cs[1], cs[2], cs[3]}, q) : false;
             if (__builtin_amdgcn_ballot_w64(self_culled) != 0ull)
-                return cull_mask_t<true, true>(lds, S, anchor, k0, n, q, self_culled ? self - k0 : -1);
-        }
-        return cull_mask_t<true, false>(lds, S, anchor, k0, n, q, -1);
+                return cull_mask_t<true, true, NG>(lds, S, anchor, k0, n, q, self_culled ? self - k0 : -1);
+        }
+        return cull_mask_t<true, false, NG>(lds, S, anchor, k0, n, q, -1);
     }
     add_origin(q, o, extent2);
-    return cull_mask_t<false, false>(lds, S, anchor, k0, n, q, -1);
-}
-
+    return cull_mask_t<false, false, NG>(lds, S, anchor, k0, n, q, -1);
+}
+
+template <int NG = 0>
 __device__ __forceinline__ unsigned long long cull_mask(const Lds &lds, int S, int anchor, int k0, int n,
                                                         const V3 &o, const V3 &R, float extent2, int self)
 {
-    return cull_mask(lds, S, anchor, k0, n, o, cull_dir32(R), extent2, self);
+    return cull_mask<NG>(lds, S, anchor, k0, n, o, cull_dir32(R), extent2, self);
 }
 
 
@@ -648,13 +658,30 @@
     asm volatile("" : "+v"(x));
     return x;
 }
-template <bool F32, bool IN_WINDOW>
+__device__ __forceinline__ unsigned small_mask(unsigned long long m, int S) { return (unsigned)m & ((1u << S) - 1u); }
+
+template <bool F32, bool IN_WINDOW, int NG = 0>
 __device__ __forceinline__ double closest_spheres(const Lds &lds, const KParams &p, int S, int canchor, const V3 &o, const V3 &d, double e,
                                                   double &bestn, int &bidx)
 {
     double a = 1.0;
     V3 Rg{0.0, 0.0, 0.0};
     if constexpr (!IN_WINDOW) { Rg = normalize3_generic(d); a = dot3(Rg, Rg); }
+    if constexpr (NG > 0) {
+      unsigned mask = small_mask(cull_mask<NG>(lds, S, canchor, 0, S, o, cull_dir32(IN_WINDOW ? d : Rg), p.extent2, -1), S);
+      RT_MARK(1);
+      if (mask) {
+        V3 R = Rg;
+        if constexpr (IN_WINDOW) { R = renormalize_unit_fast(d, pinned_here(e)); a = dot3(R, R); }
+        do {
+          const int k = __builtin_ctz(mask);
+          mask &= mask - 1u;
+          sphere_closest<F32>(lds, p, k, o, R, a, bestn, bidx);
+        } while (mask);
+      }
+      RT_MARK(2);
+      return a;
+    }
     for (int k0 = 0; k0 < S; k0 += 64) {
       const int n = (S - k0 < 64) ? S - k0 : 64;
       unsigned long long mask = cull_mask(lds, S, canchor, k0, n, o, cull_dir32(IN_WINDOW ? d : Rg), p.extent2, -1);
@@ -673,13 +700,31 @@
     }
     return a;
 }
-template <bool IN_WINDOW>
+template <bool IN_WINDOW, int NG = 0>
 __device__ __forceinline__ lanemask any_spheres_masks(const Lds &lds, const KParams &p, int S, int canchor, const V3 &o, const V3 &d, double e,
                                                       int self, lanemask live)
 {
     lanemask occ = 0ull;
     V3 Rg{0.0, 0.0, 0.0};
     if constexpr (!IN_WINDOW) Rg = normalize3_generic(d);
+    if constexpr (NG > 0) {
+      unsigned mask = small_mask(cull_mask<NG>(lds, S, canchor, 0, S, o, cull_dir32(IN_WINDOW ? d : Rg), p.extent2, self), S);
+      RT_MARK(7);
+      if (mask) {
+        V3 R = Rg;
+        if constexpr (IN_WINDOW) R = renormalize_unit_fast(d, pinned_here(e));
+        const double a = dot3(R, R);
+        const lanemask a_sane = lanes_where(a > 0.999999) & lanes_where(a < 1.000001);
+        do {
+          const int k = __builtin_ctz(mask);
+          mask &= mask - 1u;
+          occ |= sphere_any_mask<false>(lds, k, o, R, a, a_sane);
+          if (mask && (live & ~occ) == 0ull) break;
+        } while (mask);
+      }
+      RT_MARK(8);
+      return occ;
+    }
     for (int k0 = 0; k0 < S; k0 += 64) {
       if (k0 > 0 && (live & ~occ) == 0ull) break;
       const int n = (S - k0 < 64) ? S - k0 : 64;
@@ -703,7 +748,7 @@
     return occ;
 }
 
-template <int MODE, bool GROUND = false>
+template <int MODE, bool GROUND = false, int NG = 0>
 __device__ __forceinline__ void closest_hit(const Lds &lds, const KParams &p, const V3 &o, const V3 &d, int anchor,
                                             double &t_out, int &idx_out, int &type_out)
 {
@@ -717,17 +762,26 @@
         const double e = unit_excess(d);
         const bool in_window = cull_reads_d(__builtin_amdgcn_ballot_w64(outside_unit_window(e)));
         RT_MARK(0);
-        const int canchor = (opaque(p.anchors) > 0) ? anchor : -1;
-        if (in_window) aq = closest_spheres<F32, true>(lds, p, S, canchor, o, d, e, bestn, bidx);
-        else aq = closest_spheres<F32, false>(lds, p, S, canchor, o, d, e, bestn, bidx);
+        const int canchor = (NG > 0 || opaque(p.anchors) > 0) ? anchor : -1;
+        if (in_window) aq = closest_spheres<F32, true, NG>(lds, p, S, canchor, o, d, e, bestn, bidx);
+        else aq = closest_spheres<F32, false, NG>(lds, p, S, canchor, o, d, e, bestn, bidx);
     } else {
     const V3 R = renormalize_unit(d);
     const double a = dot3(R, R);
     RT_MARK(0);
-    const int canchor = (opaque(p.anchors) > 0) ? anchor : -1;
+    const int canchor = (NG > 0 || opaque(p.anchors) > 0) ? anchor : -1;
     if (MODE >= 2 && lds.NC > 0 && (canchor < 0 || p.lanes_primary)) {
         if (canchor >= 0) lanes_closest<true>(lds, p, canchor, o, R, a, bestn, bidx);
         else lanes_closest<false>(lds, p, -1, o, R, a, bestn, bidx);
+    } else if constexpr (NG > 0) {
+      unsigned mask = small_mask(cull_mask<NG>(lds, S, canchor, 0, S, o, R, p.extent2, -1), S);
+      RT_MARK(1);
+      while (mask) {
+        const int k = __builtin_ctz(mask);
+        mask &= mask - 1u;
+        sphere_closest<F32>(lds, p, k, o, R, a, bestn, bidx);
+      }
+      RT_MARK(2);
     } else
     for (int k0 = 0; k0 < S; k0 += 64) {
       const int n = (S - k0 < 64) ? S - k0 : 64;
@@ -763,7 +817,7 @@
     RT_MARK(3);
 }
 
-template <bool GROUND = false>
+template <bool GROUND = false, int NG = 0>
 __device__ __forceinline__ bool any_hit_masks(const Lds &lds, const KParams &p, const V3 &o, const V3 &d, int anchor, int self)
 {
     const int P = plane_count<GROUND>(p);
@@ -774,16 +828,27 @@
         const double e = unit_excess(d);
         const bool in_window = cull_reads_d(__builtin_amdgcn_ballot_w64(outside_unit_window(e)));
         RT_MARK(6);
-        const int canchor = (opaque(p.anchors) > 0) ? anchor : -1;
-        if (in_window) occ = any_spheres_masks<true>(lds, p, S, canchor, o, d, e, self, live);
-        else occ = any_spheres_masks<false>(lds, p, S, canchor, o, d, e, self, live);
+        const int canchor = (NG > 0 || opaque(p.anchors) > 0) ? anchor : -1;
+        if (in_window) occ = any_spheres_masks<true, NG>(lds, p, S, canchor, o, d, e, self, live);
+        else occ = any_spheres_masks<false, NG>(lds, p, S, canchor, o, d, e, self, live);
     } else {
     const V3 R = renormalize_unit(d);
     const double a = dot3(R, R);
     RT_MARK(6);
-    const int canchor = (opaque(p.anchors) > 0) ? anchor : -1;
+    const int canchor = (NG > 0 || opaque(p.anchors) > 0) ? anchor : -1;
     const lanemask a_sane = lanes_where(a > 0.999999) & lanes_where(a < 1.000001);
     occ = 0ull;
+    if constexpr (NG > 0) {
+      unsigned mask = small_mask(cull_mask<NG>(lds, S, canchor, 0, S, o, R, p.extent2, self), S);
+      RT_MARK(7);
+      while (mask) {
+        const int k = __builtin_ctz(mask);
+        mask &= mask - 1u;
+        occ |= sphere_any_mask<false>(lds, k, o, R, a, a_sane);
+        if (mask && (live & ~occ) == 0ull) break;
+      }
+      RT_MARK(8);
+    } else
     for (int k0 = 0; k0 < S; k0 += 64) {
       if (k0 > 0 && (live & ~occ) == 0ull) break;
       const int n = (S - k0 < 64) ? S - k0 : 64;
@@ -822,10 +887,11 @@
     return lane_of(occ);
 }
 
-template <int MODE, bool GROUND = false>
+template <int MODE, bool GROUND = false, int NG = 0>
 __device__ __forceinline__ bool any_hit(const Lds &lds, const KParams &p, const V3 &o, const V3 &d, int anchor, int self, bool lanes = true)
 {
-    if (MODE == 0 && lds.trim) return any_hit_masks<GROUND>(lds, p, o, d, anchor, self);
+    static_assert(NG == 0 || MODE == 0, "small-scene kernels are wave-uniform (MODE 0)");
+    if (MODE == 0 && lds.trim) return any_hit_masks<GROUND, NG>(lds, p, o, d, anchor, self);
     const int P = plane_count<GROUND>(p);
     const int S = p.S;
     const V3 R = renormalize_unit(d);
@@ -1041,7 +1107,7 @@
     }
 }
 
-template <bool PARK, int WGT, bool COUNT, int MODE, class MS, bool GROUND = false>
+template <bool PARK, int WGT, bool COUNT, int MODE, class MS, bool GROUND = false, int NG = 0>
 __device__ __forceinline__ void trace_bounce(const Lds &lds, const KParams &p, bool &alive, int anchor,
                                              V3 &o, V3 &d, V3 &rgb, RayCount<COUNT> &cnt, MS &ms, int b = 0)
 {
@@ -1052,7 +1118,7 @@
     double t = 999.0; int idx = -1, type = HIT_NONE;
     cnt.closest(alive);
     RT_MARK(11);
-    if (alive) closest_hit<MODE, GROUND>(lds, p, o, d, MS::lens ? -1 : anchor, t, idx, type);
+    if (alive) closest_hit<MODE, GROUND, NG>(lds, p, o, d, MS::lens ? -1 : anchor, t, idx, type);
     if constexpr (MS::sky) {
         if (alive && type == HIT_NONE) rgb = sky_color(p.scene + (size_t)p.lens.sky, d);
     }
@@ -1157,7 +1223,7 @@
                     const double k = SLOT(LAMB) * cN;
                     RT_MARK(5);
                     if (k > 0.0 || (lit_row()[0] > 0.0 && cN > 0.0)) {
-                        const bool occluded = any_hit<MODE, GROUND>(lds, p, Pt, Ld, -1, self, true);
+                        const bool occluded = any_hit<MODE, GROUND, NG>(lds, p, Pt, Ld, -1, self, true);
                         if (!occluded) lit_add(m, k, [&]() { return soft_Ld(again(m), i); });
                     }
                 }
@@ -1173,7 +1239,7 @@
                 const double k = SLOT(LAMB) * cN;
                 RT_MARK(5);
                 if (k > 0.0 || (lit_row()[0] > 0.0 && cN > 0.0)) {
-                    const bool occluded = any_hit<MODE, GROUND>(lds, p, Pt, Ld, 1 + m, self, anchor != 0 || p.lanes_primary);
+                    const bool occluded = any_hit<MODE, GROUND, NG>(lds, p, Pt, Ld, 1 + m, self, anchor != 0 || p.lanes_primary);
                     if (!occluded) lit_add(m, k, [&]() { return point_Ld(again(m)); });
                 }
             }
@@ -1188,7 +1254,7 @@
                 const double k = SLOT(LAMB) * dot3(Ld, N);
                 RT_MARK(5);
                 if (k > 0.0) {
-                    const bool occluded = any_hit<MODE, GROUND>(lds, p, Pt, Ld, -1, self, true);
+                    const bool occluded = any_hit<MODE, GROUND, NG>(lds, p, Pt, Ld, -1, self, true);
                     if (!occluded) lambert_add(k, V3{1.0, 1.0, 1.0});
                 }
             }
@@ -1214,7 +1280,7 @@
             cnt.shadow(true, k > 0.0);
             RT_MARK(5);
             if (k > 0.0) {
-                const bool occluded = any_hit<MODE, GROUND>(lds, p, Pt, Ld, 1 + m, self, anchor != 0 || p.lanes_primary);
+                const bool occluded = any_hit<MODE, GROUND, NG>(lds, p, Pt, Ld, 1 + m, self, anchor != 0 || p.lanes_primary);
                 if (!occluded) lambert_add(k, V3{1.0, 1.0, 1.0});
             }
         }
@@ -1233,7 +1299,7 @@
 }
 
 
-template <bool PARK, int WGT, bool COUNT, int MODE, class MS, bool GROUND = false>
+template <bool PARK, int WGT, bool COUNT, int MODE, class MS, bool GROUND = false, int NG = 0>
 __device__ __forceinline__ V3 sample(const Lds &lds, const KParams &p, bool alive, V3 o, V3 d, RayCount<COUNT> &cnt, MS &ms,
                                      unsigned key = 0u, unsigned lkey = 0u)
 {
@@ -1255,7 +1321,7 @@
 #ifdef RT_REGION_STATS
         ((volatile unsigned *)lds.reg)[(threadIdx.x >> 6) * 32 + 30] = b >= 2 ? 12u : 0u;
 #endif
-        trace_bounce<PARK, WGT, COUNT, MODE, MS, GROUND>(lds, p, alive, b == 0 ? 0 : -1, o, d, rgb, cnt, ms, b);
+        trace_bounce<PARK, WGT, COUNT, MODE, MS, GROUND, NG>(lds, p, alive, b == 0 ? 0 : -1, o, d, rgb, cnt, ms, b);
         if (b == 0) acc.set(rgb);
         else {
             double wgt;
@@ -1460,12 +1526,13 @@
     ty = tile - tx * p.tiles_y;
 }
 
-template <bool AA, bool PARK, int WPW, bool COUNT = false, bool LAT = false, int MODE = 0, Family F = Family::PLAIN, bool GROUND = false>
+template <bool AA, bool PARK, int WPW, bool COUNT = false, bool LAT = false, int MODE = 0, Family F = Family::PLAIN, bool GROUND = false, int NG = 0>
 __global__ __launch_bounds__(64 * WPW, MODE >= 2 ? RT_W_LANES : (AA ? (PARK ? RT_W_AAPARK : 4) : (PARK ? RT_W_PARK : 5))) void render_kernel(const KParams p)
 {
     constexpr int WG_THREADS = 64 * WPW, WAVES_PER_WG = WPW;
     constexpr bool M2 = MODE >= 2;
     constexpr bool NOREC = MODE >= 1;
+    static_assert(NG == 0 || (NG <= 2 && GROUND && WPW == 2 && MODE == 0 && !COUNT && F == Family::PLAIN), "small-scene twins: two-wave ground-plane kernels");
     constexpr bool MAT = has_mat(F), SCAT = has_scat(F), SOFT = has_soft(F), LENS = has_lens(F), TEX = has_tex(F);
     const int nrec = (int)lds_doubles(NOREC ? 0 : p.S, p.P, p.L);
     const double *rec_src = p.scene + (NOREC ? (size_t)p.S * SPH_STRIDE : 0);
@@ -1551,7 +1618,7 @@
         V3 ro = o, rd;
         if constexpr (LENS) lens_ray(p, LAT ? (unsigned)xc : 2u * xc, LAT ? (unsigned)yc : 2u * yc, 0u, P0, ro, rd);
         else rd = primary_dir(p, P0);
-        const V3 c = sample<PARK, WG_THREADS, COUNT, MODE, decltype(ms), GROUND>(lds, p, inb, ro, rd, cnt, ms, key, lkey);
+        const V3 c = sample<PARK, WG_THREADS, COUNT, MODE, decltype(ms), GROUND, NG>(lds, p, inb, ro, rd, cnt, ms, key, lkey);
         R = c.x; G = c.y; B = c.z;
     } else {
         const bool stoch = (p.aa == 2);
@@ -1584,7 +1651,7 @@
             V3 ro = o, rd;
             if constexpr (LENS) lens_ray(p, lx, ly, stoch ? (unsigned)tap : 0u, Pt, ro, rd);
             else rd = primary_dir(p, Pt);
-            const V3 s = sample<PARK, WG_THREADS, COUNT, MODE, decltype(ms), GROUND>(lds, p, (tap && !stoch) ? interior : inb, ro, rd, cnt, ms, key, lkey);
+            const V3 s = sample<PARK, WG_THREADS, COUNT, MODE, decltype(ms), GROUND, NG>(lds, p, (tap && !stoch) ? interior : inb, ro, rd, cnt, ms, key, lkey);
             if (tap == 0) taps.set(s);
             else if (stoch) { const V3 a = taps.get(); taps.set(V3{a.x + s.x, a.y + s.y, a.z + s.z}); }
             else if (interior) { const V3 a = taps.get(); taps.set(V3{a.x + s.x, a.y + s.z, a.z + s.y}); }
diff --git a/python-ray-tracer_amd/csrc/rt_plan.h b/python-ray-tracer_amd/csrc/rt_plan.h
--- a/python-ray-tracer_amd/csrc/rt_plan.h
+++ b/python-ray-tracer_amd/csrc/rt_plan.h
@@ -17,6 +17,7 @@
     int order_tiles = 1;
     int seq_order = -1;
     int ground_plane = 1;
+    int small_scene = 1;
 };
 
 inline Family family_of(const SceneLayout &s, double lens_a)
@@ -79,6 +80,27 @@
 {
     const int code0 = (int)(signed char)(lay.plane_codes & 0xffu);
     return kn.ground_plane != 0 && fam == Family::PLAIN && !(flags & RT_FLAG_COUNT_RAYS) && lay.P == 1 && code0 == 3;
+}
+
+constexpr int SMALL_MAX_GROUPS = 2;
+constexpr Shape SMALL_TWIN[] = {
+    {false, true, 2, false, false, 0},
+    {true, true, 2, false, false, 0},
+    {false, true, 2, false, true, 0},
+};
+constexpr bool has_small_kernel(Family f, const Shape &s)
+{
+    if (!has_ground_kernel(f, s)) return false;
+    for (const Shape &k : SMALL_TWIN)
+        if (k == s) return true;
+    return false;
+}
+
+inline int cull_groups(const SceneLayout &lay, const PlanKnobs &kn, Family fam, int flags, int anchors)
+{
+    if (!ground_plane(lay, kn, fam, flags) || kn.small_scene == 0) return 0;
+    if (lay.NC != 0 || lay.S < 1 || lay.S > 4 * SMALL_MAX_GROUPS || anchors != lay.L + 1) return 0;
+    return (lay.S + 3) / 4;
 }
 
 constexpr int PARK_WAVES = 24;
```

New measurement: 246,800, median of 6. 1.09x the previous value.
